# wiedenhoeft/HaMMLET

Hardware: AMD Instinct MI355X
Metric: block-updates/sec (Gibbs sweep) + HBM GB/s, 10^8 pos / 5 states (higher is better)
Workload: dtype f32; 1 GPU; c3_1e8_k5_dynamic; positions=100000000, states=5, block_structure=dynamic, chains=1, parallelism=chain-parallel x1

## Files before the change

### hammlet_amd/capi.py

```python
import ctypes as C
import os

import numpy as np

from . import build as _build

_lib = None


class HmlError(RuntimeError):
    def __init__(self, code, msg):
        super().__init__(msg)
        self.code = code


class HmlStats(C.Structure):
    _fields_ = [("sweeps", C.c_uint64), ("block_updates", C.c_uint64), ("uniform_fallbacks", C.c_uint64),
                ("forward_refits", C.c_uint64), ("forward_serial", C.c_uint64), ("forward_warmup", C.c_uint64),
                ("fused_fallbacks", C.c_uint64), ("buffer_growths", C.c_uint64), ("block_capacity", C.c_uint64)]


RECORD_CB = C.CFUNCTYPE(None, C.c_void_p, C.c_uint64, C.c_void_p)

_P = C.c_void_p
SIGNATURES = {
    "hml_last_error": (C.c_char_p, []),
    "hml_abi_version": (C.c_uint32, []),
    "hml_device_arch": (C.c_char_p, []),
    "hml_device_count": (C.c_int, [C.POINTER(C.c_int)]),
    "hml_create": (C.c_int, [C.POINTER(_P), C.c_int, C.c_uint64, C.c_uint32, _P]),
    "hml_destroy": (None, [_P]),
    "hml_load_observations": (C.c_int, [_P, _P, C.c_uint64]),
    "hml_load_observations_device": (C.c_int, [_P, _P, C.c_uint64]),
    "hml_attach_observations": (C.c_int, [_P, _P]),
    "hml_text_open": (C.c_int, [C.POINTER(_P), C.c_int, C.c_uint64]),
    "hml_text_close": (None, [_P]),
    "hml_text_buffer": (C.c_int, [_P, C.POINTER(_P), C.POINTER(C.c_uint64)]),
    "hml_text_commit": (C.c_int, [_P, C.c_uint64]),
    "hml_text_feed": (C.c_int, [_P, C.c_char_p, C.c_uint64]),
    "hml_text_reserve": (C.c_int, [_P, C.c_uint64]),
    "hml_text_finish": (C.c_int, [_P, C.POINTER(C.c_uint64), C.POINTER(C.c_int)]),
    "hml_text_values": (C.c_int, [_P, _P]),
    "hml_text_counters": (C.c_int, [_P, C.POINTER(C.c_uint64), C.POINTER(C.c_uint64), C.POINTER(C.c_uint64)]),
    "hml_set_dimensions": (C.c_int, [_P, C.c_int, C.c_int]),
    "hml_get_dimensions": (C.c_int, [_P, C.POINTER(C.c_int), C.POINTER(C.c_int)]),
    "hml_set_weights": (C.c_int, [_P, _P, C.c_uint64]),
    "hml_noise_sigma": (C.c_int, [_P, C.POINTER(C.c_double)]),
    "hml_scale_weights": (C.c_int, [_P, C.c_float]),
    "hml_autoprior": (C.c_int, [_P, C.c_float, C.c_float, _P]),
    "hml_set_model": (C.c_int, [_P, C.c_int, _P, C.c_float, C.c_float, C.c_float, C.c_int]),
    "hml_set_self_transitions": (C.c_int, [_P, C.c_int]),
    "hml_sample_prior": (C.c_int, [_P]),
    "hml_set_static_blocks": (C.c_int, [_P]),
    "hml_set_dynamic": (C.c_int, [_P, C.c_int]),
    "hml_create_blocks": (C.c_int, [_P, C.c_float]),
    "hml_iterate": (C.c_int, [_P, C.c_char, C.c_uint64, C.c_uint64]),
    "hml_iterate_many": (C.c_int, [_P, C.c_int, C.c_char, C.c_uint64, C.c_uint64]),
    "hml_set_recording": (C.c_int, [_P, C.c_int, RECORD_CB, _P]),
    "hml_set_option": (C.c_int, [_P, C.c_char_p, C.c_int]),
    "hml_sync": (C.c_int, [_P]),
    "hml_get_num_blocks": (C.c_int, [_P, C.POINTER(C.c_uint64)]),
    "hml_get_blocks": (C.c_int, [_P, _P]),
    "hml_get_block_stats": (C.c_int, [_P, _P, _P]),
    "hml_get_states": (C.c_int, [_P, _P]),
    "hml_get_theta": (C.c_int, [_P, _P]),
    "hml_get_transitions": (C.c_int, [_P, _P, _P]),
    "hml_set_parameters": (C.c_int, [_P, _P, _P, _P]),
    "hml_get_threshold": (C.c_int, [_P, C.POINTER(C.c_float)]),
    "hml_enable_probes": (C.c_int, [_P, C.c_int]),
    "hml_get_block_loglik": (C.c_int, [_P, _P]),
    "hml_get_forward_rows": (C.c_int, [_P, _P]),
    "hml_get_counts": (C.c_int, [_P, _P, _P, _P, _P, _P]),
    "hml_get_weights": (C.c_int, [_P, _P]),
    "hml_get_coefficients": (C.c_int, [_P, _P]),
    "hml_get_integral_array": (C.c_int, [_P, _P, _P]),
    "hml_marginals_rle": (C.c_int, [_P, C.POINTER(C.c_uint64), C.POINTER(C.c_int), _P, _P]),
    "hml_max_segmentation": (C.c_int, [_P, C.POINTER(C.c_uint64), _P, _P]),
    "hml_marginals_dense_device": (C.c_int, [_P, _P, _P]),
    "hml_recorded_sweeps": (C.c_int, [_P, C.POINTER(C.c_uint64)]),
    "hml_set_level_recording": (C.c_int, [_P, C.c_int]),
    "hml_levels_rle": (C.c_int, [_P, C.POINTER(C.c_uint64), C.POINTER(C.c_uint64), _P, _P, _P]),
    "hml_levels_dense_device": (C.c_int, [_P, _P]),
    "hml_levels_merge": (C.c_int, [_P, _P]),
    "hml_levels_on_segments": (C.c_int, [_P, C.c_uint64, _P, _P, _P]),
    "hml_levels_agreement_rle": (C.c_int, [_P, C.c_int, C.POINTER(C.c_uint64), C.POINTER(C.c_uint64), _P, _P, _P, _P]),
    "hml_levels_agreement_dense_device": (C.c_int, [_P, C.c_int, _P]),
    "hml_levels_agreement_summary": (C.c_int, [_P, C.c_int, C.c_double, _P, _P, _P]),
    "hml_set_break_recording": (C.c_int, [_P, C.c_int]),
    "hml_breaks_list": (C.c_int, [_P, C.POINTER(C.c_uint64), C.POINTER(C.c_uint64), _P, _P]),
    "hml_breaks_dense_device": (C.c_int, [_P, _P, C.c_uint32]),
    "hml_breaks_merge": (C.c_int, [_P, _P]),
    "hml_breaks_consensus": (C.c_int, [_P, C.c_uint32, C.c_uint64, C.POINTER(C.c_uint64), _P, _P, _P]),
    "hml_set_level_bands": (C.c_int, [_P, C.c_int, _P]),
    "hml_get_level_bands": (C.c_int, [_P, C.POINTER(C.c_int), _P]),
    "hml_bands_rle": (C.c_int, [_P, C.POINTER(C.c_uint64), C.POINTER(C.c_int), C.POINTER(C.c_uint64), _P, _P]),
    "hml_bands_dense_device": (C.c_int, [_P, _P, C.c_int]),
    "hml_bands_call": (C.c_int, [_P, C.c_uint64, C.POINTER(C.c_uint64), _P, _P]),
    "hml_bands_merge": (C.c_int, [_P, _P]),
    "hml_recording_payload_size": (C.c_int, [_P, C.c_int, C.POINTER(C.c_uint64)]),
    "hml_recording_export": (C.c_int, [_P, C.c_int, _P, C.c_uint64, C.POINTER(C.c_uint64)]),
    "hml_recording_merge_payload": (C.c_int, [_P, C.c_int, _P, C.c_uint64]),
    "hml_recording_merge_across": (C.c_int, [_P, _P, C.c_int]),
    "hml_categorical_draw": (C.c_int, [_P, _P, C.c_int, C.POINTER(C.c_uint32)]),
    "hml_relabel_permutation": (C.c_int, [_P, _P]),
    "hml_pool_payload_size": (C.c_int, [_P, C.POINTER(C.c_uint64)]),
    "hml_pool_export": (C.c_int, [_P, _P, _P]),
    "hml_pool_install": (C.c_int, [_P, _P]),
    "hml_pool_unique_id": (C.c_int, [_P]),
    "hml_pool_create": (C.c_int, [C.POINTER(_P), C.c_int, C.c_int, C.c_int, _P]),
    "hml_pool_destroy": (None, [_P]),
    "hml_pool_marginals": (C.c_int, [_P, _P, _P]),
    "hml_pool_info": (C.c_int, [_P, C.POINTER(C.c_int), C.POINTER(C.c_int), C.POINTER(C.c_double), C.POINTER(C.c_uint64), C.POINTER(C.c_int)]),
    "hml_pool_set_form": (C.c_int, [_P, C.c_int]),
    "hml_pool_last": (C.c_int, [_P, C.POINTER(C.c_int), C.POINTER(C.c_uint64)]),
    "hml_allreduce_marginals": (C.c_int, [_P, C.c_int]),
    "hml_allreduce_marginals_perm": (C.c_int, [_P, C.c_int, _P]),
    "hml_pool_permutation": (C.c_int, [_P, _P]),
    "hml_get_stats": (C.c_int, [_P, C.POINTER(HmlStats)]),
    "hml_profile_enable": (C.c_int, [_P, C.c_int]),
    "hml_profile_get": (C.c_int, [_P, C.c_char_p, C.POINTER(C.c_double), C.POINTER(C.c_uint64)]),
    "hml_debug_eval": (C.c_int, [C.c_int, C.c_int, _P, _P, _P, C.c_uint64, C.c_uint64]),
    "hml_synth_depth": (C.c_int, [_P, _P, C.c_uint64, C.c_double, C.c_double, C.c_uint64, C.c_int]),
    "hml_synth_gauss": (C.c_int, [_P, _P, C.c_uint64, C.c_int, _P, C.c_float, C.c_double, C.c_uint64, C.c_int]),
}


ABI_VERSION = 5

RECORDING_LEVELS, RECORDING_BREAKS, RECORDING_BANDS = 0, 1, 2


def load_library(path=None):
    global _lib
    if _lib is not None and path is None:
        return _lib
    path = path or os.environ.get("HML_LIBRARY") or _build.LIB_PATH
    if not os.path.exists(path):
        raise HmlError(-1, "%s is missing: build it with `python -c 'import __graft_entry__ as g; g.build()'` "
                           "(hipcc --offload-arch=gfx950); there is no CPU fallback" % path)
    lib = C.CDLL(path, mode=C.RTLD_GLOBAL)
    for name, (res, args) in SIGNATURES.items():
        fn = getattr(lib, name)
        fn.restype = res
        fn.argtypes = args
    if lib.hml_abi_version() != ABI_VERSION:
        raise HmlError(-1, "%s has ABI version %d, this package expects %d: rebuild the library" % (path, lib.hml_abi_version(), ABI_VERSION))
    _lib = lib
    return lib


def _check(rc):
    if rc != 0:
        raise HmlError(rc, load_library().hml_last_error().decode())


def parse_text(source, device=0, chunk_bytes=0, feed_bytes=None, with_info=False):
    lib = load_library()
    h = _P()
    _check(lib.hml_text_open(C.byref(h), device, chunk_bytes))
    try:
        if isinstance(source, (bytes, bytearray, memoryview)):
            data = bytes(source)
            step = feed_bytes or max(len(data), 1)
            for i in range(0, len(data), step):
                part = data[i:i + step]
                _check(lib.hml_text_feed(h, part, len(part)))
        else:
            with open(source, "rb", buffering=0) as f:
                while True:
                    buf, cap = _P(), C.c_uint64()
                    _check(lib.hml_text_buffer(h, C.byref(buf), C.byref(cap)))
                    view = (C.c_char * cap.value).from_address(buf.value)
# ... 569 lines not shown
```

### hammlet_amd/csrc/hml_capi.hip

```cpp
#include "hml_capi_shared.hpp"

static thread_local std::string g_err;
int hml_set_err(int code, const std::string& msg) { g_err = msg; return code; }

static const hml_ktab* ktab(int K);
#define HML_KTAB(KV, tab) const hml_ktab* tab = ktab(KV); if (!tab) return set_err(HML_ERR_ARG, "number of states must be in [2,16]")

std::atomic<int> hml_live_ctx[64];
int hml_ctx_bind(hml_ctx* c) { return ctx_bind(c); }
int hml_ctx_fetch_model(hml_ctx* c, hml_model* out) { return fetch_model(c, out); }

HML_KERNEL void hml_k_debug_eval(int fn, const float* __restrict__ a, const float* __restrict__ b, float* __restrict__ out,
                                 uint64_t n, uint64_t seed) {
    if (fn == 24) {
        const uint64_t nw = ((uint64_t)gridDim.x * blockDim.x) >> 6;
        if ((threadIdx.x & 63) != 0) return;
        for (uint64_t i = ((uint64_t)blockIdx.x * blockDim.x + threadIdx.x) >> 6; i < n; i += nw) {
            hml_dev_src src;
            src.s = hml_stream_open(hml_make_key(seed, 0), HML_KIND_THETA, seed, (uint32_t)i);
            out[i] = hml_gamma_f32<hml_devmath>(src, a[i], b[i]);
        }
        return;
    }
    const uint64_t stride = (uint64_t)gridDim.x * blockDim.x;
// ... 23 lines not shown
            case 40: r = hml_glibc_expf(x); break;
            case 41: r = hml_glibc_logf(x); break;
            case 42: r = hml_glibc_powf_unit(x, y); break;
            case 43: { const double Zd = (double)y; r = hml_tr2_quotient(x, Zd, hml_tr2_reciprocal(Zd)); } break;
            case 10: r = (float)(1.0 / (double)x); break;
            case 12: case 13: case 14: case 15: case 16: case 17: case 18: case 19: case 20: case 21: case 22: case 23: {
                hml_dev_src src; src.s = hml_stream_open(hml_make_key(seed, 0), HML_KIND_THETA, seed, (uint32_t)i);
                const float alpha = x, beta = y; (void)beta;
                const float malpha = alpha < 1.0f ? alpha + 1.0f : alpha;
                const float a1 = malpha - 1.0f / 3.0f;
                const float a2 = 1.0f / hml_devmath::sqrtf_(9.0f * a1);
                hml_normal_f32<hml_devmath> nd;
                float n = nd.draw(src, 0.0f, 1.0f);
                float v = 1.0f + a2 * n;
                float v3 = v * v * v;
                float u = hml_canonical_f32(src);
                const bool c1 = (double)u > (double)1.0f - 0.0331 * (double)n * (double)n * (double)n * (double)n;
                const bool c2 = ((double)hml_devmath::logf_(u) > (0.5 * (double)n * (double)n + (double)a1 * ((1.0 - (double)v3) + (double)hml_devmath::logf_(v3))));
                float n2 = nd.draw(src, 0.0f, 1.0f);
                float vb = 1.0f + a2 * n2;
                float vb3 = vb * vb * vb;
                float ub = hml_canonical_f32(src);
                const bool d1 = (double)ub > (double)1.0f - 0.0331 * (double)n2 * (double)n2 * (double)n2 * (double)n2;
                const bool d2 = ((double)hml_devmath::logf_(ub) > (0.5 * (double)n2 * (double)n2 + (double)a1 * ((1.0 - (double)vb3) + (double)hml_devmath::logf_(vb3))));
                r = fn == 12 ? n : fn == 13 ? v3 : fn == 14 ? u : fn == 15 ? (float)(c1 ? 1 : 0) + 2.0f * (c2 ? 1 : 0) : fn == 16 ? n2 : fn == 17 ? a2
                    : fn == 18 ? vb3 : fn == 19 ? ub : fn == 20 ? (float)(d1 ? 1 : 0) + 2.0f * (d2 ? 1 : 0) : fn == 21 ? (float)src.s.n : 0.0f;
                if (fn == 22) r = nd.draw(src, 0.0f, 1.0f);
                if (fn == 23) { hml_normal_f32<hml_devmath> nf; r = nf.draw(src, 0.0f, 1.0f); r = nf.draw(src, 0.0f, 1.0f); }
            } break;
            case 30: case 31: {
                r = 0.0f;
                const int Kc = fn == 30 ? 16 : 5;
                if (i % Kc == 0 && i + Kc <= n) {
                    bool unsure = false;
                    int fastr, lit;
                    if (fn == 30) { float w[16]; for (int j = 0; j < 16; ++j) w[j] = a[i + j]; fastr = hml_categorical_k_fast<16>(w, (double)y, unsure); lit = hml_categorical_k_literal<16>(w, (double)y); if (unsure) fastr = lit; }
                    else { float w[5]; for (int j = 0; j < 5; ++j) w[j] = a[i + j]; fastr = hml_categorical_k_fast<5>(w, (double)y, unsure); lit = hml_categorical_k_literal<5>(w, (double)y); if (unsure) fastr = lit; }
                    out[i] = (float)fastr; out[i + 1] = (float)lit; out[i + 2] = unsure ? 1.0f : 0.0f;
                }
                continue;
            }
            case 11: { const double d = HML_SQRT((double)x * 1.0000001); r = (float)((d - (double)(float)d) * 1e9); } break;
        }
        out[i] = r;
    }
}

static bool parse_band_edges(const char* text, int* n, float* edges) {
    *n = 0;
    const char* p = text;
    while (*p) {
        char* end = nullptr;
        const float v = strtof(p, &end);
        if (end == p || *n >= HML_MAX_BAND_EDGES) return false;
        edges[(*n)++] = v;
        p = end;
        if (*p == ',') ++p; else if (*p) return false;
    }
    return *n > 0;
}

static const char* band_edges_fault(int n, const float* edges) {
    if (n < 1 || n > HML_MAX_BAND_EDGES) return "level bands take 1 to 31 edges";
    for (int j = 0; j < n; ++j) {
        if (!std::isfinite(edges[j])) return "the edges of the level bands must be finite";
        if (j > 0 && !(edges[j - 1] < edges[j])) return "the edges of the level bands must be strictly ascending";
    }
    return nullptr;
}

static int bands_from_env(hml_ctx* c) {
    if (const char* e = getenv("HML_BANDS")) {
        int n = 0; float edges[HML_MAX_BAND_EDGES];
        if (!parse_band_edges(e, &n, edges)) return set_err(HML_ERR_ARG, "HML_BANDS: expected up to 31 comma-separated numbers");
        if (const char* why = band_edges_fault(n, edges)) return set_err(HML_ERR_ARG, std::string("HML_BANDS: ") + why);
        c->n_band_edges = n;
        memcpy(c->band_edges, edges, (size_t)n * sizeof(float));
        c->rec[HML_REC_BANDS].on = c->rec[HML_REC_BANDS].asked = true;
    }
    return 0;
}

extern "C" {

const char* hml_last_error(void) { return g_err.c_str(); }
uint32_t hml_abi_version(void) { return 5; }
const char* hml_device_arch(void) { return "gfx950"; }
int hml_device_count(int* n) {
    if (!n) return set_err(HML_ERR_ARG, "null argument");
    HIPCHK(hipGetDeviceCount(n));
    return 0;
}

static void free_all(hml_ctx* c);

static int create_inner(hml_ctx* c, void* stream) {
    HIPCHK(hipSetDevice(c->device));
    if (stream) { c->stream = (hipStream_t)stream; c->own_stream = false; }
    else { HIPCHK(hipStreamCreateWithFlags(&c->stream, hipStreamNonBlocking)); c->own_stream = true; }
    HIPCHK(hipMalloc(&c->d_mdl, sizeof(hml_model)));
    HIPCHK(hipMemsetAsync(c->d_mdl, 0, sizeof(hml_model), c->stream));
    HIPCHK(hipHostMalloc(&c->h_B, 4 * sizeof(uint32_t), hipHostMallocMapped));
    c->h_B[0] = 0; c->h_B[1] = 0; c->h_B[2] = 0; c->h_B[3] = 0;
    HIPCHK(hipHostGetDevicePointer((void**)&c->d_hB, c->h_B, 0));
    return 0;
}

int hml_create(hml_ctx** out, int device, uint64_t seed, uint32_t chain_id, void* stream) {
    if (!out) return set_err(HML_ERR_ARG, "null output pointer");
    int n = 0;
    HIPCHK(hipGetDeviceCount(&n));
    if (n <= 0) return set_err(HML_ERR_HIP, "no HIP device available: the MI355X kernels cannot run (there is no CPU fallback)");
    if (device < 0 || device >= n) return set_err(HML_ERR_ARG, "device index out of range");
    hml_ctx* c = new hml_ctx();
    c->device = device; c->seed = seed; c->chain = chain_id;
    if (int r = create_inner(c, stream)) {
        free_all(c);
        if (c->own_stream && c->stream) hipStreamDestroy(c->stream);
        delete c;
        return r;
    }
    if (const char* e = getenv("HML_FWD_CHUNK")) { int l = std::max(1, atoi(e)); int sh = 0; while ((1 << (sh + 1)) <= l && sh < 10) ++sh; c->fwdL = 1 << sh; }
    if (const char* e = getenv("HML_FWD_WARMUP")) c->fwdW = c->fwdW_init = std::max(0, atoi(e));
    if (const char* e = getenv("HML_FWD_BURNIN_SWEEPS")) c->fwd_burnin_sweeps = (uint32_t)std::max(0, atoi(e));
    if (const char* e = getenv("HML_FWD_QUIET")) c->fwd_quiet_need = (uint32_t)std::max(1, atoi(e));
    if (const char* e = getenv("HML_FWD_CHUNK_MANY")) { int l = std::max(1, atoi(e)); int sh = 0; while ((1 << (sh + 1)) <= l && sh < 6) ++sh; c->fwdL_many = 1 << sh; }
    if (const char* e = getenv("HML_FWD_CHUNK_MID")) { int l = std::max(1, atoi(e)); int sh = 0; while ((1 << (sh + 1)) <= l && sh < 10) ++sh; c->fwdL_mid = 1 << sh; }
    if (const char* e = getenv("HML_MID_MIN_BLOCKS")) c->mid_min_blocks = (uint32_t)strtoul(e, nullptr, 10);
    if (const char* e = getenv("HML_FWD_CHUNK_DENSE")) { int l = std::max(1, atoi(e)); int sh = 0; while ((1 << (sh + 1)) <= l && sh < 10) ++sh; c->fwdL_dense = 1 << sh; }
    if (const char* e = getenv("HML_DENSE_MIN_BLOCKS")) c->dense_min_blocks = (uint32_t)strtoul(e, nullptr, 10);
    if (const char* e = getenv("HML_USE_GRAPH")) c->use_graph = atoi(e) != 0;
    if (const char* e = getenv("HML_WEIGHT_KEYS")) c->use_keys = atoi(e) != 0;
    if (const char* e = getenv("HML_FUSED_BLOCKS")) { c->fused_blocks = atoi(e) != 0; c->fused_keep = atoi(e) == 2; }
    if (const char* e = getenv("HML_TRELLIS_FUSED")) c->tre_fused = atoi(e) != 0;
    if (const char* e = getenv("HML_TRELLIS_L")) { const int l = atoi(e); c->tre_L = (l <= 0) ? 0u : (l >= HML_TRE_MAX_L) ? (uint32_t)HML_TRE_MAX_L : (l < 32) ? 32u : (uint32_t)l / 32u * 32u; }
    if (const char* e = getenv("HML_TRELLIS_CKPT")) c->tre_ckpt = atoi(e) != 0;
    if (const char* e = getenv("HML_TRELLIS_REFIT_ROUNDS")) { const int r = atoi(e); c->tre_refit_rounds = r < 0 ? 0u : r > 6 ? 6u : (uint32_t)r; }
    if (const char* e = getenv("HML_STAGE_BITS")) c->stage_bits = atoi(e) != 0;
    if (const char* e = getenv("HML_TRELLIS_ROWS")) c->tre_rows = atoi(e) != 0;
    if (const char* e = getenv("HML_LATE_RESCALE")) c->late_rescale = atoi(e) != 0;
    if (const char* e = getenv("HML_PARAMS_SPREAD")) c->params_spread = atoi(e) != 0;
    if (const char* e = getenv("HML_COMPAT_CHUNKS")) c->compat_chunks = atoi(e);
    if (const char* e = getenv("HML_COMPAT_WARMUP")) c->compat_warmup = atoi(e);
    if (const char* e = getenv("HML_WIDE_LANES")) c->wide_lanes = atoi(e);
    if (const char* e = getenv("HML_WIDE_W0")) c->wide_w0 = std::max(8, atoi(e));
    if (const char* e = getenv("HML_WIDE_MAX_CHUNKS")) c->wide_max_chunks = (uint32_t)std::max(64, atoi(e));
    if (const char* e = getenv("HML_WIDE_L")) {
        const int L = atoi(e);
        if (L >= 1) { int sh = 0; while ((1 << sh) < L && sh < 20) ++sh; c->wide_lshift = sh; }
    }
    if (const char* e = getenv("HML_COMPAT")) c->compat = atoi(e) != 0;
    if (const char* e = getenv("HML_TRELLIS_TUNE")) c->tre_autotune = atoi(e) != 0;
    if (const char* e = getenv("HML_FUSED_SPIN_LIMIT")) c->fused_spin_limit = (uint32_t)strtoul(e, nullptr, 10);
    if (const char* e = getenv("HML_LEVELS")) c->rec[HML_REC_LEVELS].on = c->rec[HML_REC_LEVELS].asked = atoi(e) != 0;
    if (const char* e = getenv("HML_BREAKS")) c->rec[HML_REC_BREAKS].on = c->rec[HML_REC_BREAKS].asked = atoi(e) != 0;
    if (const char* e = getenv("HML_MAX_BLOCKS")) c->cap_opt = strtoull(e, nullptr, 10);
    if (device < 64) g_live_ctx[device].fetch_add(1);
    if (int r = bands_from_env(c)) { hml_destroy(c); return r; }
    *out = c;
    return 0;
}

static void trace_release(hml_ctx* c) {
    if (c->trace) {
        if (c->trace->refs.fetch_sub(1) == 1) {
            void* ptrs[] = {c->trace->d_w, c->trace->d_summary, c->trace->d_coeff, c->trace->d_ia};
            for (void* p : ptrs) if (p) hipFree(p);
            delete c->trace;
        }
        c->trace = nullptr;
    } else {
        void* ptrs[] = {c->d_w, c->d_summary, c->d_coeff, c->d_ia};
        for (void* p : ptrs) if (p) hipFree(p);
    }
    c->d_w = nullptr; c->d_summary = nullptr; c->d_coeff = nullptr; c->d_ia = nullptr;
}
static bool trace_shared(const hml_ctx* c) { return c->trace && c->trace->refs.load() > 1; }

static void free_sweep_buffers(hml_ctx* c, bool keep_engine = false) {
    void** ptrs[] = {(void**)&c->d_em, (void**)&c->d_gsc, (void**)&c->d_rows, (void**)&c->d_entry, (void**)&c->d_exitA, (void**)&c->d_redo, (void**)&c->d_touched,
                     (void**)&c->d_fb, (void**)&c->d_smap, (void**)&c->d_cmap, (void**)&c->d_scmap, (void**)&c->d_super, (void**)&c->d_bentry2, (void**)&c->d_bentry,
                     (void**)&c->d_q, (void**)&c->d_partial, (void**)&c->d_redo2, (void**)&c->d_tre_bitmap, (void**)&c->d_tre_ckpt, (void**)&c->d_crows, (void**)&c->d_cchunk, (void**)&c->d_cdraws, (void**)&c->d_clists, (void**)&c->d_wacc, (void**)&c->d_wA};
    for (void** p : ptrs) if (*p) { hipFree(*p); *p = nullptr; }
    if (!keep_engine && c->d_mt) { hipFree(c->d_mt); c->d_mt = nullptr; }
}

static void free_all(hml_ctx* c) {
    trace_release(c);
    free_sweep_buffers(c);
    void* ptrs[] = {c->d_group_word, c->d_wave_total, c->d_stage, c->d_span_count, c->d_starts, c->d_bstat, c->d_eprobe, c->d_aprobe, c->d_coarse1,
                    c->d_diff, c->d_boundary, c->d_mdl, c->d_many};
    for (void* p : ptrs) if (p) hipFree(p);
    for (hml_recorder& r : c->rec) { if (r.d_acc) hipFree(r.d_acc); if (r.d_boundary) hipFree(r.d_boundary); }
    if (c->h_B) hipHostFree(c->h_B);
    c->h_B = nullptr;
}


void hml_destroy(hml_ctx* c) {
    if (!c) return;
    if (c->device < 64) g_live_ctx[c->device].fetch_sub(1);
    hipSetDevice(c->device);
    hipStreamSynchronize(c->stream);
    for (auto& kv : c->prof) for (auto& p : kv.second.pending) { hipEventDestroy(p.first); hipEventDestroy(p.second); }
    for (auto e : c->ev_pool) hipEventDestroy(e);
    if (c->graph_exec) hipGraphExecDestroy(c->graph_exec);
    free_all(c);
    if (c->own_stream) hipStreamDestroy(c->stream);
    delete c;
}

static int build_keys(hml_ctx* c) {
    if (!c->use_keys) return 0;
    const uint64_t T = c->T;
    if (!c->d_summary) {
        const uint64_t n_spans = (T + HML_SPAN - 1) / HML_SPAN;
        HIPCHK(hipMalloc(&c->d_summary, n_spans * (HML_SPAN / 16) + 16));
        HIPCHK(hipMemsetAsync(c->d_summary, 0, n_spans * (HML_SPAN / 16) + 16, c->stream));
    }
    const float thr0 = (float)(std::sqrt(2 * std::log((double)std::max<uint64_t>(T, 2))) * c->sigma * c->key_scale);
    uint32_t u; memcpy(&u, &thr0, 4);
    c->key_base = (std::isfinite(thr0) && thr0 > 0 ? (int32_t)(u >> 20) : (int32_t)(0x3f800000u >> 20)) - 128;
    hipLaunchKernelGGL(hml_k_build_summary, dim3(grid_for((T + 15) / 16, 256, 1, 65536)), dim3(256), 0, c->stream, c->d_w, T,
                       c->key_base, c->d_summary);
    KLAUNCH_CHECK();
    return 0;
}

HML_KERNEL void hml_k_max_inplace(float* __restrict__ a, const float* __restrict__ b, uint64_t n) {
    const uint64_t stride = (uint64_t)gridDim.x * blockDim.x;
    for (uint64_t i = (uint64_t)blockIdx.x * blockDim.x + threadIdx.x; i < n; i += stride) { const float x = a[i], y = b[i]; a[i] = (x < y) ? y : x; }
}

static int alloc_block_buffers(hml_ctx* c) {
    const uint64_t T = c->T;
    c->n_spans = (uint32_t)((T + HML_SPAN - 1) / HML_SPAN);
    HIPCHK(hipMalloc(&c->d_stage, (uint64_t)c->n_spans * HML_SPAN * sizeof(uint16_t)));
    HIPCHK(hipMalloc(&c->d_span_count, c->n_spans * sizeof(uint32_t)));
    HIPCHK(hipMalloc(&c->d_starts, (c->cap + 1) * sizeof(uint32_t)));
    HIPCHK(hipMalloc(&c->d_coarse1, ((c->n_spans + HML_GROUP_SPANS - 1) / HML_GROUP_SPANS + 1u) * sizeof(uint32_t)));
    {
        const uint64_t n_tiles = (T + HML_FUSED_SUB_POSITIONS - 1) / HML_FUSED_SUB_POSITIONS;
        HIPCHK(hipMalloc(&c->d_group_word, (n_tiles + 1) * sizeof(unsigned long long)));
        HIPCHK(hipMemsetAsync(c->d_group_word, 0, (n_tiles + 1) * sizeof(unsigned long long), c->stream));
        HIPCHK(hipMalloc(&c->d_wave_total, (n_tiles + 1) * (HML_FUSED_WAVES + 2) * sizeof(uint32_t)));
        if (getenv("HML_FUSED_DEBUG")) { HIPCHK(hipMalloc(&c->d_dbg, 4096 * 8 * 8)); HIPCHK(hipMemset(c->d_dbg, 0, 4096 * 8 * 8)); }
    }
    HIPCHK(hipMalloc(&c->d_bstat, c->cap * (uint64_t)c->D * sizeof(float2)));
    const uint32_t cap32 = (uint32_t)c->cap;
    HIPCHK(hipMemcpyAsync(&c->d_mdl->cap, &cap32, sizeof cap32, hipMemcpyHostToDevice, c->stream));
    return 0;
}

static void choose_capacity(hml_ctx* c, bool attached) {
    const uint64_t T = c->T;
    uint64_t cap = T;
    if (c->D == 1) {
        if (c->cap_opt) cap = c->cap_opt;
        else if (attached) cap = std::max<uint64_t>(1ull << 20, T / 16);
    }
    c->cap = std::min<uint64_t>(std::max<uint64_t>(cap, 64), T);
}

static int build_from_device_x(hml_ctx* c, const float* const* d_x, const float* const* h_x) {
    const uint64_t T = c->T;
    const int D = c->D;
    {
        trace_release(c);
        void** stale[] = {(void**)&c->d_stage, (void**)&c->d_span_count, (void**)&c->d_starts, (void**)&c->d_coarse1, (void**)&c->d_group_word, (void**)&c->d_wave_total, (void**)&c->d_bstat};
        for (void** q : stale) if (*q) { hipFree(*q); *q = nullptr; }
    }
    {
        const float sqrt2 = (float)std::sqrt(2.0);
        const float sqrt2half = (float)(sqrt2 / 2.0);
        double acc = 0; uint64_t cnt = 0;
        for (uint64_t i = 1; i < T; i += 2) {
            float mx = 0.0f;
            for (int d = 0; d < D; ++d) {
                const float df = std::abs(h_x[d][i - 1] - h_x[d][i]);
                const float cf = sqrt2half * df;
                mx = (mx < cf) ? cf : mx;
            }
            acc += mx;
            cnt++;
        }
        acc /= cnt;
        acc /= 0.797884560802865355879892119868763736951717262329869315331;
        c->sigma = acc;
    }
    HIPCHK(hipMalloc(&c->d_w, T * sizeof(float)));
    HIPCHK(hipMalloc(&c->d_coeff, T * sizeof(float)));
    HIPCHK(hipMalloc(&c->d_ia, (T + 1) * (uint64_t)D * sizeof(float2)));
    {
        float h_norm[64];
        const float sqrt2 = (float)std::sqrt(2.0);
        const float sqrt2half = (float)(sqrt2 / 2.0);
        h_norm[0] = 1.0f;
        float nrm = sqrt2half;
        for (int l = 1; l < 64; ++l) { h_norm[l] = nrm; nrm *= sqrt2half; }
        DevScratch s_norm, s_a, s_b, s_other;
        HIPCHK(hipMalloc(&s_norm.p, sizeof h_norm));
        float* d_norm = s_norm.as<float>();
        HIPCHK(hipMemcpyAsync(d_norm, h_norm, sizeof h_norm, hipMemcpyHostToDevice, c->stream));
        const uint64_t n1 = T >> HML_MAXLET_LOG_TILE;
        HIPCHK(hipMalloc(&s_a.p, std::max<uint64_t>(n1, 1) * sizeof(float)));
        HIPCHK(hipMalloc(&s_b.p, std::max<uint64_t>(n1 >> HML_MAXLET_LOG_TILE, 1) * sizeof(float)));
        if (D > 1) HIPCHK(hipMalloc(&s_other.p, T * sizeof(float)));
        float *bufA = s_a.as<float>(), *bufB = s_b.as<float>(), *d_other = s_other.as<float>();
        for (int d = 0; d < D; ++d) {
            float* coeff_out = d == 0 ? c->d_coeff : d_other;
            uint64_t n = T;
            int base = 0;
            const float* in = d_x[d];
            float* outb = bufA;
            while (true) {
                const uint64_t tiles = (n + HML_MAXLET_TILE - 1) / HML_MAXLET_TILE;
                hipLaunchKernelGGL(hml_k_maxlet, dim3((unsigned)tiles), dim3(256), 0, c->stream, in, n, base, coeff_out, T, outb, d_norm);
                KLAUNCH_CHECK();
                base += HML_MAXLET_LOG_TILE;
                if (base >= 40 || (1ull << base) >= T) break;
                n = T >> base;
                in = outb;
                outb = (outb == bufA) ? bufB : bufA;
            }
            if (d > 0) {
                hipLaunchKernelGGL(hml_k_max_inplace, dim3(grid_for(T, 256, 1, 65536)), dim3(256), 0, c->stream, c->d_coeff, d_other, T);
                KLAUNCH_CHECK();
            }
        }
        HIPCHK(hipStreamSynchronize(c->stream));
    }
    hipLaunchKernelGGL(hml_k_weights, dim3(grid_for(T, 256, 1, 65536)), dim3(256), 0, c->stream, c->d_coeff, c->d_w, T, 1.0f);
    KLAUNCH_CHECK();
    if (int r = build_keys(c)) return r;
    {
        const uint64_t cells = (T + 1 + HML_CELLSIZE - 1) / HML_CELLSIZE;
        for (int d = 0; d < D; ++d) {
            hipLaunchKernelGGL(hml_k_integral, dim3((unsigned)((cells + 3) / 4)), dim3(256), 0, c->stream, d_x[d], c->d_ia + (uint64_t)d * (T + 1), T);
            KLAUNCH_CHECK();
        }
    }
    choose_capacity(c, false);
    if (int r = alloc_block_buffers(c)) return r;
    HIPCHK(hipStreamSynchronize(c->stream));
    c->trace = new hml_trace();
    c->trace->d_w = c->d_w; c->trace->d_summary = c->d_summary; c->trace->d_coeff = c->d_coeff; c->trace->d_ia = c->d_ia;
    c->loaded = true;
    return 0;
}

int hml_set_dimensions(hml_ctx* c, int D, int P) {
    if (!c) return set_err(HML_ERR_ARG, "null context");
    if (c->loaded) return set_err(HML_ERR_ARG, "dimensions must be set before the observations are loaded");
    if (D <= 0) return set_err(HML_ERR_MODEL, "Number of data dimensions must be positive!");
    if (P < 0) return set_err(HML_ERR_MODEL, "Number of parameters must be positive!");
    if (D > HML_MAX_D) return set_err(HML_ERR_ARG, "at most 4 data dimensions are supported");
    if (P > 0) {
        long k = 1;
        for (int d = 0; d < D; ++d) { k *= P; if (k > HML_CAP_K) return set_err(HML_ERR_ARG, "number of states must be in [2,64]"); }
        if (k <= 1) return set_err(HML_ERR_MODEL, "Requested parameters would yield an HMM with less than 2 states!");
    }
    c->D = D; c->P = P;
    return 0;
}

int hml_load_observations(hml_ctx* c, const float* x, uint64_t n_values) {
    if (!c || !x) return set_err(HML_ERR_ARG, "null argument");
    if (n_values == 0) return set_err(HML_ERR_ARG, "Input vector for breakpoint weights is empty!");
    const uint64_t D = (uint64_t)c->D;
    if (n_values % D != 0) return set_err(HML_ERR_MODEL, "Input stream did not contain enough values to fill all dimensions at last position!");
    const uint64_t T = n_values / D;
    if (T >= 0xffffffffull) return set_err(HML_ERR_ARG, "at most 2^32-2 positions are supported");
    if (c->loaded) return set_err(HML_ERR_ARG, "observations already loaded");
    if (int r = ctx_bind(c)) return r;
    c->T = T;
    DevScratch s_x;
    HIPCHK(hipMalloc(&s_x.p, n_values * sizeof(float)));
    float* d_x = s_x.as<float>();
    std::vector<float> planes;
    const float* h_dim[HML_MAX_D];
    const float* d_dim[HML_MAX_D];
    if (D == 1) { h_dim[0] = x; }
    else {
        planes.resize(n_values);
        for (uint64_t t = 0; t < T; ++t) for (uint64_t d = 0; d < D; ++d) planes[d * T + t] = x[t * D + d];
        for (uint64_t d = 0; d < D; ++d) h_dim[d] = planes.data() + d * T;
    }
    HIPCHK(hipMemcpyAsync(d_x, D == 1 ? x : planes.data(), n_values * sizeof(float), hipMemcpyHostToDevice, c->stream));
    for (uint64_t d = 0; d < D; ++d) d_dim[d] = d_x + d * T;
    return build_from_device_x(c, d_dim, h_dim);
}

int hml_load_observations_device(hml_ctx* c, const void* x_dev, uint64_t T) {
    if (!c || !x_dev) return set_err(HML_ERR_ARG, "null argument");
    if (c->D != 1) return set_err(HML_ERR_ARG, "device input is univariate");
    if (T == 0) return set_err(HML_ERR_ARG, "Input vector for breakpoint weights is empty!");
    if (T >= 0xffffffffull) return set_err(HML_ERR_ARG, "at most 2^32-2 positions are supported");
    if (c->loaded) return set_err(HML_ERR_ARG, "observations already loaded");
    if (int r = ctx_bind(c)) return r;
    c->T = T;
    std::vector<float> h(T);
    HIPCHK(hipMemcpy(h.data(), x_dev, T * sizeof(float), hipMemcpyDeviceToHost));
    const float* h_dim[1] = {h.data()};
    const float* d_dim[1] = {(const float*)x_dev};
    return build_from_device_x(c, d_dim, h_dim);
}

int hml_attach_observations(hml_ctx* c, hml_ctx* src) {
    if (!c || !src) return set_err(HML_ERR_ARG, "null argument");
    if (c == src) return set_err(HML_ERR_ARG, "a context cannot be attached to itself");
    if (!src->loaded || !src->trace) return set_err(HML_ERR_ARG, "the source context has no observations loaded");
    if (c->loaded) return set_err(HML_ERR_ARG, "observations already loaded");
    if (c->device != src->device) return set_err(HML_ERR_ARG, "contexts that share observations must live on one device");
    if (c->use_keys != src->use_keys) return set_err(HML_ERR_ARG, "option weight_keys differs from the source context's");
    if (int r = ctx_bind(c)) return r;
    HIPCHK(hipStreamSynchronize(src->stream));
    trace_release(c);
    {
        void** stale[] = {(void**)&c->d_stage, (void**)&c->d_span_count, (void**)&c->d_starts, (void**)&c->d_coarse1, (void**)&c->d_group_word, (void**)&c->d_wave_total, (void**)&c->d_bstat};
        for (void** q : stale) if (*q) { hipFree(*q); *q = nullptr; }
    }
    c->T = src->T; c->D = src->D;
    if (c->P == 0 || c->D > 1) c->P = src->P;
    c->sigma = src->sigma; c->key_base = src->key_base; c->key_scale = src->key_scale;
    c->trace = src->trace;
    c->trace->refs.fetch_add(1);
    c->d_w = src->d_w; c->d_summary = src->d_summary; c->d_coeff = src->d_coeff; c->d_ia = src->d_ia;
    choose_capacity(c, true);
    if (int r = alloc_block_buffers(c)) { trace_release(c); return r; }
    HIPCHK(hipStreamSynchronize(c->stream));
    c->loaded = true;
    return 0;
}

int hml_noise_sigma(hml_ctx* c, double* sigma) {
    if (!c || !c->loaded) return set_err(HML_ERR_ARG, "no observations loaded");
    *sigma = c->sigma;
    return 0;
}

int hml_scale_weights(hml_ctx* c, float mult) {
    if (!c || !c->loaded) return set_err(HML_ERR_ARG, "no observations loaded");
    if (trace_shared(c)) return set_err(HML_ERR_ARG, "the weights are shared with attached contexts: scale them before hml_attach_observations");
    if (int r = ctx_bind(c)) return r;
    hipLaunchKernelGGL(hml_k_scale, dim3(grid_for(c->T, 256, 1, 65536)), dim3(256), 0, c->stream, c->d_w, c->T, mult);
    KLAUNCH_CHECK();
    c->key_scale *= std::fabs((double)mult) > 0 ? std::fabs((double)mult) : 1.0;
    if (int r = build_keys(c)) return r;
    c->blocks_valid = false;
    return 0;
}

int hml_set_weights(hml_ctx* c, const float* w, uint64_t T) {
    if (!c || !c->loaded || !w) return set_err(HML_ERR_ARG, "no observations loaded");
    if (T != c->T) return set_err(HML_ERR_MODEL, "Block structure and statistics have different number of data points!");
    if (trace_shared(c)) return set_err(HML_ERR_ARG, "the weights are shared with attached contexts: set them before hml_attach_observations");
    if (int r = ctx_bind(c)) return r;
    HIPCHK(hipMemcpyAsync(c->d_w, w, T * sizeof(float), hipMemcpyHostToDevice, c->stream));
    HIPCHK(hipStreamSynchronize(c->stream));
    if (int r = build_keys(c)) return r;
    c->blocks_valid = false;
    c->hint_stale = true;
    return 0;
}

}

extern "C" {
}
static int grow_capacity(hml_ctx* c, uint64_t needed);
static int enumerate_blocks_sync(hml_ctx* c, float threshold) {
    if (int r = settle_if_limited(c)) return r;
    for (int round = 0; round < 64; ++round) {
        if (int r = launch_compact(c, true, threshold)) return r;
        HIPCHK(hipStreamSynchronize(c->stream));
        if (!chain_halted(c)) return 0;
        if (int r = grow_capacity(c, c->h_B[2])) return r;
    }
    return set_err(HML_ERR_HIP, "internal error: the block capacity did not settle");
}
extern "C" {

int hml_create_blocks(hml_ctx* c, float threshold) {
    if (!c || !c->loaded) return set_err(HML_ERR_ARG, "no observations loaded");
    if (int r = ctx_bind(c)) return r;
    if (int r = enumerate_blocks_sync(c, threshold)) return r;
    refresh_hint(c);
    c->blocks_valid = false;
    return 0;
}

int hml_autoprior(hml_ctx* c, float s2, float p, float out4[4]) {
    if (!c || !c->loaded) return set_err(HML_ERR_ARG, "no observations loaded");
    if (int r = ctx_bind(c)) return r;
    const float thr0 = (float)(std::sqrt(2 * std::log((double)c->T)) * c->sigma);
    if (int r = enumerate_blocks_sync(c, thr0)) return r;
    refresh_hint(c);
    const uint32_t B = *c->h_B;
    std::vector<uint32_t> st(B + 1);
    const int D = c->D;
    std::vector<float2> bs((size_t)B * D);
    HIPCHK(hipMemcpy(st.data(), c->d_starts, (B + 1) * sizeof(uint32_t), hipMemcpyDeviceToHost));
    for (int d = 0; d < D; ++d)
        HIPCHK(hipMemcpy(bs.data() + (size_t)d * B, c->d_bstat + (uint64_t)d * c->cap, B * sizeof(float2), hipMemcpyDeviceToHost));
    float muSum = 0, muSq = 0;
    for (uint32_t b = 0; b < B; ++b) {
        for (int d = 0; d < D; ++d) {
            const float m = bs[(size_t)d * B + b].x / (float)(st[b + 1] - st[b]);
            muSum += m;
            muSq += m * m;
        }
    }
    const double n = (double)((uint64_t)B * (uint64_t)D);
    const double blocksMean = (double)(float)(muSum / n);
    const double avg = (double)(float)(muSum / n);
    const double blocksVar = (double)(float)(muSq / n - (avg * avg));
    const float dataMean = (float)blocksMean, dataVar = (float)blocksVar;
    if (p < 0 || p > 1) return set_err(HML_ERR_MODEL, "Parameter p for automatic priors is a probability and must be in [0,1]!");
    if (s2 <= 0) return set_err(HML_ERR_MODEL, "Parameter s2  for automatic priors is a variance and must be positive!");
    if (dataVar <= 0) return set_err(HML_ERR_MODEL, "Data variance provided to autoprior must be positive!");
    const float M1 = 0.3361, M2 = -0.0042, M3 = -0.0201;
    const float b = -std::log(p);
    const float alpha = 2.0;
    const float beta = s2 * ((2.0 * std::sqrt(b)) / (M1 * std::sqrt(b) + std::sqrt(2.0) * (M2 * b * std::exp(M3 * std::sqrt(b)) + 1)) + b);
    const float mu0 = dataMean;
    const float nu = beta / dataVar;
    if (beta <= 0) return set_err(HML_ERR_MODEL, "Autoprior yields non-positive beta!");
    if (nu <= 0) return set_err(HML_ERR_MODEL, "Autoprior yields non-positive nu!");
    if (!std::isfinite(beta)) return set_err(HML_ERR_MODEL, "Autoprior yields non-finite beta!");
    if (!std::isfinite(mu0)) return set_err(HML_ERR_MODEL, "Autoprior yields non-finite mu0!");
    if (!std::isfinite(nu)) return set_err(HML_ERR_MODEL, "Autoprior yields non-finite nu!");
    out4[0] = alpha; out4[1] = beta; out4[2] = mu0; out4[3] = nu;
    return 0;
}

}

static uint64_t compat_list_entries(const hml_ctx* c) { return (c->cap + 4u * (uint64_t)HML_CAP_K + 3u) & ~(uint64_t)3u; }

static uint32_t wide_max_chunks_of(const hml_ctx* c) {
    if (c->wide_max_chunks) return std::min<uint32_t>(c->wide_max_chunks, HML_WL_MAX_CHUNKS);
    return c->K <= HML_WL_TWO_WAVES_KC ? (uint32_t)HML_WL_MAX_CHUNKS : (uint32_t)HML_WL_MAX_CHUNKS / 2u;
}

static int alloc_sweep_buffers(hml_ctx* c) {
    const int K = c->K;
    const uint64_t cap = c->cap;
    if (c->compat) {
        HIPCHK(hipMalloc(&c->d_em, cap * K * sizeof(float)));
        HIPCHK(hipMalloc(&c->d_gsc, cap * K * sizeof(float)));
        HIPCHK(hipMalloc(&c->d_crows, (cap + 1) * K * sizeof(float)));
        HIPCHK(hipMalloc(&c->d_cchunk, (uint64_t)HML_COMPAT_MAX_CHUNKS * (2 * K * sizeof(float) + 4 * sizeof(uint32_t)) + 64));
        HIPCHK(hipMalloc(&c->d_cdraws, 2 * cap * sizeof(uint32_t)));
        HIPCHK(hipMalloc(&c->d_clists, 3 * compat_list_entries(c) * sizeof(uint32_t) + (uint64_t)HML_CAP_K * HML_CAP_K * sizeof(unsigned long long) +
                                        ((cap + HML_COMPAT_PART_TILE - 1) / HML_COMPAT_PART_TILE) * K * sizeof(uint32_t) + 2 * (HML_CAP_K + 1) * sizeof(uint32_t) + 64));
        HIPCHK(hipMalloc(&c->d_q, cap * sizeof(int16_t)));
        return 0;
    }
    if (c->wide) {
        uint64_t Lmax = 1ull << HML_WL_MIN_LSHIFT;
        if (c->wide_lshift >= 0) Lmax = std::max<uint64_t>(Lmax, 1ull << c->wide_lshift);
        while ((cap + Lmax - 1) / Lmax > (uint64_t)wide_max_chunks_of(c)) Lmax *= 2;
        const uint64_t plane = (cap + 1 + 64 * Lmax) * K;
        HIPCHK(hipMalloc(&c->d_em, plane * sizeof(float)));
        HIPCHK(hipMalloc(&c->d_gsc, plane * sizeof(float)));
        HIPCHK(hipMalloc(&c->d_crows, plane * sizeof(float)));
        const uint64_t Lmin = c->wide_lshift >= 0 ? (1ull << c->wide_lshift) : (1ull << HML_WL_MIN_LSHIFT);
        c->wide_chunks_cap = std::max<uint64_t>(HML_COMPAT_MAX_CHUNKS, std::min<uint64_t>(HML_WL_MAX_CHUNKS, (cap + Lmin - 1) / Lmin + 64));
        const uint64_t chunk_bytes = c->wide_chunks_cap * (2 * K * sizeof(float) + 4 * sizeof(uint32_t));
        HIPCHK(hipMalloc(&c->d_cchunk, chunk_bytes + HML_WL_TOT_WORDS * sizeof(unsigned long long)));
        HIPCHK(hipMemsetAsync((char*)c->d_cchunk + chunk_bytes, 0, HML_WL_TOT_WORDS * sizeof(unsigned long long), c->stream));
        HIPCHK(hipMalloc(&c->d_wA, ((uint64_t)HML_WL_PITCH * HML_WL_PITCH + (uint64_t)HML_CAP_K * HML_WL_GTAB) * sizeof(float)));
        HIPCHK(hipMalloc(&c->d_cdraws, 2 * (cap + 1) * sizeof(uint32_t)));
        HIPCHK(hipMalloc(&c->d_q, cap * sizeof(int16_t)));
        const uint64_t n_partial = (uint64_t)HML_REDUCE_GROUPS * K * 2;
        HIPCHK(hipMalloc(&c->d_partial, n_partial * sizeof(double)));
        HIPCHK(hipMemsetAsync(c->d_partial, 0, n_partial * sizeof(double), c->stream));
        HIPCHK(hipMalloc(&c->d_wacc, sizeof(hml_wide_acc)));
        HIPCHK(hipMemsetAsync(c->d_wacc, 0, sizeof(hml_wide_acc), c->stream));
        return 0;
    }
    const int minL = std::min(std::min(std::min(c->fwdL, c->fwdL_dense), c->fwdL_many), c->fwdL_mid);
    const uint64_t maxChunks = (cap + minL - 1) / minL + 1;
    uint64_t plane = 0;
    auto layout = [&](int L, hml_layout& lay) {
        int sh = 0; while ((1 << sh) < L) ++sh;
        lay.lshift = (uint32_t)sh;
        lay.cstride = (uint32_t)(((cap + L - 1) / L + 1 + 63) / 64 * 64);
        plane = std::max(plane, (uint64_t)L * K * lay.cstride);
    };
    layout(c->fwdL, c->lay);
    layout(c->fwdL_dense, c->lay_dense);
    layout(c->fwdL_mid, c->lay_mid);
    layout(c->fwdL_many, c->lay_many);
    HIPCHK(hipMalloc(&c->d_em, plane * sizeof(float)));
    HIPCHK(hipMalloc(&c->d_gsc, plane * sizeof(float)));
    HIPCHK(hipMalloc(&c->d_rows, plane * sizeof(float)));
    HIPCHK(hipMalloc(&c->d_entry, maxChunks * K * sizeof(float)));
    HIPCHK(hipMalloc(&c->d_exitA, maxChunks * K * sizeof(float)));
    HIPCHK(hipMalloc(&c->d_fb, maxChunks * sizeof(uint32_t)));
    HIPCHK(hipMalloc(&c->d_smap, (cap + 2) * sizeof(unsigned long long)));
    const uint64_t bchunks = (cap + 15) / 16 + 1;
    HIPCHK(hipMalloc(&c->d_cmap, bchunks * sizeof(unsigned long long)));
    HIPCHK(hipMalloc(&c->d_bentry, bchunks));
    HIPCHK(hipMalloc(&c->d_scmap, bchunks * sizeof(unsigned long long)));
    HIPCHK(hipMalloc(&c->d_super, (bchunks / 64 + 2) * sizeof(unsigned long long)));
    HIPCHK(hipMalloc(&c->d_bentry2, bchunks / 64 + 2));
    HIPCHK(hipMalloc(&c->d_redo, bchunks * sizeof(uint32_t)));
    HIPCHK(hipMemsetAsync(c->d_redo, 0, bchunks * sizeof(uint32_t), c->stream));
    HIPCHK(hipMalloc(&c->d_touched, bchunks * sizeof(uint32_t)));
    HIPCHK(hipMemsetAsync(c->d_touched, 0, bchunks * sizeof(uint32_t), c->stream));
    HIPCHK(hipMalloc(&c->d_redo2, bchunks * sizeof(uint32_t)));
    HIPCHK(hipMalloc(&c->d_tre_bitmap, (bchunks / 32 + 2) * sizeof(uint32_t)));
    HIPCHK(hipMalloc(&c->d_tre_ckpt, (cap / HML_TRE_CKPT_ROWS + 64) * (uint64_t)(K + 1) * sizeof(uint32_t)));
    HIPCHK(hipMalloc(&c->d_q, cap * sizeof(int16_t)));
    const uint64_t n_partial = ((uint64_t)HML_REDUCE_GROUPS + HML_PARAMS_TREE_WGS) * K * 2;
    HIPCHK(hipMalloc(&c->d_partial, n_partial * sizeof(double)));
    HIPCHK(hipMemsetAsync(c->d_partial, 0, n_partial * sizeof(double), c->stream));
    return 0;
}

static int grow_capacity(hml_ctx* c, uint64_t needed) {
    const uint64_t cap = std::min<uint64_t>(c->T, std::max<uint64_t>(needed + needed / 2 + 1024, 2 * c->cap));
    if (c->graph_exec) { hipGraphExecDestroy(c->graph_exec); c->graph_exec = nullptr; }
    void** blocks[] = {(void**)&c->d_starts, (void**)&c->d_bstat};
    for (void** q : blocks) if (*q) { hipFree(*q); *q = nullptr; }
    free_sweep_buffers(c,  true);
    if (c->d_eprobe) { hipFree(c->d_eprobe); c->d_eprobe = nullptr; }
    if (c->d_aprobe) { hipFree(c->d_aprobe); c->d_aprobe = nullptr; }
    c->cap = cap;
    HIPCHK(hipMalloc(&c->d_starts, (cap + 1) * sizeof(uint32_t)));
    HIPCHK(hipMalloc(&c->d_bstat, cap * (uint64_t)c->D * sizeof(float2)));
    if (c->model_set) {
        if (int r = alloc_sweep_buffers(c)) return r;
        if (c->probes) {
            HIPCHK(hipMalloc(&c->d_eprobe, c->cap * c->K * sizeof(float)));
            HIPCHK(hipMalloc(&c->d_aprobe, (c->cap + 1) * c->K * sizeof(float)));
        }
    }
    const uint32_t words[2] = {(uint32_t)cap, 0u};
    static_assert(offsetof(hml_model, halted) == offsetof(hml_model, cap) + sizeof(uint32_t), "cap and halted are written together");
    HIPCHK(hipMemcpyAsync(&c->d_mdl->cap, words, sizeof words, hipMemcpyHostToDevice, c->stream));
    HIPCHK(hipStreamSynchronize(c->stream));
    c->h_B[2] = 0u;
    c->blocks_valid = false;
    c->hint_stale = false;
    c->grown++;
    return 0;
}

static int sweep_dispatch(hml_ctx* c, char method, bool record);

int hml_settle(hml_ctx* c) {
    for (int round = 0; round < 64; ++round) {
        HIPCHK(hipStreamSynchronize(c->stream));
        if (!chain_halted(c)) { c->sweep_log.clear(); c->log_base = c->requested; return 0; }
        const uint64_t needed = c->h_B[2];
        if (c->cap >= c->T) return set_err(HML_ERR_HIP, "internal error: a chain with full block capacity halted");
        std::vector<uint8_t> pending;
        if (c->model_set) {
            hml_model m;
            if (int r = fetch_model(c, &m)) return r;
            const uint64_t ran = m.sweeps >= c->log_base ? m.sweeps - c->log_base : 0;
            if (ran < c->sweep_log.size()) pending.assign(c->sweep_log.begin() + ran, c->sweep_log.end());
            c->log_base = m.sweeps;
        }
        if (int r = grow_capacity(c, needed)) return r;
        c->sweep_log = pending;
        bool halted_again = false;
        for (size_t i = 0; i < pending.size() && !halted_again; ++i) {
            const char method = (pending[i] & 1) ? HML_METHOD_MIXTURE : HML_METHOD_FB;
            const bool record = (pending[i] & 2) != 0;
            if (int r = sweep_dispatch(c, method, record)) return r;
            if (record && c->cb) {
                HIPCHK(hipStreamSynchronize(c->stream));
                halted_again = chain_halted(c);
                if (!halted_again) {
                    if (int r = check_device_error(c)) return r;
                    const unsigned long long ordinal = c->log_base + i;
                    c->cb(c, ordinal >= c->call_base ? (uint64_t)(ordinal - c->call_base) : 0u, c->cb_user);
                }
            }
        }
    }
    return set_err(HML_ERR_HIP, "internal error: the block capacity did not settle");
}

extern "C" {

int hml_set_model(hml_ctx* c, int K, const float nig4[4], float a_off, float a_diag, float pi_alpha, int self_trans) {
    if (!c || !c->loaded) return set_err(HML_ERR_ARG, "no observations loaded");
    if (K < 2) return set_err(HML_ERR_MODEL, "Requested parameters would yield an HMM with less than 2 states!");
    if (K > HML_CAP_K) return set_err(HML_ERR_ARG, "number of states must be in [2,64]");
    if (c->model_set) return set_err(HML_ERR_ARG, "model already set");
    if (c->D > 1 && c->P == 0) {
        for (int pp = 2; pp <= K; ++pp) { long k = 1; for (int d = 0; d < c->D; ++d) k *= pp; if (k == K) { c->P = pp; break; } if (k > K) break; }
        if (c->P == 0) return set_err(HML_ERR_ARG, "number of states must be (number of parameters)^(data dimensions)");
    }
    if (c->P > 0) {
        long k = 1;
        for (int d = 0; d < c->D; ++d) k *= c->P;
        if (k != K) return set_err(HML_ERR_ARG, "number of states must be (number of parameters)^(data dimensions)");
    }
    if (!(nig4[0] > 0)) return set_err(HML_ERR_MODEL, "Alpha (" + std::to_string(nig4[0]) + ") must be positive!");
    if (!(nig4[1] > 0)) return set_err(HML_ERR_MODEL, "Beta (" + std::to_string(nig4[1]) + ") must be positive!");
    if (!(nig4[3] > 0)) return set_err(HML_ERR_MODEL, "Nu (" + std::to_string(nig4[3]) + ")must be positive!");
    const hml_ktab* kt = nullptr;
    c->wide = !c->compat && (K > HML_MAX_K || (getenv("HML_WIDE") && atoi(getenv("HML_WIDE")) != 0));
    if (!c->compat && !c->wide) { kt = ktab(K); if (!kt) return set_err(HML_ERR_ARG, "number of states must be in [2,16]"); }
    if (int r = ctx_bind(c)) return r;
    free_sweep_buffers(c);
    c->K = K;
    if (!getenv("HML_PARAMS_SPREAD")) c->params_spread = K >= 8;
    const uint64_t T = c->T;
    if (int r = alloc_sweep_buffers(c)) return r;

    hml_model m;
    memset(&m, 0, sizeof m);
    m.K = K; m.self_trans = self_trans ? 1 : 0; m.dynamic = 1; m.T = (uint32_t)T;
    m.D = c->D; m.P = c->P > 0 ? c->P : K; m.stat_stride = T;
    m.cap = (uint32_t)c->cap;
    for (int st = 0; st < K; ++st) {
        int nn = st;
        for (int d = 0; d < HML_MAX_D; ++d) { m.map[st][d] = (uint8_t)(d < c->D ? nn % m.P : 0); nn /= m.P; }
    }
    for (int i = 0; i < 4; ++i) m.nig_prior[i] = nig4[i];
    m.a_off = a_off; m.a_diag = a_diag; m.pi_alpha = pi_alpha;
    m.key = hml_make_key(c->seed, c->chain);
    for (int k = 0; k < K; ++k) {
        for (int i = 0; i < 4; ++i) m.nig_post[k][i] = nig4[i];
        m.dirPi[k] = pi_alpha;
        m.pi[k] = 1.0f / K;
        for (int j = 0; j < K; ++j) { m.dirA[k * K + j] = (k == j) ? a_diag : a_off; m.A[k * K + j] = 1.0f / K; }
    }
    m.max_state_recorded = -1;
    m.tre_fused = (c->tre_fused && c->D == 1) ? 1u : 0u;
    m.tre_hi_shift = 17u; m.tre_lo_shift = 20u;
    if (const char* e = getenv("HML_TRE_REFIT_SHIFTS")) { unsigned a = 17, b = 20; if (sscanf(e, "%u,%u", &a, &b) == 2 && a < 32 && b < 32) { m.tre_hi_shift = a; m.tre_lo_shift = b; } }
    m.fwd_W0 = (uint32_t)c->fwdW;
    m.fwd_W = m.fwd_W_burnin = (uint32_t)std::max(c->fwdW, c->fwdW_init);
    if (c->compat || c->wide) { m.fwd_W = 64u; m.fwd_W0 = c->wide ? (uint32_t)c->wide_w0 : 32u; }
    m.wl_bwd_W = 64u; m.wl_bwd_quiet = 0u; m.wl_retry = 0u; m.wl_W_need = 0u; m.wl_need_age = 0u;
    m.fwd_burnin_sweeps = c->fwd_burnin_sweeps;
    m.fwd_quiet_need = c->fwd_quiet_need;
    m.n_spans = c->n_spans;
    HIPCHK(hipMemcpyAsync(c->d_mdl, &m, sizeof m, hipMemcpyHostToDevice, c->stream));
    HIPCHK(hipStreamSynchronize(c->stream));
    c->dynamic = true;
    c->hint_stale = true;
    if (c->compat) {
        hml_mt_state h;
        hml_mt_seed(&h, c->seed + (uint64_t)c->chain);
        HIPCHK(hipMalloc(&c->d_mt, sizeof(hml_mt_state)));
        HIPCHK(hipMemcpyAsync(c->d_mt, &h, sizeof h, hipMemcpyHostToDevice, c->stream));
        HIPCHK(hipStreamSynchronize(c->stream));
        hipLaunchKernelGGL(hml_k_compat_draw, dim3(1), dim3(64), 0, c->stream, c->d_mdl, (hml_mt_state*)c->d_mt, 2);
        KLAUNCH_CHECK();
        c->model_set = true;
        return 0;
    }
    if (c->wide) hipLaunchKernelGGL(hml_k_wide_params, dim3(1), dim3(1024), 0, c->stream, c->d_mdl, c->d_partial, (hml_wide_acc*)c->d_wacc, 2);
    else kt->params(c, 2);
    KLAUNCH_CHECK();
    c->model_set = true;
    return 0;
}

int hml_sample_prior(hml_ctx* c) {
    if (!c || !c->model_set) return set_err(HML_ERR_ARG, "model not set");
    if (int r = ctx_bind(c)) return r;
    if (int r = settle_if_limited(c)) return r;
    if (c->compat) {
        hipLaunchKernelGGL(hml_k_compat_draw, dim3(1), dim3(64), 0, c->stream, c->d_mdl, (hml_mt_state*)c->d_mt, 1);
    } else if (c->wide) {
        hipLaunchKernelGGL(hml_k_wide_params, dim3(1), dim3(1024), 0, c->stream, c->d_mdl, c->d_partial, (hml_wide_acc*)c->d_wacc, 1);
    } else { HML_KTAB(c->K, kt); kt->params(c, 1); }
    KLAUNCH_CHECK();
    if (c->dynamic) c->blocks_valid = false;
    c->hint_stale = true;
    return 0;
}

HML_KERNEL __launch_bounds__(64) void hml_k_set_self_trans(hml_model* mdl, int on) {
    if (threadIdx.x == 0) mdl->self_trans = on;
}

int hml_set_self_transitions(hml_ctx* c, int on) {
    if (!c || !c->model_set) return set_err(HML_ERR_ARG, "model not set");
    if (int r = ctx_bind(c)) return r;
    if (int r = settle_if_limited(c)) return r;
    hipLaunchKernelGGL(hml_k_set_self_trans, dim3(1), dim3(64), 0, c->stream, c->d_mdl, on ? 1 : 0);
    KLAUNCH_CHECK();
    if (c->graph_exec) { hipGraphExecDestroy(c->graph_exec); c->graph_exec = nullptr; }
    return 0;
}

int hml_set_static_blocks(hml_ctx* c) {
    if (!c || !c->model_set) return set_err(HML_ERR_ARG, "model not set");
    if (int r = ctx_bind(c)) return r;
    if (int r = settle_if_limited(c)) return r;
    hipLaunchKernelGGL(hml_k_set_dynamic, dim3(1), dim3(64), 0, c->stream, c->d_mdl, 0, 1);
    KLAUNCH_CHECK();
    c->dynamic = false;
    if (!cap_limited(c)) {
        if (int r = launch_compact(c, false, 0.0f)) return r;
    } else {
        bool fitted = false;
        for (int round = 0; round < 64 && !fitted; ++round) {
            if (int r = launch_compact(c, false, 0.0f)) return r;
            HIPCHK(hipStreamSynchronize(c->stream));
            fitted = !chain_halted(c);
            if (!fitted) { if (int r = grow_capacity(c, c->h_B[2])) return r; }
        }
        if (!fitted) return set_err(HML_ERR_HIP, "internal error: the block capacity did not settle");
        refresh_hint(c);
    }
    c->blocks_valid = true;
    return 0;
}

int hml_set_dynamic(hml_ctx* c, int on) {
    if (!c || !c->model_set) return set_err(HML_ERR_ARG, "model not set");
    if (int r = ctx_bind(c)) return r;
    if (int r = settle_if_limited(c)) return r;
    hipLaunchKernelGGL(hml_k_set_dynamic, dim3(1), dim3(64), 0, c->stream, c->d_mdl, on ? 1 : 0, on ? 1 : 0);
    KLAUNCH_CHECK();
    c->dynamic = on != 0;
    if (on) { c->blocks_valid = false; c->hint_stale = true; }
    return 0;
}

int hml_set_recording(hml_ctx* c, int marginals, hml_record_cb cb, void* user) {
// ... 161 lines not shown
    const int mix = method == HML_METHOD_MIXTURE ? 1 : 0;
    const bool lanes = c->wide_lanes != 0 && !c->probes && !mix && c->compat_chunks == 0;
    if (lanes) {
        hml_compat_chunks ch = chunk_views(c);
        ch.W = c->compat_warmup > 0 ? (uint32_t)c->compat_warmup : c->compat_warmup < 0 ? 0u : HML_CHUNK_W_ADAPTIVE;
        const uint64_t room = (uint64_t)hint + hint / 4 + 1024;
        hipLaunchKernelGGL(hml_k_wl_prepare, dim3(1), dim3(256), 0, s, c->d_mdl, c->d_wA, c->wide_lshift, wide_max_chunks_of(c));
        hipLaunchKernelGGL(hml_k_wl_gtable, dim3(grid_for((uint64_t)c->K * HML_WL_GTAB, 256, 1, 512)), dim3(256), 0, s, c->d_mdl, c->d_wA + HML_WL_PITCH * HML_WL_PITCH);
        {
            ProfScope ps(c, "stats_emission");
            hipLaunchKernelGGL(hml_k_wl_emission, dim3(grid_for(room, 64 * HML_WL_EMIT_ROWS * 4, 1, 32768)), dim3(256), 0, s, c->d_mdl, c->d_starts, c->d_bstat, c->d_em, c->d_gsc, c->d_wA + HML_WL_PITCH * HML_WL_PITCH);
        }
        const uint64_t minL = c->wide_lshift >= 0 ? (1ull << c->wide_lshift) : (1ull << HML_WL_MIN_LSHIFT);
        const int tiles = grid_for(room, (int)std::min<uint64_t>(64 * minL, 1u << 30), 1, HML_WL_MAX_CHUNKS / 64);
#define HML_WL_FB(KC)                                                                                                                                   \
        case KC: {                                                                                                                                      \
            constexpr int KS = (KC <= 32) ? 32 : 64;                                                                                                    \
            {                                                                                                                                           \
                ProfScope ps(c, "forward");                                                                                                             \
                hipLaunchKernelGGL(HIP_KERNEL_NAME(hml_k_wl_forward<KC>), dim3(tiles), dim3(64), 0, s, c->d_mdl, c->d_wA, c->d_em, c->d_gsc, c->d_crows, ch, 0); \
                hipLaunchKernelGGL(hml_k_wl_forward_verify, dim3(grid_for(room / 16 * c->K, 256, 1, 4096)), dim3(256), 0, s, c->d_mdl, ch, 0);          \
                                      \
                hipLaunchKernelGGL(hml_k_wl_retry_decide, dim3(1), dim3(256), 0, s, c->d_mdl, ch);                                                      \
                hipLaunchKernelGGL(HIP_KERNEL_NAME(hml_k_wl_forward<KC>), dim3(tiles), dim3(64), 0, s, c->d_mdl, c->d_wA, c->d_em, c->d_gsc, c->d_crows, ch, 1); \
                hipLaunchKernelGGL(hml_k_wl_forward_verify, dim3(grid_for(room / 16 * c->K, 256, 1, 4096)), dim3(256), 0, s, c->d_mdl, ch, 1);          \
                hipLaunchKernelGGL(HIP_KERNEL_NAME(hml_k_wl_forward_check<KS>), dim3(1), dim3(256), 0, s, c->d_mdl, c->d_em, c->d_gsc, c->d_crows, ch);  \
            }                                                                                                                                           \
            {                                                                                                                                           \
                ProfScope ps(c, "backward_maps");                                                                                                       \
                hipLaunchKernelGGL(HIP_KERNEL_NAME(hml_k_wl_backward<KC>), dim3(tiles), dim3(64), 0, s, c->d_mdl, c->d_crows, c->d_q, ch);               \
                hipLaunchKernelGGL(hml_k_wl_backward_verify, dim3(grid_for(room / 16, 256, 1, 256)), dim3(256), 0, s, c->d_mdl, ch);                     \
                hipLaunchKernelGGL(HIP_KERNEL_NAME(hml_k_wl_backward_check<KS>), dim3(1), dim3(256), 0, s, c->d_mdl, c->d_crows, c->d_q, ch);          \
            }                                                                                                                                           \
        } break;
        switch ((c->K + 3) / 4 * 4) {
            HML_WL_FB(4) HML_WL_FB(8) HML_WL_FB(12) HML_WL_FB(16)
            HML_WL_FB(20) HML_WL_FB(24) HML_WL_FB(28) HML_WL_FB(32) HML_WL_FB(36) HML_WL_FB(40) HML_WL_FB(44) HML_WL_FB(48) HML_WL_FB(52) HML_WL_FB(56)
            HML_WL_FB(60) HML_WL_FB(64)
            default: return set_err(HML_ERR_HIP, "internal error: a model of this many states on the path for more than 16");
        }
#undef HML_WL_FB
    } else {
    {
        ProfScope ps(c, "stats_emission");
        hipLaunchKernelGGL(hml_k_wide_emission, dim3(grid_for(hint, 256, 1, 4096)), dim3(256), 0, s, c->d_mdl, c->d_starts, c->d_bstat,
                           c->d_em, c->d_gsc, mix, c->probes ? c->d_eprobe : nullptr);
    }
    if (mix) hipLaunchKernelGGL(hml_k_wide_mixture, dim3(grid_for(hint, 256, 1, 16384)), dim3(256), 0, s, c->d_mdl, c->d_em, c->d_q);
    else {
        float* const aprobe = c->probes ? c->d_aprobe : nullptr;
        uint32_t C = 1u;
        if (!c->probes && c->compat_chunks > 1) C = std::min<uint32_t>((uint32_t)c->compat_chunks, HML_COMPAT_MAX_CHUNKS);
        else if (!c->probes && c->compat_chunks == 0 && hint >= 2048u) C = std::min<uint32_t>((uint32_t)HML_COMPAT_MAX_CHUNKS, hint / 64u);
        hml_compat_chunks ch = chunk_views(c);
        ch.W = c->compat_warmup > 0 ? (uint32_t)c->compat_warmup : c->compat_warmup < 0 ? 0u : HML_CHUNK_W_ADAPTIVE;
        hipLaunchKernelGGL(hml_k_wide_uniforms, dim3(grid_for((hint + 1u) / 2u, 256, 1, 4096)), dim3(256), 0, s, c->d_mdl, c->d_cdraws);
        if (c->K <= 32) launch_chunked_fb<32, hml_dev_exp, true>(c, s, C, ch, aprobe);
        else launch_chunked_fb<64, hml_dev_exp, true>(c, s, C, ch, aprobe);
    }
    }
    {
        ProfScope ps(c, "counts");
        hipLaunchKernelGGL(hml_k_wide_counts, dim3(HML_REDUCE_GROUPS), dim3(256), 0, s, c->d_q, c->d_starts, c->d_bstat, c->d_mdl, c->d_partial, (hml_wide_acc*)c->d_wacc);
    }
    if (record && c->rec_marginals) {
        if (c->pooled) return set_err(HML_ERR_ARG, "the marginals of this context are pooled (common labels, several chains): further sweeps cannot be recorded into them");
        if (int r = ensure_marginal_buffers(c)) return r;
        hipLaunchKernelGGL(hml_k_record, dim3(grid_for(hint, 256, 64, 16384)), dim3(256), 0, s, c->d_q, c->d_starts, c->d_mdl, c->d_diff, c->d_boundary);
    }
    {
        ProfScope ps(c, "params");
        hipLaunchKernelGGL(hml_k_wide_params, dim3(1), dim3(1024), 0, s, c->d_mdl, c->d_partial, (hml_wide_acc*)c->d_wacc, 0);
    }
    if (record) { if (int r = launch_recorders(c, s, hint)) return r; }
    KLAUNCH_CHECK();
    return 0;
}

static int sweep_dispatch(hml_ctx* c, char method, bool record) {
    if (c->compat) return sweep_compat(c, method, record);
    if (c->wide) return sweep_wide(c, method, record);
    HML_KTAB(c->K, kt);
    return kt->sweep(c, method, record);
}

extern "C" {

int hml_iterate(hml_ctx* c, char method, uint64_t iterations, uint64_t thinning) {
    if (!c || !c->model_set) return set_err(HML_ERR_ARG, "model not set");
    if (method != HML_METHOD_FB && method != HML_METHOD_MIXTURE)
        return set_err(HML_ERR_ARG, std::string("Unknown sampling type ") + method + "!");
    if (int r = ctx_bind(c)) return r;
    c->call_base = c->requested;
    if (thinning > 0 && thinning <= iterations && c->rec_marginals && c->pooled)
        return set_err(HML_ERR_ARG, "the marginals of this context are pooled (common labels, several chains): further sweeps cannot be recorded into them");
    for (uint64_t i = 0; i < iterations; ++i) {
        const bool record = thinning > 0 && ((i + 1) % thinning == 0);
        if (chain_halted(c)) { if (int r = hml_settle(c)) return r; }
        refresh_hint(c);
        const bool tre_path = c->tre_fused && c->D == 1 && method == HML_METHOD_FB && c->B_hint >= c->dense_min_blocks;
        if (c->use_graph && !c->compat && !record && !c->profiling && !c->probes && (c->dynamic || c->blocks_valid) &&
            !(tre_path && tre_wants_measurement(c, c->B_hint))) {
            const uint32_t hint = c->B_hint;
            bool unused = false;
            const bool wants_fused = c->fused_blocks && !(c->h_B[1] && !c->fused_keep) && !shares_device(c);
            const bool stale = !c->graph_exec || c->graph_method != method || c->graph_dynamic != c->dynamic ||
                               hint > c->graph_hint || hint * 2u < c->graph_hint || c->graph_fused != wants_fused ||
                               c->graph_dense != (hint >= c->dense_min_blocks) || c->graph_mid != (hint >= c->mid_min_blocks) ||
                               (tre_path && c->graph_tre_L != tre_pick_L(c, hint, true, &unused));
            if (stale && hint) {
                if (c->graph_exec) { hipGraphExecDestroy(c->graph_exec); c->graph_exec = nullptr; }
                hipGraph_t g = nullptr;
                HIPCHK(hipStreamBeginCapture(c->stream, hipStreamCaptureModeThreadLocal));
                int rr = sweep_dispatch(c, method, false);
                const hipError_t ec = hipStreamEndCapture(c->stream, &g);
                if (rr || ec != hipSuccess) {
                    if (g) hipGraphDestroy(g);
                    (void)hipGetLastError();
                    return rr ? rr : set_err(HML_ERR_HIP, std::string("hipStreamEndCapture: ") + hipGetErrorString(ec));
                }
                const hipError_t ei = hipGraphInstantiate(&c->graph_exec, g, nullptr, nullptr, 0);
                hipGraphDestroy(g);
                if (ei != hipSuccess) { c->graph_exec = nullptr; return set_err(HML_ERR_HIP, std::string("hipGraphInstantiate: ") + hipGetErrorString(ei)); }
                c->graph_method = method; c->graph_dynamic = c->dynamic; c->graph_hint = c->B_hint; c->graph_fused = wants_fused;
                c->graph_dense = c->B_hint >= c->dense_min_blocks;
                c->graph_mid = c->B_hint >= c->mid_min_blocks;
            }
            if (c->graph_exec) {
                log_sweep(c, method, false);
                HIPCHK(hipGraphLaunch(c->graph_exec, c->stream));
                if (tre_path) c->tre_dense_sweeps++;
                continue;
            }
        }
        log_sweep(c, method, record);
        if (int r = sweep_dispatch(c, method, record)) return r;
        if (record && c->cb) {
            HIPCHK(hipStreamSynchronize(c->stream));
            if (chain_halted(c)) { if (int r = hml_settle(c)) return r; continue; }
            if (int r = check_device_error(c)) return r;
            c->cb(c, i, c->cb_user);
        }
    }
    return 0;
}

}

extern "C" int hml_iterate_many(hml_ctx* const* cs, int n, char method, uint64_t iterations, uint64_t thinning) {
    if (!cs || n < 1) return set_err(HML_ERR_ARG, "no contexts");
    for (int i = 0; i < n; ++i) if (!cs[i] || !cs[i]->model_set) return set_err(HML_ERR_ARG, "model not set");
    if (method != HML_METHOD_FB && method != HML_METHOD_MIXTURE) return set_err(HML_ERR_ARG, std::string("Unknown sampling type ") + method + "!");
    for (int i = 0; i < n; ++i) cs[i]->call_base = cs[i]->requested;
    uint64_t done = 0;
    while (done < iterations && many_eligible(cs, n, method)) {
        if (int r = ctx_bind(cs[0])) return r;
        for (int i = 0; i < n; ++i) {
            hml_ctx* c = cs[i];
            if (int r = settle_if_limited(c)) return r;
            if (c->hint_stale) { launch_compact_pair(c, 0, 0.0f); KLAUNCH_CHECK(); }
            HIPCHK(hipStreamSynchronize(c->stream));
            c->hint_stale = false;
            if (c->graph_exec) { hipGraphExecDestroy(c->graph_exec); c->graph_exec = nullptr; }
        }
        int r = 0;
        uint64_t reached = done;
        { HML_KTAB(cs[0]->K, kt); r = kt->iterate_many(cs, n, done, iterations, thinning, &reached); }
        if (r) return r;
        hipEvent_t ev = ev_get(cs[0]);
        HIPCHK(hipEventRecord(ev, cs[0]->stream));
        for (int i = 1; i < n; ++i) HIPCHK(hipStreamWaitEvent(cs[i]->stream, ev, 0));
        cs[0]->ev_pool.push_back(ev);
        if (reached == iterations) return 0;
        HIPCHK(hipStreamSynchronize(cs[0]->stream));
        bool halted = false;
        for (int i = 0; i < n; ++i) halted = halted || chain_halted(cs[i]);
        const bool progress = reached > done;
        done = reached;
        if (!halted && !progress) break;
        if (!halted) { bool sparse = true; for (int i = 0; i < n; ++i) sparse = sparse && many_sparse(cs[i]); if (!sparse) break; }
    }
    for (int i = 0; i < n; ++i) if (int r = settle_if_limited(cs[i])) return r;
    for (uint64_t i = done; i < iterations; ++i) {
        const bool record = thinning > 0 && ((i + 1) % thinning == 0);
        for (int k = 0; k < n; ++k) {
            hml_ctx* c = cs[k];
            if (int r = ctx_bind(c)) return r;
            if (record && c->rec_marginals && c->pooled) return set_err(HML_ERR_ARG, "the marginals of a context are pooled (common labels, several chains): further sweeps cannot be recorded into them");
            if (chain_halted(c)) { if (int r = hml_settle(c)) return r; }
            log_sweep(c, method, record);
            if (int r = sweep_dispatch(c, method, record)) return r;
            if (record && c->cb) {
                HIPCHK(hipStreamSynchronize(c->stream));
                if (chain_halted(c)) { if (int r = hml_settle(c)) return r; continue; }
                if (int r = check_device_error(c)) return r;
                c->cb(c, i, c->cb_user);
            }
        }
    }
    return 0;
}

extern "C" {

int hml_set_option(hml_ctx* c, const char* name, int value) {
    if (!c || !name) return set_err(HML_ERR_ARG, "null argument");
    if (std::string(name) == "weight_keys") {
        if (c->loaded) return set_err(HML_ERR_ARG, "weight_keys must be set before the observations are loaded");
        c->use_keys = value != 0;
        c->summary_always = value == 2;
        return 0;
    }
    if (std::string(name) == "max_blocks") {
        if (c->loaded) return set_err(HML_ERR_ARG, "max_blocks must be set before the observations are loaded");
        if (value < 0) return set_err(HML_ERR_ARG, "max_blocks: a number of blocks, or 0 for the default");
        c->cap_opt = (uint64_t)value;
        return 0;
    }
    if (std::string(name) == "fused_blocks") {
        c->fused_blocks = value != 0;
        c->fused_keep = value == 2;
        if (c->graph_exec) { hipGraphExecDestroy(c->graph_exec); c->graph_exec = nullptr; }
        return 0;
    }
    if (std::string(name) == "compat") {
        if (c->model_set) return set_err(HML_ERR_ARG, "compat must be set before the model");
        c->compat = value != 0;
        return 0;
    }
    if (std::string(name) == "trellis_L") {
        if (value < 0 || value > HML_TRE_MAX_L || value % 32) return set_err(HML_ERR_ARG, "trellis_L: 0 or a multiple of 32 up to 1024");
        c->tre_L = (uint32_t)value;
        return 0;
    }
    return set_err(HML_ERR_ARG, std::string("unknown option ") + name);
}

int hml_sync(hml_ctx* c) {
    if (!c) return set_err(HML_ERR_ARG, "null context");
    if (int r = ctx_bind(c)) return r;
    if (int r = hml_settle(c)) return r;
    if (c->d_dbg && getenv("HML_FUSED_DEBUG") && atoi(getenv("HML_FUSED_DEBUG")) == 2) {
        std::vector<unsigned long long> h(4096 * 8);
        hipMemcpy(h.data(), c->d_dbg, h.size() * 8, hipMemcpyDeviceToHost);
        uint32_t n = 0; while (n < 4096 && h[n * 8]) ++n;
        unsigned long long t0 = ~0ull; for (uint32_t i = 0; i < n; ++i) t0 = std::min(t0, h[i * 8]);
        double mx[5] = {0, 0, 0, 0, 0}, av[5] = {0, 0, 0, 0, 0};
        if (n) for (uint32_t i = 0; i < n; ++i) for (int k = 0; k < 5; ++k) { const double d = (double)(h[i * 8 + k] - t0) * 0.01; mx[k] = std::max(mx[k], d); av[k] += d / n; }
        if (n) fprintf(stderr, "[fused-many dbg] n=%u start avg %.2f max %.2f | phaseA avg %.2f max %.2f | requested avg %.2f max %.2f | offsets avg %.2f max %.2f | end avg %.2f max %.2f (us)\n",
                n, av[0], mx[0], av[1], mx[1], av[2], mx[2], av[3], mx[3], av[4], mx[4]);
        if (n) for (uint32_t i : {0u, n / 4, n / 2, n - 1}) if (i < n) fprintf(stderr, "   wg %u: %.2f %.2f %.2f %.2f %.2f | wavefront 0: parameters in LDS %.2f, weights arrived %.2f, its lists done %.2f\n", i, (h[i*8]-t0)*0.01, (h[i*8+1]-t0)*0.01, (h[i*8+2]-t0)*0.01, (h[i*8+3]-t0)*0.01, (h[i*8+4]-t0)*0.01,
                                                                                  (h[i*8+5]-t0)*0.01, (h[i*8+6]-t0)*0.01, (h[i*8+7]-t0)*0.01);
    } else if (c->d_dbg) {
        std::vector<unsigned long long> h(4096 * 4);
        hipMemcpy(h.data(), c->d_dbg, h.size() * 8, hipMemcpyDeviceToHost);
        const uint32_t n = (uint32_t)std::min<uint64_t>(4096, (c->T + HML_FUSED_SUB_POSITIONS - 1) / HML_FUSED_SUB_POSITIONS);
        unsigned long long t0 = ~0ull; for (uint32_t i = 0; i < n; ++i) if (h[i * 4]) t0 = std::min(t0, h[i * 4]);
        double mx[4] = {0, 0, 0, 0}, av[4] = {0, 0, 0, 0};
        for (uint32_t i = 0; i < n; ++i) for (int k = 0; k < 4; ++k) { const double d = (double)(h[i * 4 + k] - t0) * 0.01; mx[k] = std::max(mx[k], d); av[k] += d / n; }
        fprintf(stderr, "[fused dbg] n=%u start avg %.2f max %.2f | phaseA avg %.2f max %.2f | offsets avg %.2f max %.2f | end avg %.2f max %.2f (us)\n", n, av[0], mx[0], av[1], mx[1], av[2], mx[2], av[3], mx[3]);
        { uint32_t late = 0, first_late = n; for (uint32_t i = 0; i < n; ++i) if ((h[i * 4] - t0) * 0.01 > 2.0) { ++late; first_late = std::min(first_late, i); }
          fprintf(stderr, "   late starters: %u, first index %u\n", late, first_late); }
        for (uint32_t i : {0u, n / 4, n / 2, n - 1}) fprintf(stderr, "   wg %u: %.2f %.2f %.2f %.2f\n", i, (h[i*4]-t0)*0.01, (h[i*4+1]-t0)*0.01, (h[i*4+2]-t0)*0.01, (h[i*4+3]-t0)*0.01);
    }
    if (c->model_set && getenv("HML_PARAMS_DEBUG")) {
        hml_model m;
        if (fetch_model(c, &m) == 0) {
            fprintf(stderr, "[params dbg] us since the kernel's start: accumulators read %.2f | tree %.2f | theta drawn %.2f | A gammas %.2f | barrier %.2f | end %.2f\n",
                    (m.dbg_t[1] - m.dbg_t[0]) * 0.01, (m.dbg_t[2] - m.dbg_t[0]) * 0.01, (m.dbg_t[3] - m.dbg_t[0]) * 0.01, (m.dbg_t[4] - m.dbg_t[0]) * 0.01,
                    (m.dbg_t[5] - m.dbg_t[0]) * 0.01, (m.dbg_t[6] - m.dbg_t[0]) * 0.01);
            fprintf(stderr, "[params dbg]   theta's gamma core + normal drawn %.2f | last wavefront's tree %.2f\n", (m.dbg_t[7] - m.dbg_t[0]) * 0.01, (m.dbg_t[8] - m.dbg_t[0]) * 0.01);
        }
    }
    if (c->model_set) return check_device_error(c);
    return 0;
}


static int current_B(hml_ctx* c, uint32_t* B) {
    HIPCHK(hipMemcpyAsync(c->h_B, &c->d_mdl->B, sizeof(uint32_t), hipMemcpyDeviceToHost, c->stream));
    HIPCHK(hipStreamSynchronize(c->stream));
    *B = *c->h_B;
    return 0;
}

int hml_get_num_blocks(hml_ctx* c, uint64_t* B) {
    NEED_LOADED();
    uint32_t b; if (int r = current_B(c, &b)) return r;
    *B = b; return 0;
}
int hml_get_blocks(hml_ctx* c, uint32_t* starts) {
    NEED_LOADED();
    uint32_t b; if (int r = current_B(c, &b)) return r;
    HIPCHK(hipMemcpy(starts, c->d_starts, ((uint64_t)b + 1) * sizeof(uint32_t), hipMemcpyDeviceToHost));
    return 0;
}
int hml_get_block_stats(hml_ctx* c, float* sum, float* sum_sq) {
    NEED_LOADED();
    uint32_t b; if (int r = current_B(c, &b)) return r;
    std::vector<float2> v(b);
    for (int d = 0; d < c->D; ++d) {
        HIPCHK(hipMemcpy(v.data(), c->d_bstat + (uint64_t)d * c->T, (uint64_t)b * sizeof(float2), hipMemcpyDeviceToHost));
        for (uint32_t i = 0; i < b; ++i) { sum[(uint64_t)d * b + i] = v[i].x; sum_sq[(uint64_t)d * b + i] = v[i].y; }
    }
    return 0;
}
int hml_get_states(hml_ctx* c, int16_t* q) {
    NEED_MODEL();
    uint32_t b; if (int r = current_B(c, &b)) return r;
    HIPCHK(hipMemcpy(q, c->d_q, (uint64_t)b * sizeof(int16_t), hipMemcpyDeviceToHost));
    return 0;
}
int hml_get_theta(hml_ctx* c, float* mean_var) {
    NEED_MODEL();
    hml_model m; if (int r = fetch_model(c, &m)) return r;
    for (int k = 0; k < m.P; ++k) { mean_var[2 * k] = m.mu[k]; mean_var[2 * k + 1] = m.var[k]; }
    return 0;
}
int hml_get_dimensions(hml_ctx* c, int* D, int* P) {
    if (!c) return set_err(HML_ERR_ARG, "null context");
    if (D) *D = c->D;
    if (P) *P = c->P > 0 ? c->P : c->K;
    return 0;
}
int hml_get_transitions(hml_ctx* c, float* A, float* pi) {
    NEED_MODEL();
    hml_model m; if (int r = fetch_model(c, &m)) return r;
    if (A) memcpy(A, m.A, (size_t)c->K * c->K * sizeof(float));
    if (pi) memcpy(pi, m.pi, (size_t)c->K * sizeof(float));
    return 0;
}
int hml_set_parameters(hml_ctx* c, const float* mean_var, const float* A, const float* pi) {
    NEED_MODEL();
    hml_model m; if (int r = fetch_model(c, &m)) return r;
    const int K = c->K;
    for (int k = 0; k < m.P; ++k) {
        const float mean = mean_var[2 * k], var = mean_var[2 * k + 1];
        if (!std::isfinite(mean)) return set_err(HML_ERR_MODEL, "Mean (" + std::to_string(mean) + ") must be set to a finite value!");
        if (!std::isfinite(var)) return set_err(HML_ERR_MODEL, "Variance(" + std::to_string(var) + ") must be set to a finite value!");
        if (var <= 0) return set_err(HML_ERR_MODEL, "Variance (" + std::to_string(var) + ") must be positive!");
        m.mu[k] = mean; m.var[k] = var; m.sd[k] = sqrtf(var);
    }
    memcpy(m.A, A, (size_t)K * K * sizeof(float));
    memcpy(m.pi, pi, (size_t)K * sizeof(float));
    HIPCHK(hipMemcpyAsync(c->d_mdl, &m, sizeof m, hipMemcpyHostToDevice, c->stream));
    if (c->compat) hipLaunchKernelGGL(hml_k_compat_derive, dim3(1), dim3(64), 0, c->stream, c->d_mdl);
    else if (c->wide) hipLaunchKernelGGL(hml_k_wide_derive, dim3(1), dim3(64), 0, c->stream, c->d_mdl);
    else { HML_KTAB(K, kt); kt->derive(c); }
    KLAUNCH_CHECK();
    HIPCHK(hipStreamSynchronize(c->stream));
    if (c->dynamic) c->blocks_valid = false;
    return 0;
}
int hml_get_threshold(hml_ctx* c, float* thr) {
    NEED_MODEL();
    hml_model m; if (int r = fetch_model(c, &m)) return r;
    *thr = m.thr; return 0;
}
int hml_get_block_loglik(hml_ctx* c, float* E) {
    NEED_MODEL();
    if (!c->probes) return set_err(HML_ERR_ARG, "probes are not enabled");
    uint32_t b; if (int r = current_B(c, &b)) return r;
    HIPCHK(hipMemcpy(E, c->d_eprobe, (uint64_t)b * c->K * sizeof(float), hipMemcpyDeviceToHost));
    return 0;
}
int hml_get_forward_rows(hml_ctx* c, float* rows) {
    NEED_MODEL();
    if (!c->probes) return set_err(HML_ERR_ARG, "probes are not enabled");
    uint32_t b; if (int r = current_B(c, &b)) return r;
    HIPCHK(hipMemcpy(rows, c->d_aprobe, ((uint64_t)b + 1) * c->K * sizeof(float), hipMemcpyDeviceToHost));
    return 0;
}
int hml_get_counts(hml_ctx* c, uint64_t* trans, uint64_t* occ, float* sum, float* sum_sq, uint64_t* nterms) {
    NEED_MODEL();
    hml_model m; if (int r = fetch_model(c, &m)) return r;
    const int K = c->K;
    for (int i = 0; i < K * K; ++i) trans[i] = m.last_trans[i];
    for (int k = 0; k < K; ++k) { occ[k] = m.last_occ[k]; nterms[k] = m.last_occ[k]; sum[k] = m.last_sum[k]; sum_sq[k] = m.last_sumsq[k]; }
    return 0;
}
int hml_get_weights(hml_ctx* c, float* w) {
    NEED_LOADED();
    HIPCHK(hipStreamSynchronize(c->stream));
    HIPCHK(hipMemcpy(w, c->d_w, c->T * sizeof(float), hipMemcpyDeviceToHost));
    return 0;
}
int hml_get_coefficients(hml_ctx* c, float* cf) {
    NEED_LOADED();
    HIPCHK(hipStreamSynchronize(c->stream));
    HIPCHK(hipMemcpy(cf, c->d_coeff, c->T * sizeof(float), hipMemcpyDeviceToHost));
    return 0;
}
int hml_get_integral_array(hml_ctx* c, float* sum, float* sum_sq) {
    NEED_LOADED();
    HIPCHK(hipStreamSynchronize(c->stream));
    std::vector<float2> v(c->T + 1);
    HIPCHK(hipMemcpy(v.data(), c->d_ia, (c->T + 1) * sizeof(float2), hipMemcpyDeviceToHost));
    for (uint64_t i = 0; i <= c->T; ++i) { sum[i] = v[i].x; sum_sq[i] = v[i].y; }
    return 0;
}

int hml_recorded_sweeps(hml_ctx* c, uint64_t* n) {
    NEED_MODEL();
    hml_model m; if (int r = fetch_model(c, &m)) return r;
    *n = m.n_recorded; return 0;
}

int hml_relabel_permutation(hml_ctx* c, int32_t* perm) {
    NEED_MODEL();
    if (!perm) return set_err(HML_ERR_ARG, "null argument");
    hml_model m; if (int r = fetch_model(c, &m)) return r;
    const int K = c->K, D = m.D;
    std::vector<int32_t> p(K);
    for (int k = 0; k < K; ++k) p[k] = k;
    std::stable_sort(p.begin(), p.end(), [&](int32_t a, int32_t b) {
        for (int d = 0; d < D; ++d) {
            const float ma = m.mu[m.map[a][d]], mb = m.mu[m.map[b][d]];
            if (ma < mb) return true;
            if (mb < ma) return false;
        }
        return false;
    });
    for (int k = 0; k < K; ++k) perm[k] = p[k];
    return 0;
}

int hml_categorical_draw(hml_ctx* c, const float* weights, int K, uint32_t* index) {
    if (!c || !weights || !index || K < 1) return set_err(HML_ERR_ARG, "invalid argument");
    if (K == 1) { *index = 0; return 0; }
    const uint64_t n = c->host_draws++;
    const hml_u32x4 o = hml_stream4(hml_make_key(c->seed, c->chain), HML_KIND_HOST, n >> 32, (uint32_t)n, 0);
    *index = (uint32_t)hml_categorical(weights, K, hml_canonical_f64(o.v[0], o.v[1]));
    return 0;
}

int hml_get_stats(hml_ctx* c, hml_stats* out) {
    NEED_MODEL();
    hml_model m; if (int r = fetch_model(c, &m)) return r;
    out->sweeps = m.sweeps; out->block_updates = m.block_updates; out->uniform_fallbacks = m.uniform_fallbacks;
    out->forward_refits = m.forward_refits; out->forward_serial = m.forward_serial;
    out->forward_warmup = m.fwd_W;
    out->fused_fallbacks = m.fused_fallbacks;
    out->buffer_growths = c->grown; out->block_capacity = c->cap;
    return 0;
}

int hml_profile_enable(hml_ctx* c, int on) {
    if (!c) return set_err(HML_ERR_ARG, "null context");
    if (on && c->ev_pool.size() < 64) {
        if (int r = ctx_bind(c)) return r;
        while (c->ev_pool.size() < 64) { hipEvent_t e; HIPCHK(hipEventCreate(&e)); c->ev_pool.push_back(e); }
    }
    c->profiling = on;
    return 0;
}

int hml_profile_get(hml_ctx* c, const char* name, double* total_ms, uint64_t* launches) {
    if (!c) return set_err(HML_ERR_ARG, "null context");
    if (int r = ctx_bind(c)) return r;
    HIPCHK(hipStreamSynchronize(c->stream));
    auto& acc = c->prof[name];
    for (auto& p : acc.pending) {
        float ms = 0;
        hipEventElapsedTime(&ms, p.first, p.second);
        acc.ms += ms; acc.n++;
        c->ev_pool.push_back(p.first); c->ev_pool.push_back(p.second);
    }
    acc.pending.clear();
    if (total_ms) *total_ms = acc.ms;
    if (launches) *launches = acc.n;
    return 0;
}

int hml_debug_eval(int device, int fn, const float* a, const float* b, float* out, uint64_t n, uint64_t seed) {
    HIPCHK(hipSetDevice(device));
    float *d_a = nullptr, *d_b = nullptr, *d_o = nullptr;
    HIPCHK(hipMalloc(&d_a, n * 4)); HIPCHK(hipMalloc(&d_o, n * 4));
    HIPCHK(hipMemcpy(d_a, a, n * 4, hipMemcpyHostToDevice));
    if (b) { HIPCHK(hipMalloc(&d_b, n * 4)); HIPCHK(hipMemcpy(d_b, b, n * 4, hipMemcpyHostToDevice)); }
    hipLaunchKernelGGL(hml_k_debug_eval, dim3(1024), dim3(256), 0, 0, fn, d_a, d_b, d_o, n, seed);
    KLAUNCH_CHECK();
    HIPCHK(hipMemcpy(out, d_o, n * 4, hipMemcpyDeviceToHost));
    hipFree(d_a); hipFree(d_o); if (d_b) hipFree(d_b);
    return 0;
}

int hml_synth_gauss(float* x, int16_t* states, uint64_t T, int K, const float* mu, float sigma, double mean_dwell,
                    uint64_t seed, int nthreads) {
    if (!x || !mu || K < 1) return set_err(HML_ERR_ARG, "invalid argument");
    hml_synth_gauss_trace(x, states, T, K, mu, sigma, mean_dwell, seed, nthreads);
    return 0;
}


int hml_synth_depth(float* x, int16_t* states, uint64_t T, double depth, double ln_sigma, uint64_t seed, int nthreads) {
    if (!x) return set_err(HML_ERR_ARG, "invalid argument");
    hml_synth_depth_trace(x, states, T, depth, ln_sigma, seed, nthreads);
    return 0;
}

}


#if defined(HML_ONLY_K)
#define HML_DECLARE_KTAB_(K) extern hml_ktab hml_ktab_##K; static const hml_ktab* ktab(int k) { return k == K ? &hml_ktab_##K : nullptr; }
#define HML_DECLARE_KTAB(K) HML_DECLARE_KTAB_(K)
HML_DECLARE_KTAB(HML_ONLY_K)
#else
#define HML_EXT_KTAB(K) extern hml_ktab hml_ktab_##K;
HML_EXT_KTAB(2) HML_EXT_KTAB(3) HML_EXT_KTAB(4) HML_EXT_KTAB(5) HML_EXT_KTAB(6) HML_EXT_KTAB(7) HML_EXT_KTAB(8) HML_EXT_KTAB(9)
HML_EXT_KTAB(10) HML_EXT_KTAB(11) HML_EXT_KTAB(12) HML_EXT_KTAB(13) HML_EXT_KTAB(14) HML_EXT_KTAB(15) HML_EXT_KTAB(16)
static const hml_ktab* ktab(int k) {
    static const hml_ktab* const tabs[17] = {nullptr, nullptr, &hml_ktab_2, &hml_ktab_3, &hml_ktab_4, &hml_ktab_5, &hml_ktab_6, &hml_ktab_7, &hml_ktab_8,
                                             &hml_ktab_9, &hml_ktab_10, &hml_ktab_11, &hml_ktab_12, &hml_ktab_13, &hml_ktab_14, &hml_ktab_15, &hml_ktab_16};
    return (k >= 2 && k <= 16) ? tabs[k] : nullptr;
}
#endif
```

### hammlet_amd/csrc/hml_capi_shared.hpp

```cpp
#ifndef HML_CAPI_SHARED_HPP
#define HML_CAPI_SHARED_HPP

#include <hip/hip_runtime.h>

#include <algorithm>
#include <atomic>
#include <cmath>
#include <cstdio>
#include <cstring>
#include <map>
#include <string>
#include <vector>

#include "../../include/hml.h"
#include "hml_k_backward.h"
#include "hml_k_blocks.h"
#include "hml_k_blocks_fused.h"
#include "hml_k_blocks_fused_many.h"
#include "hml_k_build.h"
#include "hml_k_forward.h"
#include "hml_k_marginals.h"
#include "hml_k_scan.h"
#include "hml_k_levels.h"
#include "hml_k_breaks.h"
#include "hml_k_bands.h"
#include "hml_k_segment.h"
#include "hml_k_trellis.h"
#include "hml_k_trellis_rows.h"
#include "hml_k_compat.h"
#include "hml_k_wide.h"
#include "hml_k_wide_lanes.h"
#include "hml_k_blocks_split_many.h"
#include "hml_k_many.h"
#include "hml_k_params.h"
#include "hml_state.h"
#include "hml_synth_host.hpp"

#include "hml_host_common.hpp"
#include "hml_ctx.hpp"

int hml_set_err(int code, const std::string& msg);
static int set_err(int code, const std::string& msg) { return hml_set_err(code, msg); }


struct hml_ktab {
    int (*sweep)(hml_ctx* c, char method, bool record);
    int (*iterate_many)(hml_ctx* const* cs, int n, uint64_t first, uint64_t iterations, uint64_t thinning, uint64_t* done);
    void (*params)(hml_ctx* c, int mode);
    void (*derive)(hml_ctx* c);
};

extern std::atomic<int> hml_live_ctx[64];
#define g_live_ctx hml_live_ctx
static bool shares_device(const hml_ctx* c) { return c->device < 64 && g_live_ctx[c->device].load() > 1; }


static int ctx_bind(hml_ctx* c) {
    HIPCHK(hipSetDevice(c->device));
    return 0;
}

static hipEvent_t ev_get(hml_ctx* c) {
    if (!c->ev_pool.empty()) { hipEvent_t e = c->ev_pool.back(); c->ev_pool.pop_back(); return e; }
    hipEvent_t e;
    hipEventCreate(&e);
    return e;
}

struct ProfScope {
    hml_ctx* c; const char* name; hipEvent_t a = nullptr, b = nullptr;
    bool on;
    ProfScope(hml_ctx* c_, const char* n, int level = 2) : c(c_), name(n), on(c_->profiling >= level) {
        if (on && c->profiling == 1 && (c->prof[name].tick++ & 31u) != 0u) on = false;
        if (on) { a = ev_get(c); b = ev_get(c); hipEventRecord(a, c->stream); }
    }
    ~ProfScope() {
        if (!on) return;
        hipEventRecord(b, c->stream);
        c->prof[name].pending.push_back({a, b});
        if (c->profiling == 1) {
            hipEvent_t n0 = ev_get(c), n1 = ev_get(c);
            hipEventRecord(n0, c->stream);
            hipEventRecord(n1, c->stream);
            c->prof["event_null"].pending.push_back({n0, n1});
        }
    }
};

struct DevScratch {
    void* p = nullptr;
    ~DevScratch() { if (p) hipFree(p); }
    template <typename T> T* as() const { return static_cast<T*>(p); }
};

static int grid_for(uint64_t items, int per_block, int lo, int hi) {
    uint64_t g = (items + per_block - 1) / per_block;
    if (g < (uint64_t)lo) g = lo;
    if (g > (uint64_t)hi) g = hi;
    return (int)g;
}

static const char* deverr_text(uint32_t code, float v, char* buf, size_t n) {
    switch (code) {
        case HML_DEVERR_IP_NOT_FINITE: snprintf(buf, n, "Result of Normal inner product is not finite!"); break;
        case HML_DEVERR_NEG_BACKWARD: snprintf(buf, n, "Negative backward variable!"); break;
        case HML_DEVERR_NEG_SUMSQ: snprintf(buf, n, "Sum of squares is negative (%s)!", std::to_string(v).c_str()); break;
        case HML_DEVERR_NIG_ALPHA: snprintf(buf, n, "Alpha (%s) must be positive!", std::to_string(v).c_str()); break;
        case HML_DEVERR_NIG_BETA: snprintf(buf, n, "Beta (%s) must be positive!", std::to_string(v).c_str()); break;
        case HML_DEVERR_NIG_NU: snprintf(buf, n, "Nu (%s)must be positive!", std::to_string(v).c_str()); break;
        case HML_DEVERR_NIG_MU0: snprintf(buf, n, "Mu0 (%s)  must be finite!", std::to_string(v).c_str()); break;
        case HML_DEVERR_MEAN_NOT_FINITE: snprintf(buf, n, "Mean (%s) must be set to a finite value!", std::to_string(v).c_str()); break;
        case HML_DEVERR_VAR_NOT_FINITE: snprintf(buf, n, "Variance(%s) must be set to a finite value!", std::to_string(v).c_str()); break;
        case HML_DEVERR_VAR_NOT_POSITIVE: snprintf(buf, n, "Variance (%s) must be positive!", std::to_string(v).c_str()); break;
        case HML_DEVERR_TOO_MANY_RECORDS: snprintf(buf, n, "Too many recorded iterations for the marginal counters!"); break;
        case HML_DEVERR_LAUNCH_GEOMETRY: snprintf(buf, n, "internal error: a one-wavefront kernel was launched with %d threads per workgroup", (int)v); break;
        default: snprintf(buf, n, "device error %u", code);
    }
    return buf;
}

static int fetch_model(hml_ctx* c, hml_model* out) {
    HIPCHK(hipMemcpyAsync(out, c->d_mdl, sizeof(hml_model), hipMemcpyDeviceToHost, c->stream));
    HIPCHK(hipStreamSynchronize(c->stream));
    return 0;
}

static int check_device_error(hml_ctx* c) {
    struct { uint32_t code; float value; } e;
    static_assert(offsetof(hml_model, err_value) == offsetof(hml_model, err_code) + sizeof(uint32_t), "err_code and err_value are read together");
    HIPCHK(hipMemcpyAsync(&e, &c->d_mdl->err_code, sizeof e, hipMemcpyDeviceToHost, c->stream));
    HIPCHK(hipStreamSynchronize(c->stream));
    if (e.code != 0) {
        char buf[256];
        return set_err(HML_ERR_MODEL, deverr_text(e.code, e.value, buf, sizeof buf));
    }
    return 0;
}



static void launch_compact_pair(hml_ctx* c, int mode, float thr) {
    const uint32_t n_groups = (c->n_spans + HML_GROUP_SPANS - 1) / HML_GROUP_SPANS;
    const bool dense = !c->summary_always && c->B_hint && (uint64_t)c->B_hint * 24u > c->T;
    const bool bits = dense && c->stage_bits;
    {
        ProfScope ps(c, "blocks_compact", 1);
        if (c->use_keys && !dense) {
            hipLaunchKernelGGL(hml_k_compact_scan_summary, dim3(n_groups), dim3(256), 0, c->stream, c->d_summary, c->d_w,
                               (uint32_t)c->T, c->d_mdl, thr, mode, c->key_base, c->d_stage, c->d_span_count, c->d_coarse1);
        } else if (bits) {
            hipLaunchKernelGGL(hml_k_compact_scan_bits, dim3((c->n_spans + 3) / 4), dim3(256), 0, c->stream, c->d_w, (uint32_t)c->T,
                               c->d_mdl, thr, mode, (unsigned long long*)c->d_stage, c->d_span_count);
        } else {
            hipLaunchKernelGGL(hml_k_compact_scan, dim3((c->n_spans + 3) / 4), dim3(256), 0, c->stream, c->d_w, (uint32_t)c->T,
                               c->d_mdl, thr, mode, c->d_stage, c->d_span_count);
        }
    }
    {
        ProfScope ps(c, "blocks_scatter");
        if (!(c->use_keys && !dense))
            hipLaunchKernelGGL(hml_k_group_totals, dim3((n_groups + 255) / 256), dim3(256), 0, c->stream, c->d_span_count,
                               c->n_spans, c->d_coarse1);
        if (bits)
            hipLaunchKernelGGL(hml_k_compact_scatter_bits, dim3(n_groups), dim3(256), 0, c->stream, (const unsigned long long*)c->d_stage,
                               c->d_span_count, c->d_coarse1, c->n_spans, (uint32_t)c->T, c->d_mdl, c->d_starts, c->d_hB);
        else
        hipLaunchKernelGGL(hml_k_compact_scatter, dim3(n_groups), dim3(256), 0, c->stream, c->d_stage, c->d_span_count,
                           c->d_coarse1, c->n_spans, (uint32_t)c->T, c->d_mdl, c->d_starts, c->d_hB);
    }
}

static int launch_compact(hml_ctx* c, bool use_override, float thr) {
    launch_compact_pair(c, use_override ? 1 : 0, thr);
    KLAUNCH_CHECK();
    {
        ProfScope ps(c, "block_stats");
        const uint32_t hint = c->B_hint ? c->B_hint : (uint32_t)std::min<uint64_t>(c->T, 1u << 20);
        for (int d = 0; d < c->D; ++d)
            hipLaunchKernelGGL(hml_k_block_stats, dim3(grid_for(hint, 256, 64, 16384)), dim3(256), 0, c->stream,
                               c->d_ia + (uint64_t)d * (c->T + 1), c->d_starts, c->d_mdl, c->d_bstat + (uint64_t)d * c->T);
    }
    KLAUNCH_CHECK();
    return 0;
}

static inline bool cap_limited(const hml_ctx* c) { return c->cap != 0 && c->cap < c->T; }
static inline bool chain_halted(const hml_ctx* c) { return cap_limited(c) && ((volatile uint32_t*)c->h_B)[2] != 0u; }
static inline void log_sweep(hml_ctx* c, char method, bool record) {
    c->requested++;
    if (cap_limited(c)) c->sweep_log.push_back((uint8_t)((method == HML_METHOD_MIXTURE ? 1 : 0) | (record ? 2 : 0)));
}
static inline int settle_if_limited(hml_ctx* c) { return cap_limited(c) ? hml_settle(c) : 0; }

#define NEED_MODEL() if (!c || !c->model_set) return set_err(HML_ERR_ARG, "model not set"); if (int r_ = ctx_bind(c)) return r_; if (int r_ = settle_if_limited(c)) return r_
#define NEED_LOADED() if (!c || !c->loaded) return set_err(HML_ERR_ARG, "no observations loaded"); if (int r_ = ctx_bind(c)) return r_; if (int r_ = settle_if_limited(c)) return r_

static void refresh_hint(hml_ctx* c) {
    const uint32_t b = *(volatile uint32_t*)c->h_B;
    if (b) c->B_hint = b + b / 4 + 1024;
}


static int ensure_marginal_buffers(hml_ctx* c) {
    if (c->d_diff) return 0;
    const uint64_t n = (uint64_t)c->K * (c->T + 1);
    HIPCHK(hipMalloc(&c->d_diff, n * sizeof(int32_t)));
    HIPCHK(hipMemsetAsync(c->d_diff, 0, n * sizeof(int32_t), c->stream));
    const uint64_t words = (c->T + 1 + 31) / 32 + 1;
    HIPCHK(hipMalloc(&c->d_boundary, words * sizeof(uint32_t)));
    HIPCHK(hipMemsetAsync(c->d_boundary, 0, words * sizeof(uint32_t), c->stream));
    return 0;
}

struct hml_recorder_kind {
    const char* family;
    size_t elem;
    size_t counter;
    const char* none;
    const char* noun;
    const char* file;
};
static const hml_recorder_kind hml_recorder_kinds[HML_REC_KINDS] = {
    {"levels", sizeof(double), offsetof(hml_model, n_levels_recorded),
     "no emission levels were recorded by %s context: enable them with hml_set_level_recording (or HML_LEVELS=1) before the recorded sweeps", "emission levels", "levels"},
    {"breaks", sizeof(uint32_t), offsetof(hml_model, n_breaks_recorded),
     "no breakpoints were recorded by %s context: enable them with hml_set_break_recording (or HML_BREAKS=1) before the recorded sweeps", "breakpoints", "breakpoints"},
    {"bands", sizeof(int32_t), offsetof(hml_model, n_bands_recorded),
     "no level bands were recorded by %s context: give the edges with hml_set_level_bands (or HML_BANDS=e0,e1,...) before the recorded sweeps", "level bands", "bands"},
};
static int recorder_rows(const hml_ctx* c, int kind) {
    return kind == HML_REC_LEVELS ? 2 * c->D : kind == HML_REC_BREAKS ? 1 : c->D * (c->n_band_edges + 1);
}
static unsigned long long* recorder_counter(const hml_ctx* c, int kind) {
    return (unsigned long long*)((char*)c->d_mdl + hml_recorder_kinds[kind].counter);
}
static int recorder_none(int kind, const char* whose) {
    char buf[256];
    snprintf(buf, sizeof buf, hml_recorder_kinds[kind].none, whose);
    return set_err(HML_ERR_ARG, buf);
}

static int ensure_recorder_buffers(hml_ctx* c, int kind) {
    hml_recorder& r = c->rec[kind];
    if (r.d_acc) return 0;
    if (kind == HML_REC_BANDS && (c->n_band_edges < 1 || recorder_rows(c, kind) > HML_CAP_K))
        return set_err(HML_ERR_ARG, "level bands: the data dimensions times (edges + 1) must be between 2 and 64 columns");
    const uint64_t bytes = (uint64_t)recorder_rows(c, kind) * (c->T + 1) * hml_recorder_kinds[kind].elem;
    const uint64_t words = (c->T + 32) / 32;
    HIPCHK(hipMalloc(&r.d_acc, bytes));
    HIPCHK(hipMalloc(&r.d_boundary, words * sizeof(uint32_t)));
    HIPCHK(hipMemsetAsync(r.d_acc, 0, bytes, c->stream));
    HIPCHK(hipMemsetAsync(r.d_boundary, 0, words * sizeof(uint32_t), c->stream));
    hipStreamCaptureStatus cap = hipStreamCaptureStatusNone;
    if (hipStreamIsCapturing(c->stream, &cap) == hipSuccess && cap == hipStreamCaptureStatusNone) HIPCHK(hipStreamSynchronize(c->stream));
    return 0;
}
static int ensure_recorders(hml_ctx* c) {
    for (int kind = 0; kind < HML_REC_KINDS; ++kind)
        if (c->rec[kind].on) { if (int r = ensure_recorder_buffers(c, kind)) return r; }
    return 0;
}

static hml_band_edges band_edges_of(const hml_ctx* c) {
    hml_band_edges ed;
    memset(&ed, 0, sizeof ed);
    ed.n = c->n_band_edges;
    for (int j = 0; j < c->n_band_edges; ++j) ed.e[j] = c->band_edges[j];
    return ed;
}
static bool same_band_edges(const hml_ctx* a, int n, const float* edges) {
    return a->n_band_edges == n && memcmp(a->band_edges, edges, (size_t)n * sizeof(float)) == 0;
}

static void launch_record_kernel(hml_ctx* c, int kind, hipStream_t s, dim3 grid) {
    const hml_recorder& r = c->rec[kind];
    if (kind == HML_REC_LEVELS)
        hipLaunchKernelGGL(hml_k_levels_record, grid, dim3(256), 0, s, c->d_q, c->d_starts, c->d_mdl, r.acc<double>(), r.d_boundary);
    else if (kind == HML_REC_BREAKS)
        hipLaunchKernelGGL(hml_k_breaks_record, grid, dim3(256), 0, s, c->d_q, c->d_starts, c->d_mdl, r.acc<uint32_t>(), r.d_boundary);
    else
        hipLaunchKernelGGL(hml_k_bands_record, grid, dim3(256), 0, s, c->d_q, c->d_starts, c->d_mdl, band_edges_of(c), r.acc<int32_t>(), r.d_boundary);
}

static int launch_recorders(hml_ctx* c, hipStream_t s, uint32_t hint) {
    for (int kind = 0; kind < HML_REC_KINDS; ++kind) {
        if (!c->rec[kind].on) continue;
        if (int r = ensure_recorder_buffers(c, kind)) return r;
        ProfScope ps(c, hml_recorder_kinds[kind].family);
        launch_record_kernel(c, kind, s, dim3(grid_for(hint, 256, 64, 16384)));
    }
    return 0;
}


#define HML_TRE_TUNE_AFTER 48u
static uint32_t tre_default_L_old(uint32_t hint) { return hint >= (1u << 26) ? 128u : hint >= (1u << 24) ? 64u : (uint32_t)HML_TRE_MIN_L; }
static int tre_candidates(const hml_ctx* c, uint32_t hint, uint32_t* out) {
    int n = 0;
    if (!c->tre_rows || c->tre_slots <= 0) {
        const uint32_t L0 = tre_default_L_old(hint);
        for (uint32_t q = 4; q <= 8; ++q) {
            const uint32_t l = L0 * q / 4u;
            if (l % 32u == 0u && l <= 256u) out[n++] = l;
        }
        return n;
    }
    const uint32_t blocks = hint > 1024u ? (uint32_t)(((uint64_t)hint - 1024u) * 4u / 5u) : hint;
    for (uint32_t rounds = 1; rounds <= 8u && n < 6; ++rounds) {
        const double waves = 0.985 * (double)c->tre_slots * rounds;
        uint32_t l = (uint32_t)((double)blocks / (64.0 * waves)) + 1u;
        l = (l + 31u) / 32u * 32u;
        if (l < (uint32_t)HML_TRE_MIN_L) l = HML_TRE_MIN_L;
        if (l > (c->tre_ckpt ? (uint32_t)HML_TRE_MAX_L : 512u)) continue;
        bool seen = false;
        for (int i = 0; i < n; ++i) seen = seen || out[i] == l;
        if (!seen) out[n++] = l;
        if (l == (uint32_t)HML_TRE_MIN_L) break;
    }
    if (n == 0) out[n++] = 512u;
    return n;
}
static uint32_t tre_default_L(const hml_ctx* c, uint32_t hint) {
    if (!c->tre_rows || c->tre_slots <= 0) return tre_default_L_old(hint);
    uint32_t cand[8];
    const int n = tre_candidates(c, hint, cand);
    return cand[n > 1 ? 1 : 0];
}
static bool tre_tuned_for(const hml_ctx* c, uint32_t hint) {
    return c->tre_tuned_L && hint <= c->tre_tuned_hint + c->tre_tuned_hint / 8u && hint + hint / 8u >= c->tre_tuned_hint;
}
static bool tre_wants_measurement(const hml_ctx* c, uint32_t hint) {
    return !c->tre_L && c->tre_autotune && !tre_tuned_for(c, hint) && c->tre_dense_sweeps >= HML_TRE_TUNE_AFTER;
}
static uint32_t tre_pick_L(hml_ctx* c, uint32_t hint, bool capturing, bool* measure) {
    *measure = false;
    if (c->tre_L) return c->tre_L;
    if (tre_tuned_for(c, hint)) return c->tre_tuned_L;
    if (capturing || !tre_wants_measurement(c, hint)) return c->tre_tuned_L ? c->tre_tuned_L : tre_default_L(c, hint);
    if (c->tre_tune_step < 0) {
        c->tre_cand_n = tre_candidates(c, hint, c->tre_cand);
        if (c->tre_cand_n < 2) { c->tre_tuned_L = c->tre_cand[0]; c->tre_tuned_hint = hint; return c->tre_cand[0]; }
        c->tre_tune_step = 0;
        for (float& v : c->tre_tune_ms) v = 3.4e38f;
    }
    *measure = true;
// ... 41 lines not shown
```

### hammlet_amd/csrc/hml_ctx.hpp

```cpp
#ifndef HML_CTX_HPP
#define HML_CTX_HPP

#include <hip/hip_runtime.h>

#include <atomic>
#include <map>
#include <string>
#include <utility>
#include <vector>

#include "../../include/hml.h"
#include "hml_host_common.hpp"
#include "hml_state.h"

struct hml_trace {
    std::atomic<int> refs{1};
    float* d_w = nullptr;
    uint8_t* d_summary = nullptr;
    float* d_coeff = nullptr;
    float2* d_ia = nullptr;
};

struct ProfAcc { double ms = 0; uint64_t n = 0; uint32_t tick = 0; std::vector<std::pair<hipEvent_t, hipEvent_t>> pending; };

enum { HML_REC_LEVELS = 0, HML_REC_BREAKS = 1, HML_REC_BANDS = 2, HML_REC_KINDS = 3 };
struct hml_recorder {
    bool on = false;
    bool asked = false;
    void* d_acc = nullptr;
    uint32_t* d_boundary = nullptr;
    template <class E> E* acc() const { return static_cast<E*>(d_acc); }
};

struct hml_ctx {
    int device = 0;
    hipStream_t stream = nullptr;
    bool own_stream = false;
    uint64_t seed = 0;
    uint32_t chain = 0;
    uint64_t T = 0;
    int K = 0;
    int D = 1, P = 0;
    bool loaded = false, model_set = false;
    bool dynamic = true;
    bool blocks_valid = false;
    double sigma = 0;
    hml_trace* trace = nullptr;
    float* d_w = nullptr;
    uint8_t* d_summary = nullptr;
    int32_t key_base = 0;
    double key_scale = 1.0;
    bool use_keys = true;
    bool fused_blocks = true;
    uint64_t host_draws = 0;
    bool summary_always = false;
    float* d_coeff = nullptr;
    float2* d_ia = nullptr;
    uint16_t* d_stage = nullptr;
    uint32_t *d_span_count = nullptr, *d_starts = nullptr;
    float2* d_bstat = nullptr;
    uint32_t n_spans = 0;
    uint32_t* d_coarse1 = nullptr;
    unsigned long long* d_group_word = nullptr;
    uint32_t* d_wave_total = nullptr;
    int fused_slots = 0;
    uint32_t fused_spin_limit = 4096;
    bool fused_keep = false;
    unsigned long long* d_dbg = nullptr;
    bool use_graph = false;
    hipGraphExec_t graph_exec = nullptr;
    char graph_method = 0;
    uint32_t graph_hint = 0;
    bool graph_dynamic = false, graph_valid_blocks = false;
    bool graph_fused = false;
    float *d_em = nullptr, *d_gsc = nullptr, *d_rows = nullptr, *d_eprobe = nullptr, *d_aprobe = nullptr;
    float *d_entry = nullptr, *d_exitA = nullptr;
    uint32_t* d_redo = nullptr;
    uint32_t* d_redo2 = nullptr;
    uint32_t* d_tre_bitmap = nullptr;
    uint32_t* d_tre_ckpt = nullptr;
    bool late_rescale = true;
    uint32_t tre_L = 0;
    bool tre_autotune = true;
    uint32_t tre_tuned_L = 0, tre_tuned_hint = 0;
    int tre_tune_step = -1;
    float tre_tune_ms[8] = {0, 0, 0, 0, 0, 0, 0, 0};
    uint32_t tre_cand[8] = {0, 0, 0, 0, 0, 0, 0, 0};
    int tre_cand_n = 0;
    uint64_t tre_dense_sweeps = 0;
    uint32_t graph_tre_L = 0;
    int tre_slots = 0;
    bool stage_bits = true;
    uint32_t tre_refit_rounds = 2;
    bool tre_ckpt = true;
    bool tre_rows = true;
    bool tre_fused = true;
    uint32_t* d_touched = nullptr;
    uint32_t* d_fb = nullptr;
    unsigned long long *d_smap = nullptr, *d_cmap = nullptr;
    unsigned long long *d_scmap = nullptr, *d_super = nullptr;
    uint8_t *d_bentry = nullptr, *d_bentry2 = nullptr;
    int16_t* d_q = nullptr;
    double* d_partial = nullptr;
    bool params_spread = false;
    int32_t* d_diff = nullptr;
    uint32_t* d_boundary = nullptr;
    hml_recorder rec[HML_REC_KINDS];
    int n_band_edges = 0;
    float band_edges[31] = {};
    hml_model* d_mdl = nullptr;
    uint32_t* h_B = nullptr;
    uint64_t cap = 0;
    uint64_t cap_opt = 0;
    std::vector<uint8_t> sweep_log;
    unsigned long long log_base = 0;
    unsigned long long requested = 0;
    unsigned long long call_base = 0;
    uint64_t grown = 0;
    uint32_t* d_hB = nullptr;
    uint32_t B_hint = 0;
    bool hint_stale = true;
    int fwdL = 4, fwdW = 12;
    uint32_t fwd_burnin_sweeps = 64, fwd_quiet_need = 16;
    int fwdW_init = 24;
    hml_layout lay = {2, 0};
    int fwdL_dense = 16;
    hml_layout lay_dense = {4, 0};
    int fwdL_mid = 8;
    hml_layout lay_mid = {3, 0};
    uint32_t mid_min_blocks = 1u << 18;
    int fwdL_many = 8;
    hml_layout lay_many = {3, 0};
    uint32_t dense_min_blocks = 1u << 22;
    bool graph_dense = false, graph_mid = false;
    bool probes = false;
    bool rec_marginals = true;
    hml_record_cb cb = nullptr;
    void* cb_user = nullptr;
    int fm_slots = 0;
    void* d_many = nullptr;
    int many_cap = 0;
    bool compat = false;
    void* d_mt = nullptr;
    float* d_crows = nullptr;
    void* d_cchunk = nullptr;
    uint32_t* d_cdraws = nullptr;
    void* d_clists = nullptr;
    int compat_chunks = 0;
    int compat_warmup = 0;
    bool wide = false;
    void* d_wacc = nullptr;
    float* d_wA = nullptr;
    int wide_lanes = 1;
    int wide_w0 = 32;
    uint32_t wide_max_chunks = 0;
    uint64_t wide_chunks_cap = 0;
    int wide_lshift = -1;
    bool pooled = false;
    std::vector<int32_t> pool_perm;
    int profiling = 0;
    uint32_t prof_tick = 0;
    std::map<std::string, ProfAcc> prof;
    std::vector<hipEvent_t> ev_pool;
};

int hml_ctx_bind(hml_ctx* c);
int hml_ctx_fetch_model(hml_ctx* c, hml_model* out);
int hml_ctx_ensure_marginal_buffers(hml_ctx* c);
int hml_settle(hml_ctx* c);
int hml_ctx_gather_marginal_segments(hml_ctx* c, uint64_t* M, DevBuf& d_seg, DevBuf& d_g);

#endif
```

### hammlet_amd/csrc/hml_k_blocks.h

```cpp
#ifndef HML_K_BLOCKS_H
#define HML_K_BLOCKS_H

#include "hml_state.h"


typedef float hml_f4 __attribute__((ext_vector_type(4)));

HML_KERNEL __launch_bounds__(256) void hml_k_compact_scan(const float* __restrict__ w, uint32_t T,
                                                          const hml_model* __restrict__ mdl, float thr_override,
                                                          int use_override, uint16_t* __restrict__ stage,
                                                          uint32_t* __restrict__ span_count) {
    const int wave = threadIdx.x >> 6, lane = threadIdx.x & 63;
    const uint32_t span = blockIdx.x * 4u + (uint32_t)wave;
    const uint64_t base = (uint64_t)span * HML_SPAN;
    if (base >= T) return;
    const float thr = use_override ? thr_override : mdl->thr;
    uint32_t running = 0;
    uint16_t* __restrict__ out = stage + base;
    if (base + HML_SPAN <= T) {
        hml_f4 v[16];
        const hml_f4* __restrict__ p = reinterpret_cast<const hml_f4*>(w + base) + lane;
#pragma unroll
        for (int it = 0; it < 16; ++it) v[it] = __builtin_nontemporal_load(p + it * 64);
#pragma unroll
// ... 257 lines not shown
        const uint32_t in_group = (uint32_t)wave * HML_SUM_SPANS + (uint32_t)k;
        const uint32_t span = first + in_group;
        if (span >= n_spans) break;
        const uint32_t cnt = __shfl(cnt_l, (int)in_group);
        const uint32_t off = __shfl(excl_l, (int)in_group);
        const bool is_last = (span == n_spans - 1u);
        const uint32_t base = span * (uint32_t)HML_SPAN;
        const uint16_t* __restrict__ in = stage + (uint64_t)base;
        for (uint32_t i = lane; i < cnt; i += 64) if (off + i < cap) starts[off + i] = base + (uint32_t)in[i];
        if (is_last && lane == 0) {
            const uint32_t B = off + cnt;
            if (B > cap) hml_halt(mdl, B, host_B);
            else {
                mdl->B = B;
                hml_warmup_for_many_blocks(mdl, B);
                starts[B] = T;
                if (host_B) __hip_atomic_store(host_B, B, __ATOMIC_RELAXED, __HIP_MEMORY_SCOPE_SYSTEM);
            }
        }
    }
}
HML_KERNEL __launch_bounds__(256) void hml_k_compact_scatter(const uint16_t* __restrict__ stage,
                                                             const uint32_t* __restrict__ span_count,
                                                             const uint32_t* __restrict__ group_total, uint32_t n_spans,
                                                             uint32_t T, hml_model* __restrict__ mdl,
                                                             uint32_t* __restrict__ starts, uint32_t* __restrict__ host_B) {
    hml_b_compact_scatter(stage, span_count, group_total, n_spans, T, mdl, starts, host_B);
}


__device__ __forceinline__ void hml_wave_lds_order() {
    __builtin_amdgcn_fence(__ATOMIC_RELEASE, "wavefront");
    __builtin_amdgcn_wave_barrier();
    __builtin_amdgcn_fence(__ATOMIC_ACQUIRE, "wavefront");
}
HML_KERNEL __launch_bounds__(256) void hml_k_compact_scan_bits(const float* __restrict__ w, uint32_t T,
                                                               const hml_model* __restrict__ mdl, float thr_override,
                                                               int use_override, unsigned long long* __restrict__ stage_bits,
                                                               uint32_t* __restrict__ span_count) {
    const int wave = threadIdx.x >> 6, lane = threadIdx.x & 63;
    const uint32_t span = blockIdx.x * 4u + (uint32_t)wave;
    const uint64_t base = (uint64_t)span * HML_SPAN;
    if (base >= T) return;
    const float thr = use_override ? thr_override : mdl->thr;
    uint32_t running = 0;
    unsigned long long mine = 0ull;
    if (base + HML_SPAN <= T) {
        hml_f4 v[16];
        const hml_f4* __restrict__ p = reinterpret_cast<const hml_f4*>(w + base) + lane;
#pragma unroll
        for (int it = 0; it < 16; ++it) v[it] = __builtin_nontemporal_load(p + it * 64);
#pragma unroll
        for (int it = 0; it < 16; ++it) {
            bool f0 = !(v[it].x < thr);
            const bool f1 = !(v[it].y < thr), f2 = !(v[it].z < thr), f3 = !(v[it].w < thr);
            if (span == 0 && it == 0 && lane == 0) f0 = true;
            const unsigned long long m0 = __ballot(f0), m1 = __ballot(f1), m2 = __ballot(f2), m3 = __ballot(f3);
            mine = (lane == 4 * it) ? m0 : (lane == 4 * it + 1) ? m1 : (lane == 4 * it + 2) ? m2 : (lane == 4 * it + 3) ? m3 : mine;
            running += __popcll(m0) + __popcll(m1) + __popcll(m2) + __popcll(m3);
        }
    } else {
        for (int it = 0; it < 16; ++it) {
            bool f[4];
#pragma unroll
            for (int j = 0; j < 4; ++j) {
                const uint64_t t = base + (uint64_t)it * 256u + (uint64_t)lane * 4u + j;
                f[j] = (t < T) ? (t == 0 || !(w[t] < thr)) : false;
            }
            const unsigned long long m0 = __ballot(f[0]), m1 = __ballot(f[1]), m2 = __ballot(f[2]), m3 = __ballot(f[3]);
            mine = (lane == 4 * it) ? m0 : (lane == 4 * it + 1) ? m1 : (lane == 4 * it + 2) ? m2 : (lane == 4 * it + 3) ? m3 : mine;
            running += __popcll(m0) + __popcll(m1) + __popcll(m2) + __popcll(m3);
        }
    }
    stage_bits[(uint64_t)span * 64u + (uint32_t)lane] = mine;
    if (lane == 0) span_count[span] = running;
}

HML_KERNEL __launch_bounds__(256) void hml_k_compact_scatter_bits(const unsigned long long* __restrict__ stage_bits,
                                                                  const uint32_t* __restrict__ span_count,
                                                                  const uint32_t* __restrict__ group_total, uint32_t n_spans,
                                                                  uint32_t T, hml_model* __restrict__ mdl,
                                                                  uint32_t* __restrict__ starts, uint32_t* __restrict__ host_B) {
    static_assert(4 * HML_SUM_SPANS == HML_GROUP_SPANS && HML_GROUP_SPANS <= 64, "one workgroup per span group");
    __shared__ uint32_t part[4];
    __shared__ uint32_t buf[4][256];
    const int wave = threadIdx.x >> 6, lane = threadIdx.x & 63;
    const uint32_t g = blockIdx.x;
    const uint32_t first = g * HML_GROUP_SPANS;
    const uint32_t cap = mdl->cap;
    uint32_t acc = 0u;
    for (uint32_t i = threadIdx.x; i < g; i += 256u) acc += group_total[i];
    const uint32_t cnt_l = ((uint32_t)lane < HML_GROUP_SPANS && first + (uint32_t)lane < n_spans) ? span_count[first + (uint32_t)lane] : 0u;
    acc = hml_wave_sum_u32(acc);
    if (lane == 0) part[wave] = acc;
    __syncthreads();
    const uint32_t before_group = part[0] + part[1] + part[2] + part[3];
    uint32_t incl = cnt_l;
#pragma unroll
    for (int d = 1; d < HML_GROUP_SPANS; d <<= 1) {
        const uint32_t o = __shfl_up(incl, d);
        if (lane >= d) incl += o;
    }
    const uint32_t excl_l = before_group + incl - cnt_l;
    uint32_t* const mybuf = buf[wave];
    const unsigned long long lt = (1ull << lane) - 1ull;
    unsigned long long word[HML_SUM_SPANS];
#pragma unroll
    for (int k = 0; k < HML_SUM_SPANS; ++k) {
        const uint32_t span = first + (uint32_t)wave * HML_SUM_SPANS + (uint32_t)k;
        word[k] = (span < n_spans) ? stage_bits[(uint64_t)span * 64u + (uint32_t)lane] : 0ull;
    }
#pragma unroll
    for (int k = 0; k < HML_SUM_SPANS; ++k) {
        const uint32_t in_group = (uint32_t)wave * HML_SUM_SPANS + (uint32_t)k;
        const uint32_t span = first + in_group;
        if (span >= n_spans) break;
        const uint32_t cnt = __shfl(cnt_l, (int)in_group);
        const uint32_t off = __shfl(excl_l, (int)in_group);
        const uint32_t base = span * (uint32_t)HML_SPAN;
        const uint32_t wlo = (uint32_t)word[k], whi = (uint32_t)(word[k] >> 32);
        uint32_t running = 0u;
        for (int it = 0; it < 16; ++it) {
            unsigned long long m[4];
#pragma unroll
            for (int j = 0; j < 4; ++j)
                m[j] = ((unsigned long long)(uint32_t)__builtin_amdgcn_readlane((int)whi, 4 * it + j) << 32) |
                       (unsigned long long)(uint32_t)__builtin_amdgcn_readlane((int)wlo, 4 * it + j);
            const uint32_t n_it = (uint32_t)(__popcll(m[0]) + __popcll(m[1]) + __popcll(m[2]) + __popcll(m[3]));
            if (n_it == 0u) continue;
            uint32_t pos = (uint32_t)(__popcll(m[0] & lt) + __popcll(m[1] & lt) + __popcll(m[2] & lt) + __popcll(m[3] & lt));
            const uint32_t t0 = base + (uint32_t)it * 256u + (uint32_t)lane * 4u;
#pragma unroll
            for (int j = 0; j < 4; ++j)
                if ((m[j] >> lane) & 1ull) mybuf[pos++] = t0 + (uint32_t)j;
            hml_wave_lds_order();
            for (uint32_t i = (uint32_t)lane; i < n_it; i += 64u) if (off + running + i < cap) starts[off + running + i] = mybuf[i];
            hml_wave_lds_order();
            running += n_it;
        }
        if (span == n_spans - 1u && lane == 0) {
            const uint32_t B = off + cnt;
            if (B > cap) hml_halt(mdl, B, host_B);
            else {
                mdl->B = B;
                hml_warmup_for_many_blocks(mdl, B);
                starts[B] = T;
                if (host_B) __hip_atomic_store(host_B, B, __ATOMIC_RELAXED, __HIP_MEMORY_SCOPE_SYSTEM);
            }
        }
    }
}


__device__ __forceinline__ void hml_block_stats_one(const float2* __restrict__ ia, uint32_t start, uint32_t end,
                                                    float& s, float& q) {
    float ps = 0.0f, pq = 0.0f, es = 0.0f, eq = 0.0f;
    {
        const float2 v = ia[start];
        const float y = v.x - es, t = ps + y; es = (t - ps) - y; ps = t;
        const float y2 = v.y - eq, t2 = pq + y2; eq = (t2 - pq) - y2; pq = t2;
    }
    for (uint64_t c = ((uint64_t)start + HML_CELLSIZE) / HML_CELLSIZE * HML_CELLSIZE; c < end; c += HML_CELLSIZE) {
        const float2 v = ia[c];
        const float y = v.x - es, t = ps + y; es = (t - ps) - y; ps = t;
        const float y2 = v.y - eq, t2 = pq + y2; eq = (t2 - pq) - y2; pq = t2;
    }
    float ns = 0.0f, nq = 0.0f;
    if (end % HML_CELLSIZE != 0) {
        const float2 v = ia[end];
        const float y = v.x - 0.0f; ns = 0.0f + y;
        const float y2 = v.y - 0.0f; nq = 0.0f + y2;
    }
    s = ps - ns;
    q = pq - nq;
}

HML_KERNEL __launch_bounds__(256) void hml_k_block_stats(const float2* __restrict__ ia,
                                                         const uint32_t* __restrict__ starts,
                                                         const hml_model* __restrict__ mdl,
                                                         float2* __restrict__ bstat) {
    const uint32_t B = mdl->B;
    const uint32_t stride = gridDim.x * blockDim.x;
    for (uint32_t b = blockIdx.x * blockDim.x + threadIdx.x; b < B; b += stride) {
        const uint32_t s = starts[b], e = starts[b + 1];
        float sx, sq;
        hml_block_stats_one(ia, s, e, sx, sq);
        bstat[b] = make_float2(sx, sq);
    }
}

#endif
```

### hammlet_amd/csrc/hml_state.h

```cpp
#ifndef HML_STATE_H
#define HML_STATE_H

#include "hml_common.h"
#include "hml_philox.h"

#define HML_TRE_HALO_MAX 128
#define HML_SPAN 4096
#define HML_GROUP_SPANS 16
#define HML_REDUCE_CHUNK 256
#define HML_REDUCE_GROUPS 1024
#define HML_BWD_CHUNK 64
#define HML_FWD_GROUP 16
struct hml_layout {
    uint32_t lshift;
    uint32_t cstride;
};
HML_HD uint64_t hml_bk(const hml_layout lay, uint32_t b, int K, int s) {
    const uint32_t r = b & ((1u << lay.lshift) - 1u), c = b >> lay.lshift;
    return ((uint64_t)r * (uint32_t)K + (uint32_t)s) * lay.cstride + c;
}

#define HML_CNT_SPLIT 16

enum {
    HML_DEVERR_NONE = 0,
    HML_DEVERR_IP_NOT_FINITE = 1,
    HML_DEVERR_NEG_BACKWARD = 2,
    HML_DEVERR_NEG_SUMSQ = 3,
    HML_DEVERR_NIG_ALPHA = 4,
    HML_DEVERR_NIG_BETA = 5,
    HML_DEVERR_NIG_NU = 6,
    HML_DEVERR_NIG_MU0 = 7,
    HML_DEVERR_MEAN_NOT_FINITE = 8,
    HML_DEVERR_VAR_NOT_FINITE = 9,
    HML_DEVERR_VAR_NOT_POSITIVE = 10,
    HML_DEVERR_TOO_MANY_RECORDS = 11,
    HML_DEVERR_LAUNCH_GEOMETRY = 12
};

#define HML_MAX_D 4

struct hml_model {
    int32_t K;
    int32_t D, P;
    uint8_t map[HML_CAP_K][HML_MAX_D];
    float logNs[HML_CAP_K];
    uint64_t stat_stride;
    int32_t self_trans;
    int32_t dynamic;
    uint32_t T;
    float nig_prior[4];
    float a_off, a_diag, pi_alpha;
    hml_key key;
    float mu[HML_CAP_K], var[HML_CAP_K], sd[HML_CAP_K];
    double rvar2[HML_CAP_K];
    float logN[HML_CAP_K];
    float logA[HML_CAP_K];
    float A[HML_CAP_K * HML_CAP_K];
    float pi[HML_CAP_K];
    float thr;
    float thr_theta;
    float nig_post[HML_CAP_K][4];
    float dirA[HML_CAP_K * HML_CAP_K];
    float dirPi[HML_CAP_K];
    uint32_t B;
    uint32_t n_spans;
    uint32_t cap;
    uint32_t halted;
    unsigned long long trans[HML_CNT_SPLIT][HML_MAX_K * HML_MAX_K];
    unsigned long long occ[HML_CNT_SPLIT][HML_MAX_K];
    unsigned long long last_trans[HML_CAP_K * HML_CAP_K];
    unsigned long long last_occ[HML_CAP_K];
    float last_sum[HML_CAP_K], last_sumsq[HML_CAP_K];
    unsigned long long epoch;
    unsigned long long sweeps, block_updates, uniform_fallbacks, forward_refits, forward_serial;
    unsigned long long fused_fallbacks;
    unsigned long long n_recorded;
    int32_t max_state_recorded;
    uint32_t err_code;
    float err_value;
    unsigned long long err_count;
    uint32_t fwd_mismatch;
    uint32_t fwd_mismatch2;
    uint32_t fwd_W, fwd_W0, fwd_serial_ran, fwd_quiet;
    uint32_t fwd_W_burnin;
    uint32_t fwd_burnin_sweeps;
    uint32_t fwd_quiet_need;
    uint32_t tre_fused;
    uint32_t tre_hi_shift, tre_lo_shift;
    uint32_t tre_W_floor, tre_floor_age;
    unsigned long long fwd_refits_seen, fwd_serial_seen;
    uint32_t params_ticket;
    unsigned long long dbg_t[12];
    uint32_t wl_lshift, wl_cstride;
    uint32_t wl_bwd_W, wl_bwd_quiet;
    uint32_t wl_W_need, wl_need_age;
    uint32_t wl_retry;
    unsigned long long n_levels_recorded;
    unsigned long long n_breaks_recorded;
    unsigned long long n_bands_recorded;
};

#if defined(__HIPCC__)
__device__ __forceinline__ void hml_halt(hml_model* mdl, uint32_t found, uint32_t* host_words) {
    mdl->B = 0u;
    mdl->halted = found;
    if (host_words) {
        __hip_atomic_store(host_words, found, __ATOMIC_RELAXED, __HIP_MEMORY_SCOPE_SYSTEM);
        __hip_atomic_store(host_words + 2, found, __ATOMIC_RELAXED, __HIP_MEMORY_SCOPE_SYSTEM);
    }
}
__device__ __forceinline__ void hml_warmup_for_many_blocks(hml_model* mdl, uint32_t B) {
    if (B >= (1u << 22) && !mdl->tre_fused && mdl->sweeps < 4ull && mdl->fwd_W < 4u * mdl->fwd_W_burnin) mdl->fwd_W = 4u * mdl->fwd_W_burnin;
    if (B >= (1u << 22) && mdl->tre_fused && mdl->sweeps < 4ull && mdl->fwd_W < 64u) mdl->fwd_W = 64u;
}
#endif

#endif
```

### hammlet_amd/csrc/hml_sweep.hip

```cpp
#include "hml_capi_shared.hpp"

template <int KK>
static bool fused_geometry(hml_ctx* c, uint32_t* n_sub, uint32_t* n_wg) {
    if (c->fused_slots == 0) {
        int per_cu = 0, cus = 0;
        if (hipOccupancyMaxActiveBlocksPerMultiprocessor(&per_cu, hml_k_blocks_fused<KK>, HML_FUSED_WAVES * 64, 0) != hipSuccess ||
            hipDeviceGetAttribute(&cus, hipDeviceAttributeMultiprocessorCount, c->device) != hipSuccess || per_cu <= 0 || cus <= 0) {
            (void)hipGetLastError();
            c->fused_slots = -1;
        } else {
            c->fused_slots = per_cu * cus;
        }
        if (const char* e = getenv("HML_FUSED_SLOTS")) c->fused_slots = atoi(e);
    }
    if (c->fused_slots <= 0) return false;
    const uint64_t batches = (c->T + HML_FUSED_SUB_POSITIONS - 1) / HML_FUSED_SUB_POSITIONS;
    const uint64_t m = (batches + (uint64_t)c->fused_slots - 1) / (uint64_t)c->fused_slots;
    if (m > HML_FUSED_MAX_SUB) return false;
    *n_sub = (uint32_t)m;
    *n_wg = (uint32_t)((c->T + m * HML_FUSED_SUB_POSITIONS - 1) / (m * HML_FUSED_SUB_POSITIONS));
    return true;
}


template <int KK>
static int sweep_k(hml_ctx* c, char method, bool record) {
    hipStream_t s = c->stream;
    const bool mix = (method == HML_METHOD_MIXTURE);
    const uint32_t T = (uint32_t)c->T;
    bool emitted = false, fused = false;
    if (c->hint_stale && (c->dynamic || !c->blocks_valid)) {
        hipStreamCaptureStatus cap = hipStreamCaptureStatusNone;
        if (hipStreamIsCapturing(s, &cap) == hipSuccess && cap == hipStreamCaptureStatusNone) {
            launch_compact_pair(c, 0, 0.0f);
            KLAUNCH_CHECK();
            HIPCHK(hipStreamSynchronize(s));
        }
    }
    c->hint_stale = false;
    refresh_hint(c);
    const bool dense_geo = c->B_hint >= c->dense_min_blocks;
    const bool trellis = dense_geo && !mix && c->D == 1 && c->tre_fused;
    const bool mid_geo = !dense_geo && c->fwdL_mid > c->fwdL && c->B_hint >= c->mid_min_blocks;
    const int L = dense_geo ? c->fwdL_dense : mid_geo ? c->fwdL_mid : c->fwdL;
    const hml_layout lay = dense_geo ? c->lay_dense : mid_geo ? c->lay_mid : c->lay;
    float* const gsc_plane = (!dense_geo && c->late_rescale) ? nullptr : c->d_gsc;
    const uint32_t* const starts_for_maps = gsc_plane ? nullptr : c->d_starts;
    if (c->dynamic || !c->blocks_valid) {
        uint32_t n_sub = 0u, n_wg = 0u;
        if (c->h_B[1] && !c->fused_keep) c->fused_blocks = false;
        if (c->D == 1 && c->use_keys && c->fused_blocks && !shares_device(c) &&
            !(!c->summary_always && c->B_hint && (uint64_t)c->B_hint * 24u > c->T) && fused_geometry<KK>(c, &n_sub, &n_wg)) {
            ProfScope ps(c, "blocks_compact", 1);
            hipLaunchKernelGGL(HIP_KERNEL_NAME(hml_k_blocks_fused<KK>), dim3(n_wg), dim3(HML_FUSED_WAVES * 64), 0, s, c->d_summary, c->d_w, c->d_ia,
                               T, c->d_mdl, c->key_base, c->d_group_word, c->d_stage, c->d_starts, c->d_bstat, c->d_em,
                               gsc_plane, c->probes ? c->d_eprobe : nullptr, mix ? 1 : 0, lay, c->d_hB, n_sub, c->fused_spin_limit, c->d_dbg, c->d_mdl);
            fused = true;
        } else {
            launch_compact_pair(c, 0, 0.0f);
        }
        if (!fused && !trellis) {
            refresh_hint(c);
            const uint32_t h0 = c->B_hint ? c->B_hint : (uint32_t)std::min<uint64_t>(c->T, 1u << 20);
            ProfScope ps(c, "stats_emission");
            if (c->D > 1)
                hipLaunchKernelGGL(HIP_KERNEL_NAME(hml_k_emission_mv<KK, true>), dim3(grid_for(h0, 256, 64, 16384)), dim3(256), 0, s,
                                   c->d_ia, c->d_starts, c->d_mdl, c->d_bstat, c->d_em, gsc_plane, c->probes ? c->d_eprobe : nullptr,
                                   mix ? 1 : 0, lay);
            else if (dense_geo && L <= hml_emit_tile<KK>::MAXL)
                hipLaunchKernelGGL(HIP_KERNEL_NAME(hml_k_emission_tiled<KK, true>), dim3(grid_for(h0, hml_emit_tile<KK>::BLOCKS, 64, 65536)),
                                   dim3(256), 0, s, c->d_ia, c->d_starts, c->d_mdl, c->d_bstat, c->d_em, gsc_plane,
                                   c->probes ? c->d_eprobe : nullptr, mix ? 1 : 0, lay);
            else
            hipLaunchKernelGGL(HIP_KERNEL_NAME(hml_k_stats_emission<KK>), dim3(grid_for(h0, 256, 64, 16384)), dim3(256), 0, s,
                               c->d_ia, c->d_starts, c->d_mdl, c->d_bstat, c->d_em, gsc_plane, c->probes ? c->d_eprobe : nullptr,
                               mix ? 1 : 0, lay);
        }
        KLAUNCH_CHECK();
        emitted = true;
        if (!c->dynamic) c->blocks_valid = true;
    }
    refresh_hint(c);
    const uint32_t hint = c->B_hint ? c->B_hint : (uint32_t)std::min<uint64_t>(c->T, 1u << 20);
    const int gB = grid_for(hint, 256, 64, 16384);
    if (!emitted && !trellis) {
        ProfScope ps(c, "emission");
        if (c->D > 1)
            hipLaunchKernelGGL(HIP_KERNEL_NAME(hml_k_emission_mv<KK, false>), dim3(gB), dim3(256), 0, s, c->d_ia, c->d_starts, c->d_mdl,
                               c->d_bstat, c->d_em, gsc_plane, c->probes ? c->d_eprobe : nullptr, mix ? 1 : 0, lay);
        else if (dense_geo && L <= hml_emit_tile<KK>::MAXL)
            hipLaunchKernelGGL(HIP_KERNEL_NAME(hml_k_emission_tiled<KK, false>), dim3(grid_for(hint, hml_emit_tile<KK>::BLOCKS, 64, 65536)),
                               dim3(256), 0, s, c->d_ia, c->d_starts, c->d_mdl, c->d_bstat, c->d_em, gsc_plane,
                               c->probes ? c->d_eprobe : nullptr, mix ? 1 : 0, lay);
        else
        hipLaunchKernelGGL(HIP_KERNEL_NAME(hml_k_emission<KK>), dim3(gB), dim3(256), 0, s, c->d_bstat, c->d_starts, c->d_mdl,
                           c->d_em, gsc_plane, c->probes ? c->d_eprobe : nullptr, mix ? 1 : 0, lay);
    }
    if (trellis) {
        hipStreamCaptureStatus capst = hipStreamCaptureStatusNone;
        (void)hipStreamIsCapturing(s, &capst);
        bool measure = false;
        if (c->tre_rows && c->tre_slots == 0) {
            int per_cu = 0, cus = 0;
            if (hipOccupancyMaxActiveBlocksPerMultiprocessor(&per_cu, hml_k_trellis_rows<KK, false>, 64 * HML_TR2_WAVES, 0) == hipSuccess &&
                hipDeviceGetAttribute(&cus, hipDeviceAttributeMultiprocessorCount, c->device) == hipSuccess && per_cu > 0 && cus > 0)
                c->tre_slots = per_cu * cus * HML_TR2_WAVES;
            else { (void)hipGetLastError(); c->tre_slots = -1; }
            if (const char* e = getenv("HML_TRELLIS_SLOTS")) c->tre_slots = atoi(e);
        }
        const uint32_t TL = tre_pick_L(c, hint, capst != hipStreamCaptureStatusNone, &measure);
        hipEvent_t tev0 = nullptr, tev1 = nullptr;
        if (measure) { tev0 = ev_get(c); tev1 = ev_get(c); hipEventRecord(tev0, s); }
        if (c->graph_tre_L != TL && getenv("HML_TRELLIS_TUNE_DEBUG")) fprintf(stderr, "[trellis] chunk length %u for %u blocks (%d wavefront slots)\n", TL, hint, c->tre_slots);
        c->graph_tre_L = TL;
        const uint64_t tchunks = ((uint64_t)hint + TL - 1) / TL;
        const uint64_t tgroups = (tchunks + HML_TRE_NCH - 1) / HML_TRE_NCH;
        float* ep = c->probes ? c->d_eprobe : nullptr;
        float* ap = c->probes ? c->d_aprobe : nullptr;
        {
            ProfScope ps(c, "trellis", 1);
            if (c->tre_rows && hint > 1024u && ((uint64_t)hint - 1024u) * 8u >= c->T * 9u)
                hipLaunchKernelGGL(HIP_KERNEL_NAME(hml_k_trellis_rows<KK, true>), dim3(grid_for(tgroups, HML_TR2_WAVES, 4, 1 << 20)), dim3(64 * HML_TR2_WAVES), 0, s,
                                   c->d_ia, c->d_starts, c->d_mdl, c->d_mdl, c->d_bstat, c->d_smap, c->d_cmap, c->d_entry, c->d_exitA, c->d_fb, ep, ap, c->d_tre_ckpt, TL);
            else if (c->tre_rows)
                hipLaunchKernelGGL(HIP_KERNEL_NAME(hml_k_trellis_rows<KK, false>), dim3(grid_for(tgroups, HML_TR2_WAVES, 4, 1 << 20)), dim3(64 * HML_TR2_WAVES), 0, s,
                                   c->d_ia, c->d_starts, c->d_mdl, c->d_mdl, c->d_bstat, c->d_smap, c->d_cmap, c->d_entry, c->d_exitA, c->d_fb, ep, ap, c->d_tre_ckpt, TL);
            else
            hipLaunchKernelGGL(HIP_KERNEL_NAME(hml_k_trellis_tile<KK>), dim3(grid_for(tgroups, 1, 16, 1 << 20)), dim3(64), 0, s,
                               c->d_ia, c->d_starts, c->d_mdl, c->d_mdl, c->d_bstat, c->d_smap, c->d_cmap, c->d_entry, c->d_exitA, c->d_fb, ep, ap, TL);
        }
        {
            ProfScope ps(c, "trellis_repair");
            hipLaunchKernelGGL(HIP_KERNEL_NAME(hml_k_trellis_verify<KK>), dim3(grid_for(tchunks, 256, 16, 1 << 14)), dim3(256), 0, s, c->d_mdl,
                               c->d_entry, c->d_exitA, c->d_redo, TL);
            int in_a = 1;
            for (uint32_t round = 0; round < c->tre_refit_rounds; ++round, in_a ^= 1) {
                uint32_t* lin = in_a ? c->d_redo : c->d_redo2;
                uint32_t* lout = in_a ? c->d_redo2 : c->d_redo;
                hipLaunchKernelGGL(HIP_KERNEL_NAME(hml_k_trellis_refit<KK>), dim3(4096), dim3(64), 0, s, c->d_ia, c->d_starts, c->d_mdl, c->d_smap,
                                   c->d_cmap, c->d_entry, c->d_exitA, c->d_fb, ep, ap, lin, in_a, (c->tre_rows && c->tre_ckpt) ? c->d_tre_ckpt : nullptr, TL);
                hipLaunchKernelGGL(HIP_KERNEL_NAME(hml_k_trellis_verify_list<KK>), dim3(64), dim3(256), 0, s, c->d_mdl, c->d_entry, c->d_exitA,
                                   lin, lout, c->d_touched, in_a, round, TL);
            }
            hipLaunchKernelGGL(HIP_KERNEL_NAME(hml_k_trellis_serial<KK>), dim3(1), dim3(256), 0, s, c->d_ia, c->d_starts, c->d_mdl, c->d_smap,
                               c->d_cmap, c->d_entry, c->d_exitA, c->d_fb, ep, ap, in_a ? c->d_redo : c->d_redo2, in_a, c->d_tre_bitmap, TL);
        }
        {
            ProfScope ps(c, "backward_chain");
            const uint64_t supers = (tchunks + 63) / 64;
            hipLaunchKernelGGL(HIP_KERNEL_NAME(hml_k_trellis_super<KK>), dim3(grid_for(supers * 64, 256, 16, 1 << 16)), dim3(256), 0, s, c->d_cmap,
                               c->d_mdl, c->d_scmap, c->d_super, TL);
            hipLaunchKernelGGL(HIP_KERNEL_NAME(hml_k_trellis_chain<KK>), dim3(1), dim3(1024), 0, s, c->d_super, c->d_mdl, c->d_bentry2, TL);
            hipLaunchKernelGGL(HIP_KERNEL_NAME(hml_k_trellis_states<KK>), dim3(grid_for(tgroups, 1, 16, 1 << 20)), dim3(64), 0, s, c->d_smap,
                               c->d_scmap, c->d_bentry2, c->d_mdl, c->d_q, TL);
        }
        if (measure) {
            hipEventRecord(tev1, s);
            float ms = 0.0f;
            const bool ok = hipEventSynchronize(tev1) == hipSuccess && hipEventElapsedTime(&ms, tev0, tev1) == hipSuccess;
            c->ev_pool.push_back(tev0);
            c->ev_pool.push_back(tev1);
            if (ok) tre_tune_report(c, hint, ms); else { (void)hipGetLastError(); c->tre_autotune = false; }
        }
        c->tre_dense_sweeps++;
        {
            ProfScope ps(c, "counts");
            hipLaunchKernelGGL(HIP_KERNEL_NAME(hml_k_counts_dense<KK, false>), dim3(HML_REDUCE_GROUPS), dim3(256), 0, s, c->d_q,
                               c->d_starts, c->d_bstat, c->d_mdl, c->d_partial, (const unsigned long long*)nullptr, (const uint8_t*)nullptr);
        }
    } else if (!mix) {
        const uint64_t chunks = ((uint64_t)hint + L - 1) / L;
        const int gF = grid_for(chunks, 256, 16, 1 << 20);
        {
            ProfScope ps(c, "forward");
            hipLaunchKernelGGL(HIP_KERNEL_NAME(hml_k_forward<KK>), dim3(gF), dim3(256), 0, s, c->d_em, gsc_plane, c->d_mdl, c->d_rows,
                               c->probes ? c->d_aprobe : nullptr, c->d_entry, c->d_exitA, c->d_fb, L, lay);
        }
        {
            const uint64_t bch = ((uint64_t)hint + HML_BWD_CHUNK - 1) / HML_BWD_CHUNK;
            {
                ProfScope ps(c, "backward_maps");
                hipLaunchKernelGGL(HIP_KERNEL_NAME(hml_k_backward_maps<KK>), dim3(grid_for(bch * 64, 256, 16, 1 << 18)), dim3(256), 0,
                                   s, c->d_rows, c->d_mdl, c->d_smap, c->d_cmap, lay, c->d_entry, c->d_exitA, c->d_redo, L, starts_for_maps, c->d_mdl);
            }
            ProfScope ps(c, "backward_chain");
            if (!dense_geo) {
                hipLaunchKernelGGL(HIP_KERNEL_NAME(hml_k_backward_chain<KK>), dim3(1), dim3(1024), 0, s, c->d_cmap, c->d_mdl,
                                   c->d_bentry, c->d_em, gsc_plane, c->d_rows, c->probes ? c->d_aprobe : nullptr, c->d_entry,
                                   c->d_exitA, c->d_fb, c->d_redo, c->d_touched, c->d_smap, L, lay, 3, 0, starts_for_maps);
            } else {
                hipLaunchKernelGGL(HIP_KERNEL_NAME(hml_k_backward_chain<KK>), dim3(1), dim3(1024), 0, s, c->d_cmap, c->d_mdl,
                                   c->d_bentry, c->d_em, gsc_plane, c->d_rows, c->probes ? c->d_aprobe : nullptr, c->d_entry,
                                   c->d_exitA, c->d_fb, c->d_redo, c->d_touched, c->d_smap, L, lay, 1, 0, starts_for_maps);
                hipLaunchKernelGGL(HIP_KERNEL_NAME(hml_k_backward_super<KK>), dim3(grid_for(bch, 256, 16, 1 << 16)), dim3(256), 0, s,
                                   c->d_cmap, c->d_mdl, c->d_scmap, c->d_super);
                hipLaunchKernelGGL(HIP_KERNEL_NAME(hml_k_backward_chain<KK>), dim3(1), dim3(1024), 0, s, c->d_super, c->d_mdl,
                                   c->d_bentry2, c->d_em, gsc_plane, c->d_rows, c->probes ? c->d_aprobe : nullptr, c->d_entry,
                                   c->d_exitA, c->d_fb, c->d_redo, c->d_touched, c->d_smap, L, lay, 2, 1, starts_for_maps);
                hipLaunchKernelGGL(hml_k_backward_entries, dim3(grid_for(bch, 256, 16, 1 << 16)), dim3(256), 0, s, c->d_scmap,
                                   c->d_bentry2, c->d_mdl, c->d_bentry);
            }
        }
        {
            ProfScope ps(c, "counts");
            if (c->D > 1)
                hipLaunchKernelGGL(HIP_KERNEL_NAME(hml_k_counts<KK, true, true>), dim3(HML_REDUCE_GROUPS), dim3(256), 0, s, c->d_q,
// ... 236 lines not shown
```

### include/hml.h

```cpp
#ifndef HML_H
#define HML_H

#include <stddef.h>
#include <stdint.h>

#ifdef __cplusplus
extern "C" {
#endif

typedef struct hml_ctx hml_ctx;

#define HML_METHOD_FB 'F'
#define HML_METHOD_MIXTURE 'M'

#define HML_OK 0
#define HML_ERR_ARG 1
#define HML_ERR_HIP 2
#define HML_ERR_MODEL 3

const char* hml_last_error(void);

uint32_t hml_abi_version(void);
const char* hml_device_arch(void);
int hml_device_count(int* n);

int hml_create(hml_ctx** out, int device, uint64_t seed, uint32_t chain_id, void* stream);
void hml_destroy(hml_ctx* ctx);

int hml_load_observations(hml_ctx* ctx, const float* x, uint64_t n_values);
int hml_load_observations_device(hml_ctx* ctx, const void* x_dev, uint64_t T);

int hml_attach_observations(hml_ctx* ctx, hml_ctx* source);

typedef struct hml_text hml_text;
int hml_text_open(hml_text** out, int device, uint64_t chunk_bytes);
void hml_text_close(hml_text* reader);
int hml_text_buffer(hml_text* reader, char** buf, uint64_t* capacity);
int hml_text_commit(hml_text* reader, uint64_t nbytes);
int hml_text_feed(hml_text* reader, const char* bytes, uint64_t nbytes);
int hml_text_reserve(hml_text* reader, uint64_t n_values);
int hml_text_finish(hml_text* reader, uint64_t* n_values, int* stopped);
int hml_text_values(hml_text* reader, float* out );
int hml_text_counters(hml_text* reader, uint64_t* bytes_in, uint64_t* irregular_tokens, uint64_t* host_chunks);

int hml_set_dimensions(hml_ctx* ctx, int D, int P);
int hml_get_dimensions(hml_ctx* ctx, int* D, int* P);

int hml_set_weights(hml_ctx* ctx, const float* w, uint64_t T);

int hml_noise_sigma(hml_ctx* ctx, double* sigma);

int hml_scale_weights(hml_ctx* ctx, float multiplier);

int hml_autoprior(hml_ctx* ctx, float s2, float p, float out4[4]);

int hml_set_model(hml_ctx* ctx, int K, const float nig4[4], float a_off, float a_diag, float pi_alpha,
                  int self_trans);

int hml_set_self_transitions(hml_ctx* ctx, int on);

int hml_sample_prior(hml_ctx* ctx);

int hml_set_static_blocks(hml_ctx* ctx);
int hml_set_dynamic(hml_ctx* ctx, int on);

int hml_create_blocks(hml_ctx* ctx, float threshold);

int hml_iterate(hml_ctx* ctx, char method, uint64_t iterations, uint64_t thinning);

typedef void (*hml_record_cb)(hml_ctx* ctx, uint64_t sweep_in_call, void* user);
int hml_set_recording(hml_ctx* ctx, int marginals, hml_record_cb cb, void* user);

int hml_set_option(hml_ctx* ctx, const char* name, int value);

int hml_iterate_many(hml_ctx* const* ctxs, int n, char method, uint64_t iterations, uint64_t thinning);

int hml_sync(hml_ctx* ctx);

int hml_get_num_blocks(hml_ctx* ctx, uint64_t* B);
int hml_get_blocks(hml_ctx* ctx, uint32_t* starts );
int hml_get_block_stats(hml_ctx* ctx, float* sum , float* sum_sq );
int hml_get_states(hml_ctx* ctx, int16_t* q );
int hml_get_theta(hml_ctx* ctx, float* mean_var );
int hml_get_transitions(hml_ctx* ctx, float* A , float* pi );
int hml_set_parameters(hml_ctx* ctx, const float* mean_var, const float* A, const float* pi);
int hml_get_threshold(hml_ctx* ctx, float* thr);
int hml_enable_probes(hml_ctx* ctx, int on);
int hml_get_block_loglik(hml_ctx* ctx, float* E );
int hml_get_forward_rows(hml_ctx* ctx, float* rows );
int hml_get_counts(hml_ctx* ctx, uint64_t* trans , uint64_t* occ , float* sum ,
                   float* sum_sq , uint64_t* nterms );
int hml_get_weights(hml_ctx* ctx, float* w );
int hml_get_coefficients(hml_ctx* ctx, float* c );
int hml_get_integral_array(hml_ctx* ctx, float* sum , float* sum_sq );

int hml_marginals_rle(hml_ctx* ctx, uint64_t* n_segments, int* n_columns, uint64_t* seg_len ,
                      int32_t* counts );
int hml_max_segmentation(hml_ctx* ctx, uint64_t* n_runs, uint64_t* run_len , int32_t* run_state );
int hml_marginals_dense_device(hml_ctx* ctx, void* out_dev, const int32_t* perm);
int hml_recorded_sweeps(hml_ctx* ctx, uint64_t* n);

int hml_set_level_recording(hml_ctx* ctx, int on);
int hml_levels_rle(hml_ctx* ctx, uint64_t* n_segments, uint64_t* n_recorded, uint64_t* seg_len ,
                   double* sum , double* sum_sq );
int hml_levels_dense_device(hml_ctx* ctx, void* out_dev );
int hml_levels_merge(hml_ctx* dst, hml_ctx* src);
int hml_levels_on_segments(hml_ctx* ctx, uint64_t n_cuts, const uint32_t* cuts ,
                           double* sum , double* sum_sq );

int hml_levels_agreement_rle(hml_ctx* const* ctxs, int n, uint64_t* n_segments, uint64_t* n_recorded, uint64_t* seg_len ,
                             double* within , double* between , double* rhat );
int hml_levels_agreement_dense_device(hml_ctx* const* ctxs, int n, void* out_dev );
int hml_levels_agreement_summary(hml_ctx* const* ctxs, int n, double threshold, uint64_t* n_above , double* max_finite ,
                                 uint64_t* n_infinite );

int hml_set_break_recording(hml_ctx* ctx, int on);
int hml_breaks_list(hml_ctx* ctx, uint64_t* n_breaks, uint64_t* n_recorded, uint32_t* pos , uint32_t* count );
int hml_breaks_dense_device(hml_ctx* ctx, void* out_dev , uint32_t window);
int hml_breaks_merge(hml_ctx* dst, hml_ctx* src);
int hml_breaks_consensus(hml_ctx* ctx, uint32_t window, uint64_t min_count, uint64_t* n_selected, uint32_t* pos ,
                         uint64_t* mass , uint32_t* peak );

int hml_set_level_bands(hml_ctx* ctx, int n_edges, const float* edges );
int hml_get_level_bands(hml_ctx* ctx, int* n_edges, float* edges );
int hml_bands_rle(hml_ctx* ctx, uint64_t* n_segments, int* n_columns, uint64_t* n_recorded, uint64_t* seg_len ,
                  int32_t* counts );
int hml_bands_dense_device(hml_ctx* ctx, void* out_dev , int cumulative);
int hml_bands_call(hml_ctx* ctx, uint64_t rank, uint64_t* n_runs, uint64_t* run_len , int32_t* run_band );
int hml_bands_merge(hml_ctx* dst, hml_ctx* src);

#define HML_RECORDING_LEVELS 0
#define HML_RECORDING_BREAKS 1
#define HML_RECORDING_BANDS 2
int hml_recording_payload_size(hml_ctx* ctx, int kind, uint64_t* n_bytes);
int hml_recording_export(hml_ctx* ctx, int kind, void* payload_dev, uint64_t capacity_bytes, uint64_t* n_bytes);
int hml_recording_merge_payload(hml_ctx* dst, int kind, const void* payload_dev, uint64_t n_bytes);
int hml_recording_merge_across(hml_ctx* dst, hml_ctx* src, int kind);

int hml_categorical_draw(hml_ctx* ctx, const float* weights, int K, uint32_t* index);

int hml_relabel_permutation(hml_ctx* ctx, int32_t* perm );
int hml_pool_payload_size(hml_ctx* ctx, uint64_t* n_int32);
int hml_pool_export(hml_ctx* ctx, void* payload_dev, int32_t* perm_out_or_null);
int hml_pool_install(hml_ctx* ctx, const void* payload_dev);
typedef struct hml_pool hml_pool;
#define HML_POOL_ID_BYTES 128
int hml_pool_unique_id(void* id );
int hml_pool_create(hml_pool** out, int device, int rank, int n_ranks, const void* id);
void hml_pool_destroy(hml_pool* pool);
int hml_pool_marginals(hml_pool* pool, hml_ctx* ctx, int32_t* perm_out_or_null);
int hml_pool_info(hml_pool* pool, int* rank, int* n_ranks, double* last_allreduce_ms, uint64_t* last_bytes, int* rccl_version);
int hml_pool_set_form(hml_pool* pool, int form);
int hml_pool_last(hml_pool* pool, int* form, uint64_t* entries);
int hml_allreduce_marginals(hml_ctx* const* ctxs, int n);
int hml_allreduce_marginals_perm(hml_ctx* const* ctxs, int n, int32_t* perms );
int hml_pool_permutation(hml_ctx* ctx, int32_t* perm );

typedef struct {
    uint64_t sweeps;
    uint64_t block_updates;
    uint64_t uniform_fallbacks;
    uint64_t forward_refits;
    uint64_t forward_serial;
    uint64_t forward_warmup;
    uint64_t fused_fallbacks;
    uint64_t buffer_growths;
    uint64_t block_capacity;
} hml_stats;
int hml_get_stats(hml_ctx* ctx, hml_stats* out);

int hml_profile_enable(hml_ctx* ctx, int level);
int hml_profile_get(hml_ctx* ctx, const char* name, double* total_ms, uint64_t* launches);

int hml_debug_eval(int device, int fn, const float* a, const float* b_or_null, float* out, uint64_t n, uint64_t seed);

int hml_synth_gauss(float* x, int16_t* states_or_null, uint64_t T, int K, const float* mu, float sigma,
                    double mean_dwell, uint64_t seed, int nthreads);

int hml_synth_depth(float* x, int16_t* states_or_null, uint64_t T, double depth, double ln_sigma, uint64_t seed, int nthreads);

#ifdef __cplusplus
}
#endif
#endif
```

Before: 3.094 billion block-updates/s.

## Add candidate block-boundary table to skip full-position scans in dynamic block builds

```diff
diff --git a/hammlet_amd/capi.py b/hammlet_amd/capi.py
--- a/hammlet_amd/capi.py
+++ b/hammlet_amd/capi.py
@@ -17,7 +17,8 @@
 class HmlStats(C.Structure):
     _fields_ = [("sweeps", C.c_uint64), ("block_updates", C.c_uint64), ("uniform_fallbacks", C.c_uint64),
                 ("forward_refits", C.c_uint64), ("forward_serial", C.c_uint64), ("forward_warmup", C.c_uint64),
-                ("fused_fallbacks", C.c_uint64), ("buffer_growths", C.c_uint64), ("block_capacity", C.c_uint64)]
+                ("fused_fallbacks", C.c_uint64), ("buffer_growths", C.c_uint64), ("block_capacity", C.c_uint64),
+                ("table_builds", C.c_uint64), ("table_misses", C.c_uint64)]
 
 
 RECORD_CB = C.CFUNCTYPE(None, C.c_void_p, C.c_uint64, C.c_void_p)
diff --git a/hammlet_amd/csrc/hml_capi.hip b/hammlet_amd/csrc/hml_capi.hip
--- a/hammlet_amd/csrc/hml_capi.hip
+++ b/hammlet_amd/csrc/hml_capi.hip
@@ -199,6 +199,11 @@
     if (const char* e = getenv("HML_COMPAT")) c->compat = atoi(e) != 0;
     if (const char* e = getenv("HML_TRELLIS_TUNE")) c->tre_autotune = atoi(e) != 0;
     if (const char* e = getenv("HML_FUSED_SPIN_LIMIT")) c->fused_spin_limit = (uint32_t)strtoul(e, nullptr, 10);
+    if (const char* e = getenv("HML_BLOCK_TABLE")) c->tb.enable = atoi(e) != 0;
+    if (const char* e = getenv("HML_TABLE_AFTER")) c->tb.after = (uint32_t)std::max(0, atoi(e));
+    if (const char* e = getenv("HML_TABLE_MARGIN")) { const float m = strtof(e, nullptr); if (m >= 0.0f && m < 1.0f) c->tb.margin = m; }
+    if (const char* e = getenv("HML_TABLE_MAX_SHIFT")) c->tb.max_shift = (uint32_t)std::min(31, std::max(0, atoi(e)));
+    c->tb.next = c->tb.after;
     if (const char* e = getenv("HML_LEVELS")) c->rec[HML_REC_LEVELS].on = c->rec[HML_REC_LEVELS].asked = atoi(e) != 0;
     if (const char* e = getenv("HML_BREAKS")) c->rec[HML_REC_BREAKS].on = c->rec[HML_REC_BREAKS].asked = atoi(e) != 0;
     if (const char* e = getenv("HML_MAX_BLOCKS")) c->cap_opt = strtoull(e, nullptr, 10);
@@ -236,7 +241,7 @@
     trace_release(c);
     free_sweep_buffers(c);
     void* ptrs[] = {c->d_group_word, c->d_wave_total, c->d_stage, c->d_span_count, c->d_starts, c->d_bstat, c->d_eprobe, c->d_aprobe, c->d_coarse1,
-                    c->d_diff, c->d_boundary, c->d_mdl, c->d_many};
+                    c->d_diff, c->d_boundary, c->d_mdl, c->d_many, c->d_table, c->d_table_word};
     for (void* p : ptrs) if (p) hipFree(p);
     for (hml_recorder& r : c->rec) { if (r.d_acc) hipFree(r.d_acc); if (r.d_boundary) hipFree(r.d_boundary); }
     if (c->h_B) hipHostFree(c->h_B);
@@ -490,6 +495,8 @@
     if (!c || !c->loaded) return set_err(HML_ERR_ARG, "no observations loaded");
     if (trace_shared(c)) return set_err(HML_ERR_ARG, "the weights are shared with attached contexts: scale them before hml_attach_observations");
     if (int r = ctx_bind(c)) return r;
+    if (int r = settle_if_limited(c)) return r;
+    hml_table_drop(c->tb);
     hipLaunchKernelGGL(hml_k_scale, dim3(grid_for(c->T, 256, 1, 65536)), dim3(256), 0, c->stream, c->d_w, c->T, mult);
     KLAUNCH_CHECK();
     c->key_scale *= std::fabs((double)mult) > 0 ? std::fabs((double)mult) : 1.0;
@@ -503,6 +510,8 @@
     if (T != c->T) return set_err(HML_ERR_MODEL, "Block structure and statistics have different number of data points!");
     if (trace_shared(c)) return set_err(HML_ERR_ARG, "the weights are shared with attached contexts: set them before hml_attach_observations");
     if (int r = ctx_bind(c)) return r;
+    if (int r = settle_if_limited(c)) return r;
+    hml_table_drop(c->tb);
     HIPCHK(hipMemcpyAsync(c->d_w, w, T * sizeof(float), hipMemcpyHostToDevice, c->stream));
     HIPCHK(hipStreamSynchronize(c->stream));
     if (int r = build_keys(c)) return r;
@@ -699,21 +708,32 @@
 static int sweep_dispatch(hml_ctx* c, char method, bool record);
 
 int hml_settle(hml_ctx* c) {
+    if (c->settling) { HIPCHK(hipStreamSynchronize(c->stream)); return 0; }
+    struct Settling { hml_ctx* c; ~Settling() { c->settling = false; } } settling_guard{c};
+    c->settling = true;
     for (int round = 0; round < 64; ++round) {
         HIPCHK(hipStreamSynchronize(c->stream));
-        if (!chain_halted(c)) { c->sweep_log.clear(); c->log_base = c->requested; return 0; }
+        if (!chain_halted(c)) { c->sweep_log.clear(); c->log_base = c->requested; c->tb.live = false; return 0; }
         const uint64_t needed = c->h_B[2];
-        if (c->cap >= c->T) return set_err(HML_ERR_HIP, "internal error: a chain with full block capacity halted");
+        const bool miss = table_missed(c);
+        if (!miss && c->cap >= c->T) return set_err(HML_ERR_HIP, "internal error: a chain with full block capacity halted");
         std::vector<uint8_t> pending;
         if (c->model_set) {
             hml_model m;
             if (int r = fetch_model(c, &m)) return r;
-            const uint64_t ran = m.sweeps >= c->log_base ? m.sweeps - c->log_base : 0;
-            if (ran < c->sweep_log.size()) pending.assign(c->sweep_log.begin() + ran, c->sweep_log.end());
+            pending = hml_log_pending(c->sweep_log, c->log_base, m.sweeps);
             c->log_base = m.sweeps;
         }
-        if (int r = grow_capacity(c, needed)) return r;
+        if (miss) {
+            hml_table_missed(c->tb);
+            const uint32_t words[2] = {0u, 0u};
+            HIPCHK(hipMemcpyAsync(&c->d_mdl->halted, words, sizeof(uint32_t), hipMemcpyHostToDevice, c->stream));
+            HIPCHK(hipMemcpyAsync(&c->d_mdl->table_miss, words + 1, sizeof(uint32_t), hipMemcpyHostToDevice, c->stream));
+            HIPCHK(hipStreamSynchronize(c->stream));
+            c->h_B[2] = 0u; c->h_B[3] = 0u;
+        } else if (int r = grow_capacity(c, needed)) return r;
         c->sweep_log = pending;
+        const unsigned long long base = c->log_base;
         bool halted_again = false;
         for (size_t i = 0; i < pending.size() && !halted_again; ++i) {
             const char method = (pending[i] & 1) ? HML_METHOD_MIXTURE : HML_METHOD_FB;
@@ -724,7 +744,7 @@
                 halted_again = chain_halted(c);
                 if (!halted_again) {
                     if (int r = check_device_error(c)) return r;
-                    const unsigned long long ordinal = c->log_base + i;
+                    const unsigned long long ordinal = base + i;
                     c->cb(c, ordinal >= c->call_base ? (uint64_t)(ordinal - c->call_base) : 0u, c->cb_user);
                 }
             }
@@ -1192,6 +1212,13 @@
     for (int i = 0; i < n; ++i) if (!cs[i] || !cs[i]->model_set) return set_err(HML_ERR_ARG, "model not set");
     if (method != HML_METHOD_FB && method != HML_METHOD_MIXTURE) return set_err(HML_ERR_ARG, std::string("Unknown sampling type ") + method + "!");
     for (int i = 0; i < n; ++i) cs[i]->call_base = cs[i]->requested;
+    struct InMany { hml_ctx* const* cs; int n; ~InMany() { for (int i = 0; i < n; ++i) cs[i]->in_many = false; } } in_many_guard{cs, n};
+    for (int i = 0; i < n; ++i) {
+        if (int r = ctx_bind(cs[i])) return r;
+        if (int r = settle_if_limited(cs[i])) return r;
+        cs[i]->in_many = true;
+        hml_table_drop(cs[i]->tb);
+    }
     uint64_t done = 0;
     while (done < iterations && many_eligible(cs, n, method)) {
         if (int r = ctx_bind(cs[0])) return r;
@@ -1261,6 +1288,23 @@
         c->fused_blocks = value != 0;
         c->fused_keep = value == 2;
         if (c->graph_exec) { hipGraphExecDestroy(c->graph_exec); c->graph_exec = nullptr; }
+        return 0;
+    }
+    if (std::string(name) == "block_table") {
+        if (c->model_set) { if (int r = ctx_bind(c)) return r; if (int r = settle_if_limited(c)) return r; }
+        c->tb.enable = value != 0;
+        hml_table_drop(c->tb);
+        return 0;
+    }
+    if (std::string(name) == "table_after" || std::string(name) == "table_margin_ppm" || std::string(name) == "table_max_shift") {
+        const bool is_after = std::string(name) == "table_after", is_margin = std::string(name) == "table_margin_ppm";
+        if (value < 0 || (is_margin && value >= 1000000) || (!is_after && !is_margin && value > 31))
+            return set_err(HML_ERR_ARG, "table_after: sweeps >= 0; table_margin_ppm: 0 ... 999999; table_max_shift: 0 ... 31");
+        if (c->model_set) { if (int r = ctx_bind(c)) return r; if (int r = settle_if_limited(c)) return r; }
+        if (is_after) c->tb.after = (uint32_t)value;
+        else if (is_margin) c->tb.margin = (float)value * 1e-6f;
+        else c->tb.max_shift = (uint32_t)value;
+        hml_table_drop(c->tb);
         return 0;
     }
     if (std::string(name) == "compat") {
@@ -1294,7 +1338,8 @@
     } else if (c->d_dbg) {
         std::vector<unsigned long long> h(4096 * 4);
         hipMemcpy(h.data(), c->d_dbg, h.size() * 8, hipMemcpyDeviceToHost);
-        const uint32_t n = (uint32_t)std::min<uint64_t>(4096, (c->T + HML_FUSED_SUB_POSITIONS - 1) / HML_FUSED_SUB_POSITIONS);
+        const uint32_t n = c->tb.valid ? std::min(4096u, c->table_wg)
+                                       : (uint32_t)std::min<uint64_t>(4096, (c->T + HML_FUSED_SUB_POSITIONS - 1) / HML_FUSED_SUB_POSITIONS);
         unsigned long long t0 = ~0ull; for (uint32_t i = 0; i < n; ++i) if (h[i * 4]) t0 = std::min(t0, h[i * 4]);
         double mx[4] = {0, 0, 0, 0}, av[4] = {0, 0, 0, 0};
         for (uint32_t i = 0; i < n; ++i) for (int k = 0; k < 4; ++k) { const double d = (double)(h[i * 4 + k] - t0) * 0.01; mx[k] = std::max(mx[k], d); av[k] += d / n; }
@@ -1482,6 +1527,7 @@
     out->forward_warmup = m.fwd_W;
     out->fused_fallbacks = m.fused_fallbacks;
     out->buffer_growths = c->grown; out->block_capacity = c->cap;
+    out->table_builds = c->tb.builds; out->table_misses = c->tb.misses;
     return 0;
 }
 
diff --git a/hammlet_amd/csrc/hml_capi_shared.hpp b/hammlet_amd/csrc/hml_capi_shared.hpp
--- a/hammlet_amd/csrc/hml_capi_shared.hpp
+++ b/hammlet_amd/csrc/hml_capi_shared.hpp
@@ -17,6 +17,7 @@
 #include "hml_k_blocks.h"
 #include "hml_k_blocks_fused.h"
 #include "hml_k_blocks_fused_many.h"
+#include "hml_k_blocks_table.h"
 #include "hml_k_build.h"
 #include "hml_k_forward.h"
 #include "hml_k_marginals.h"
@@ -185,12 +186,59 @@
 }
 
 static inline bool cap_limited(const hml_ctx* c) { return c->cap != 0 && c->cap < c->T; }
-static inline bool chain_halted(const hml_ctx* c) { return cap_limited(c) && ((volatile uint32_t*)c->h_B)[2] != 0u; }
+static inline bool may_halt(const hml_ctx* c) { return cap_limited(c) || c->tb.live; }
+static inline bool chain_halted(const hml_ctx* c) { return may_halt(c) && ((volatile uint32_t*)c->h_B)[2] != 0u; }
+static inline bool table_missed(const hml_ctx* c) { return ((volatile uint32_t*)c->h_B)[3] != 0u; }
 static inline void log_sweep(hml_ctx* c, char method, bool record) {
-    c->requested++;
-    if (cap_limited(c)) c->sweep_log.push_back((uint8_t)((method == HML_METHOD_MIXTURE ? 1 : 0) | (record ? 2 : 0)));
-}
-static inline int settle_if_limited(hml_ctx* c) { return cap_limited(c) ? hml_settle(c) : 0; }
+    hml_log_note(c->sweep_log, c->log_base, c->requested, may_halt(c), method == HML_METHOD_MIXTURE, record);
+}
+static inline int settle_if_limited(hml_ctx* c) { return may_halt(c) ? hml_settle(c) : 0; }
+
+static int table_build(hml_ctx* c, int slots) {
+    HIPCHK(hipStreamSynchronize(c->stream));
+    float thr = 0.0f;
+    HIPCHK(hipMemcpyAsync(&thr, &c->d_mdl->thr, sizeof thr, hipMemcpyDeviceToHost, c->stream));
+    HIPCHK(hipStreamSynchronize(c->stream));
+    if (!std::isfinite(thr) || !(thr > 0.0f)) { hml_table_built(c->tb, false); return 0; }
+    const float floor = thr * (1.0f - c->tb.margin);
+    const uint32_t hint_word = c->h_B[0];
+    const int profiling = c->profiling;
+    c->profiling = 0;
+    const int r = launch_compact(c, true, floor);
+    c->profiling = profiling;
+    if (r) return r;
+    HIPCHK(hipStreamSynchronize(c->stream));
+    const uint64_t n = (uint64_t)c->h_B[0] + 1u;
+    c->h_B[0] = hint_word;
+    const uint64_t n_wg = (n + HML_TABLE_WG_RECORDS - 1) / HML_TABLE_WG_RECORDS;
+    if (c->h_B[2] != 0u || n < 2 || n > std::max<uint64_t>(c->T >> c->tb.max_shift, 2) || n >= (1ull << HML_TABLE_IDX_BITS) || slots <= 0 ||
+        n_wg > (uint64_t)slots) {
+        hml_table_built(c->tb, false);
+        return 0;
+    }
+    if (c->table_cap < n) {
+        if (c->d_table) { HIPCHK(hipFree(c->d_table)); c->d_table = nullptr; }
+        if (c->d_table_word) { HIPCHK(hipFree(c->d_table_word)); c->d_table_word = nullptr; }
+        c->table_cap = 0;
+        const uint64_t cap = n + n / 4 + HML_TABLE_WG_RECORDS;
+        HIPCHK(hipMalloc(&c->d_table, cap * sizeof(hml_table_rec)));
+        HIPCHK(hipMalloc(&c->d_table_word, (cap / HML_TABLE_WG_RECORDS + 2) * sizeof(unsigned long long)));
+        c->table_cap = cap;
+    }
+    HIPCHK(hipMemsetAsync(c->d_table_word, 0, (c->table_cap / HML_TABLE_WG_RECORDS + 2) * sizeof(unsigned long long), c->stream));
+    hipLaunchKernelGGL(hml_k_table_gather, dim3(grid_for(n, 256, 1, 4096)), dim3(256), 0, c->stream, c->d_starts, c->d_w, c->d_ia, (uint32_t)c->T,
+                       (uint32_t)n, (hml_table_rec*)c->d_table);
+    KLAUNCH_CHECK();
+    struct { float floor; uint32_t n; uint32_t miss; } words = {floor, (uint32_t)n, 0u};
+    static_assert(offsetof(hml_model, table_n) == offsetof(hml_model, table_floor) + 4 && offsetof(hml_model, table_miss) == offsetof(hml_model, table_floor) + 8,
+                  "floor, record count and miss flag are written together");
+    HIPCHK(hipMemcpyAsync(&c->d_mdl->table_floor, &words, sizeof words, hipMemcpyHostToDevice, c->stream));
+    HIPCHK(hipStreamSynchronize(c->stream));
+    c->table_n = (uint32_t)n;
+    c->table_wg = (uint32_t)n_wg;
+    hml_table_built(c->tb, true);
+    return 0;
+}
 
 #define NEED_MODEL() if (!c || !c->model_set) return set_err(HML_ERR_ARG, "model not set"); if (int r_ = ctx_bind(c)) return r_; if (int r_ = settle_if_limited(c)) return r_
 #define NEED_LOADED() if (!c || !c->loaded) return set_err(HML_ERR_ARG, "no observations loaded"); if (int r_ = ctx_bind(c)) return r_; if (int r_ = settle_if_limited(c)) return r_
diff --git a/hammlet_amd/csrc/hml_ctx.hpp b/hammlet_amd/csrc/hml_ctx.hpp
--- a/hammlet_amd/csrc/hml_ctx.hpp
+++ b/hammlet_amd/csrc/hml_ctx.hpp
@@ -12,6 +12,7 @@
 #include "../../include/hml.h"
 #include "hml_host_common.hpp"
 #include "hml_state.h"
+#include "hml_table_host.hpp"
 
 struct hml_trace {
     std::atomic<int> refs{1};
@@ -67,6 +68,14 @@
     uint32_t fused_spin_limit = 4096;
     bool fused_keep = false;
     unsigned long long* d_dbg = nullptr;
+    void* d_table = nullptr;
+    unsigned long long* d_table_word = nullptr;
+    uint64_t table_cap = 0;
+    uint32_t table_n = 0, table_wg = 0;
+    int table_slots = 0;
+    hml_table_book tb;
+    bool settling = false;
+    bool in_many = false;
     bool use_graph = false;
     hipGraphExec_t graph_exec = nullptr;
     char graph_method = 0;
diff --git a/hammlet_amd/csrc/hml_k_blocks.h b/hammlet_amd/csrc/hml_k_blocks.h
--- a/hammlet_amd/csrc/hml_k_blocks.h
+++ b/hammlet_amd/csrc/hml_k_blocks.h
@@ -433,11 +433,11 @@
 }
 
 
-__device__ __forceinline__ void hml_block_stats_one(const float2* __restrict__ ia, uint32_t start, uint32_t end,
-                                                    float& s, float& q) {
+__device__ __forceinline__ void hml_block_stats_ends(const float2* __restrict__ ia, uint32_t start, uint32_t end,
+                                                     const float2 v_start, const float2 v_end, float& s, float& q) {
     float ps = 0.0f, pq = 0.0f, es = 0.0f, eq = 0.0f;
     {
-        const float2 v = ia[start];
+        const float2 v = v_start;
         const float y = v.x - es, t = ps + y; es = (t - ps) - y; ps = t;
         const float y2 = v.y - eq, t2 = pq + y2; eq = (t2 - pq) - y2; pq = t2;
     }
@@ -448,12 +448,18 @@
     }
     float ns = 0.0f, nq = 0.0f;
     if (end % HML_CELLSIZE != 0) {
-        const float2 v = ia[end];
+        const float2 v = v_end;
         const float y = v.x - 0.0f; ns = 0.0f + y;
         const float y2 = v.y - 0.0f; nq = 0.0f + y2;
     }
     s = ps - ns;
     q = pq - nq;
+}
+__device__ __forceinline__ void hml_block_stats_one(const float2* __restrict__ ia, uint32_t start, uint32_t end,
+                                                    float& s, float& q) {
+    const float2 v_start = ia[start];
+    const float2 v_end = (end % HML_CELLSIZE != 0) ? ia[end] : make_float2(0.0f, 0.0f);
+    hml_block_stats_ends(ia, start, end, v_start, v_end, s, q);
 }
 
 HML_KERNEL __launch_bounds__(256) void hml_k_block_stats(const float2* __restrict__ ia,
diff --git a/hammlet_amd/csrc/hml_k_blocks_table.h b/hammlet_amd/csrc/hml_k_blocks_table.h
--- /dev/null
+++ b/hammlet_amd/csrc/hml_k_blocks_table.h
@@ -0,0 +1,210 @@
+#ifndef HML_K_BLOCKS_TABLE_H
+#define HML_K_BLOCKS_TABLE_H
+
+#include "hml_k_blocks_fused.h"
+
+struct __attribute__((aligned(16))) hml_table_rec {
+    uint32_t pos;
+    float w;
+    float2 ia;
+};
+
+#define HML_TABLE_THREADS 512
+#define HML_TABLE_PER_THREAD 4
+#define HML_TABLE_WG_RECORDS (HML_TABLE_THREADS * HML_TABLE_PER_THREAD)
+#define HML_TABLE_IDX_BITS 27
+#define HML_TABLE_CNT_BITS 12
+__device__ __forceinline__ unsigned long long hml_table_word(uint32_t gen, uint32_t count, uint32_t last_idx) {
+    static_assert(25 + HML_TABLE_CNT_BITS + HML_TABLE_IDX_BITS == 64 && (1u << (HML_TABLE_CNT_BITS - 1)) >= HML_TABLE_WG_RECORDS, "bit fields of the word");
+    return ((unsigned long long)(gen & HML_FUSED_GEN_MASK) << (HML_TABLE_CNT_BITS + HML_TABLE_IDX_BITS)) |
+           ((unsigned long long)count << HML_TABLE_IDX_BITS) | (unsigned long long)last_idx;
+}
+__device__ __forceinline__ bool hml_table_selected(const hml_table_rec& r, uint32_t idx, uint32_t n_rec, float thr) {
+    return idx < n_rec && (idx == 0u || idx == n_rec - 1u || !(r.w < thr));
+}
+__device__ __forceinline__ unsigned long long hml_table_wg_word(const hml_table_rec* __restrict__ table, uint32_t n_rec, float thr,
+                                                                uint32_t wg, uint32_t gen) {
+    uint32_t count = 0u, last = 0u;
+    const uint32_t first = wg * (uint32_t)HML_TABLE_WG_RECORDS;
+    for (uint32_t i = first; i < first + (uint32_t)HML_TABLE_WG_RECORDS && i < n_rec; ++i) {
+        const hml_table_rec r = table[i];
+        if (hml_table_selected(r, i, n_rec, thr)) { ++count; last = i; }
+    }
+    return hml_table_word(gen, count, last);
+}
+
+HML_KERNEL __launch_bounds__(256) void hml_k_table_gather(const uint32_t* __restrict__ starts, const float* __restrict__ w,
+                                                          const float2* __restrict__ ia, uint32_t T, uint32_t n_rec,
+                                                          hml_table_rec* __restrict__ table) {
+    const uint32_t stride = gridDim.x * blockDim.x;
+    for (uint32_t i = blockIdx.x * blockDim.x + threadIdx.x; i < n_rec; i += stride) {
+        const uint32_t t = (i == n_rec - 1u) ? T : starts[i];
+        hml_table_rec r;
+        r.pos = t;
+        r.w = (t < T) ? w[t] : 0.0f;
+        r.ia = ia[t <= T ? t : T];
+        table[i] = r;
+    }
+}
+
+template <int K>
+HML_KERNEL __launch_bounds__(HML_TABLE_THREADS) void hml_k_blocks_table(const hml_table_rec* __restrict__ table, const float2* __restrict__ ia,
+                                                                      uint32_t T, hml_model* __restrict__ mdl,
+                                                                      unsigned long long* __restrict__ group_word,
+                                                                      uint32_t* __restrict__ starts, float2* __restrict__ bstat,
+                                                                      float* __restrict__ em, float* __restrict__ gsc,
+                                                                      float* __restrict__ eprobe, int mixture, const hml_layout lay,
+                                                                      uint32_t* __restrict__ host_words, uint32_t spin_limit,
+                                                                      unsigned long long* __restrict__ dbg,
+                                                                      const hml_model* __restrict__ mdl_ro) {
+    constexpr uint32_t NT = HML_TABLE_THREADS;
+    constexpr int NW = HML_TABLE_THREADS / 64;
+    constexpr int PT = HML_TABLE_PER_THREAD;
+    const float thr = mdl_ro->thr;
+    const uint32_t n_rec = mdl_ro->table_n;
+    if (!(thr >= mdl_ro->table_floor) || n_rec < 2u) {
+        if (blockIdx.x == 0 && threadIdx.x == 0) {
+            mdl->B = 0u;
+            mdl->halted = 1u;
+            mdl->table_miss = 1u;
+            if (host_words) {
+                __hip_atomic_store(host_words + 3, 1u, __ATOMIC_RELAXED, __HIP_MEMORY_SCOPE_SYSTEM);
+                __hip_atomic_store(host_words + 2, 1u, __ATOMIC_RELAXED, __HIP_MEMORY_SCOPE_SYSTEM);
+            }
+        }
+        return;
+    }
+    if (dbg && threadIdx.x == 0) dbg[blockIdx.x * 4 + 0] = wall_clock64();
+    __shared__ uint32_t sel_pos[HML_TABLE_WG_RECORDS];
+    __shared__ float2 sel_ia[HML_TABLE_WG_RECORDS];
+    __shared__ uint32_t plane_count[PT][NW];
+    __shared__ unsigned long long red_sum[NW], red_near[NW];
+    __shared__ uint64_t sm_exp_tab[32];
+    if (threadIdx.x < 32u) sm_exp_tab[threadIdx.x] = HML_EXP2F_TAB[threadIdx.x];
+    constexpr bool LOOPED = K > 6;
+    __shared__ hml_emit_lds<LOOPED ? K : 1> sm_emit;
+    if (LOOPED) hml_emit_lds_fill<LOOPED ? K : 1>(sm_emit, mdl_ro, (int)threadIdx.x);
+
+    const int lane = threadIdx.x & 63, wave = threadIdx.x >> 6;
+    const uint32_t g = blockIdx.x;
+    const uint32_t gen = hml_fused_generation(mdl_ro);
+    const uint32_t cap = mdl_ro->cap;
+    const uint32_t first_rec = g * (uint32_t)HML_TABLE_WG_RECORDS;
+
+    hml_table_rec rec[PT];
+    bool sel[PT];
+    unsigned long long ball[PT];
+#pragma unroll
+    for (int j = 0; j < PT; ++j) {
+        const uint32_t idx = first_rec + (uint32_t)j * NT + threadIdx.x;
+        if (idx < n_rec) {
+            const hml_f4 v = __builtin_nontemporal_load(reinterpret_cast<const hml_f4*>(table) + idx);
+            rec[j].pos = __float_as_uint(v.x); rec[j].w = v.y; rec[j].ia = make_float2(v.z, v.w);
+        } else {
+            rec[j].pos = 0u; rec[j].w = 0.0f; rec[j].ia = make_float2(0.0f, 0.0f);
+        }
+    }
+#pragma unroll
+    for (int j = 0; j < PT; ++j) {
+        const uint32_t idx = first_rec + (uint32_t)j * NT + threadIdx.x;
+        sel[j] = hml_table_selected(rec[j], idx, n_rec, thr);
+        ball[j] = __ballot(sel[j]);
+        if (lane == 0) plane_count[j][wave] = (uint32_t)__popcll(ball[j]);
+    }
+    __syncthreads();
+    uint32_t wg_count = 0u, wg_last = 0u;
+    uint32_t my_rank[PT];
+#pragma unroll
+    for (int j = 0; j < PT; ++j) {
+#pragma unroll
+        for (int q = 0; q < NW; ++q) {
+            const uint32_t n = plane_count[j][q];
+            if (q == wave) my_rank[j] = wg_count + hml_mbcnt(ball[j]);
+            if (n) wg_last = first_rec + (uint32_t)j * NT + (uint32_t)q * 64u;
+            wg_count += n;
+        }
+    }
+    __shared__ uint32_t sm_last;
+#pragma unroll
+    for (int j = 0; j < PT; ++j)
+        if (ball[j] && wg_last == first_rec + (uint32_t)j * NT + (uint32_t)wave * 64u && lane == 0)
+            sm_last = wg_last + (63u - (uint32_t)__clzll((long long)ball[j]));
+#pragma unroll
+    for (int j = 0; j < PT; ++j)
+        if (sel[j]) { sel_pos[my_rank[j]] = rec[j].pos; sel_ia[my_rank[j]] = rec[j].ia; }
+    __syncthreads();
+    if (dbg && threadIdx.x == 0) dbg[blockIdx.x * 4 + 1] = wall_clock64();
+    if (threadIdx.x == 0)
+        __hip_atomic_store(&group_word[g], hml_table_word(gen, wg_count, wg_count ? sm_last : 0u), __ATOMIC_RELAXED, __HIP_MEMORY_SCOPE_AGENT);
+
+    unsigned long long acc = 0ull, near = 0ull;
+    for (uint32_t i = threadIdx.x; i < g; i += NT) {
+        unsigned long long d = spin_limit ? __hip_atomic_load(&group_word[i], __ATOMIC_RELAXED, __HIP_MEMORY_SCOPE_AGENT)
+                                          : hml_table_word(gen + 1u, 0u, 0u);
+        uint32_t tries = 0u;
+        while ((uint32_t)(d >> (HML_TABLE_CNT_BITS + HML_TABLE_IDX_BITS)) != gen) {
+            if (tries++ >= spin_limit) {
+                d = hml_table_wg_word(table, n_rec, thr, i, gen);
+                __hip_atomic_store(&group_word[i], d, __ATOMIC_RELAXED, __HIP_MEMORY_SCOPE_AGENT);
+                if (host_words) __hip_atomic_store(host_words + 1, 1u, __ATOMIC_RELAXED, __HIP_MEMORY_SCOPE_SYSTEM);
+                atomicAdd(&mdl->fused_fallbacks, 1ull);
+                break;
+            }
+            __builtin_amdgcn_s_sleep(1);
+            d = __hip_atomic_load(&group_word[i], __ATOMIC_RELAXED, __HIP_MEMORY_SCOPE_AGENT);
+        }
+        const uint32_t cnt = (uint32_t)(d >> HML_TABLE_IDX_BITS) & ((1u << HML_TABLE_CNT_BITS) - 1u);
+        acc += cnt;
+        if (cnt) near = (d & ((1ull << HML_TABLE_IDX_BITS) - 1ull)) + 1ull;
+    }
+#pragma unroll
+    for (int m = 1; m < 64; m <<= 1) {
+        acc += __shfl_xor(acc, m);
+        const unsigned long long o = __shfl_xor(near, m);
+        near = o > near ? o : near;
+    }
+    if (lane == 0) { red_sum[wave] = acc; red_near[wave] = near; }
+    __syncthreads();
+    unsigned long long sum_all = 0ull, nr = 0ull;
+#pragma unroll
+    for (int k = 0; k < NW; ++k) { sum_all += red_sum[k]; nr = red_near[k] > nr ? red_near[k] : nr; }
+    const uint32_t before_group = (uint32_t)sum_all;
+    uint32_t prev_pos = 0u;
+    float2 prev_ia = make_float2(0.0f, 0.0f);
+    if (threadIdx.x == 0 && wg_count && nr) {
+        const hml_table_rec r = table[(uint32_t)(nr - 1ull)];
+        prev_pos = r.pos; prev_ia = r.ia;
+    }
+    if (dbg && threadIdx.x == 0) dbg[blockIdx.x * 4 + 2] = wall_clock64();
+
+    hml_emit_params<LOOPED ? 1 : K> p;
+    if (!LOOPED) hml_emit_load<LOOPED ? 1 : K>(p, mdl_ro, mixture);
+    const bool self_trans = mdl_ro->self_trans != 0;
+    for (uint32_t k = threadIdx.x; k < wg_count; k += NT) {
+        const uint32_t b = before_group + k;
+        const uint32_t t = sel_pos[k];
+        if (b > cap) continue;
+        starts[b] = t;
+        if (t == 0u) continue;
+        const uint32_t pt = k ? sel_pos[k - 1u] : prev_pos;
+        const float2 pv = k ? sel_ia[k - 1u] : prev_ia;
+        float sx, sq;
+        hml_block_stats_ends(ia, pt, t, pv, sel_ia[k], sx, sq);
+        bstat[b - 1u] = make_float2(sx, sq);
+        const uint32_t n = t - pt;
+        if constexpr (LOOPED)
+            hml_emit_block_looped<K>(reinterpret_cast<const hml_emit_lds<K>&>(sm_emit), mdl, self_trans, b - 1u, sx, sq, (float)n, em, gsc, eprobe, mixture, lay, sm_exp_tab);
+        else
+            hml_emit_block<LOOPED ? 1 : K, true>(p, mdl, b - 1u, sx, sq, (float)n, em, gsc, eprobe, mixture, lay, sm_exp_tab);
+    }
+    if (dbg) { __syncthreads(); if (threadIdx.x == 0) dbg[blockIdx.x * 4 + 3] = wall_clock64(); }
+    if (g == gridDim.x - 1u && threadIdx.x == 0) {
+        const uint32_t Bn = before_group + wg_count - 1u;
+        if (Bn > cap) { hml_halt(mdl, Bn, host_words); return; }
+        mdl->B = Bn;
+        hml_warmup_for_many_blocks(mdl, Bn);
+        if (host_words) __hip_atomic_store(host_words, Bn, __ATOMIC_RELAXED, __HIP_MEMORY_SCOPE_SYSTEM);
+    }
+}
+
+#endif
diff --git a/hammlet_amd/csrc/hml_state.h b/hammlet_amd/csrc/hml_state.h
--- a/hammlet_amd/csrc/hml_state.h
+++ b/hammlet_amd/csrc/hml_state.h
@@ -99,6 +99,9 @@
     unsigned long long n_levels_recorded;
     unsigned long long n_breaks_recorded;
     unsigned long long n_bands_recorded;
+    float table_floor;
+    uint32_t table_n;
+    uint32_t table_miss;
 };
 
 #if defined(__HIPCC__)
diff --git a/hammlet_amd/csrc/hml_sweep.hip b/hammlet_amd/csrc/hml_sweep.hip
--- a/hammlet_amd/csrc/hml_sweep.hip
+++ b/hammlet_amd/csrc/hml_sweep.hip
@@ -37,7 +37,26 @@
             HIPCHK(hipStreamSynchronize(s));
         }
     }
+    if (c->hint_stale) hml_table_drop(c->tb);
     c->hint_stale = false;
+    if (hml_table_due(c->tb) && c->dynamic && c->D == 1 && c->use_keys && c->fused_blocks && !(c->h_B[1] && !c->fused_keep) && !shares_device(c) &&
+        !cap_limited(c) && !c->in_many && !c->use_graph) {
+        hipStreamCaptureStatus cap = hipStreamCaptureStatusNone;
+        if (hipStreamIsCapturing(s, &cap) == hipSuccess && cap == hipStreamCaptureStatusNone) {
+            if (c->table_slots == 0) {
+                int per_cu = 0, cus = 0;
+                if (hipOccupancyMaxActiveBlocksPerMultiprocessor(&per_cu, hml_k_blocks_table<KK>, HML_TABLE_THREADS, 0) != hipSuccess ||
+                    hipDeviceGetAttribute(&cus, hipDeviceAttributeMultiprocessorCount, c->device) != hipSuccess || per_cu <= 0 || cus <= 0) {
+                    (void)hipGetLastError();
+                    c->table_slots = -1;
+                } else {
+                    c->table_slots = per_cu * cus;
+                }
+            }
+            if (int r = table_build(c, c->table_slots)) return r;
+        }
+    }
+    c->tb.age++;
     refresh_hint(c);
     const bool dense_geo = c->B_hint >= c->dense_min_blocks;
     const bool trellis = dense_geo && !mix && c->D == 1 && c->tre_fused;
@@ -52,6 +71,12 @@
         if (c->D == 1 && c->use_keys && c->fused_blocks && !shares_device(c) &&
             !(!c->summary_always && c->B_hint && (uint64_t)c->B_hint * 24u > c->T) && fused_geometry<KK>(c, &n_sub, &n_wg)) {
             ProfScope ps(c, "blocks_compact", 1);
+            if (c->tb.valid && c->dynamic && !c->in_many) {
+                hipLaunchKernelGGL(HIP_KERNEL_NAME(hml_k_blocks_table<KK>), dim3(c->table_wg), dim3(HML_TABLE_THREADS), 0, s, (const hml_table_rec*)c->d_table,
+                                   c->d_ia, T, c->d_mdl, c->d_table_word, c->d_starts, c->d_bstat, c->d_em, gsc_plane, c->probes ? c->d_eprobe : nullptr,
+                                   mix ? 1 : 0, lay, c->d_hB, c->fused_spin_limit, c->table_wg <= 4096u ? c->d_dbg : nullptr, c->d_mdl);
+                c->tb.live = true;
+            } else
             hipLaunchKernelGGL(HIP_KERNEL_NAME(hml_k_blocks_fused<KK>), dim3(n_wg), dim3(HML_FUSED_WAVES * 64), 0, s, c->d_summary, c->d_w, c->d_ia,
                                T, c->d_mdl, c->key_base, c->d_group_word, c->d_stage, c->d_starts, c->d_bstat, c->d_em,
                                gsc_plane, c->probes ? c->d_eprobe : nullptr, mix ? 1 : 0, lay, c->d_hB, n_sub, c->fused_spin_limit, c->d_dbg, c->d_mdl);
diff --git a/hammlet_amd/csrc/hml_table_host.hpp b/hammlet_amd/csrc/hml_table_host.hpp
--- /dev/null
+++ b/hammlet_amd/csrc/hml_table_host.hpp
@@ -0,0 +1,49 @@
+#ifndef HML_TABLE_HOST_HPP
+#define HML_TABLE_HOST_HPP
+
+#include <algorithm>
+#include <cstdint>
+#include <vector>
+
+#define HML_TABLE_MAX_MISSES 3
+
+struct hml_table_book {
+    bool enable = true;
+    uint32_t after = 32;
+    float margin = 0.01f;
+    uint32_t max_shift = 6;
+    bool valid = false;
+    bool live = false;
+    bool off = false;
+    uint64_t age = 0;
+    uint64_t next = 32;
+    uint32_t chain_misses = 0;
+    uint64_t builds = 0, misses = 0;
+};
+
+inline void hml_table_drop(hml_table_book& b) { b.valid = false; b.age = 0; b.next = b.after; }
+inline bool hml_table_due(const hml_table_book& b) { return b.enable && !b.off && !b.valid && b.age >= b.next; }
+inline void hml_table_built(hml_table_book& b, bool usable) {
+    if (usable) { b.valid = true; ++b.builds; }
+    else b.next = b.age + std::max<uint64_t>(std::max<uint64_t>(b.age, b.after), 1);
+}
+inline void hml_table_missed(hml_table_book& b) {
+    ++b.misses;
+    b.valid = false;
+    b.next = b.age;
+    if (++b.chain_misses >= HML_TABLE_MAX_MISSES) b.off = true;
+}
+
+inline void hml_log_note(std::vector<uint8_t>& log, unsigned long long& log_base, unsigned long long& requested, bool may_have_halted,
+                         bool mixture, bool record) {
+    ++requested;
+    if (!may_have_halted) { log.clear(); log_base = requested - 1; }
+    log.push_back((uint8_t)((mixture ? 1 : 0) | (record ? 2 : 0)));
+}
+inline std::vector<uint8_t> hml_log_pending(const std::vector<uint8_t>& log, unsigned long long log_base, unsigned long long sweeps_done) {
+    const unsigned long long ran = sweeps_done >= log_base ? sweeps_done - log_base : 0;
+    if (ran >= log.size()) return {};
+    return std::vector<uint8_t>(log.begin() + (size_t)ran, log.end());
+}
+
+#endif
diff --git a/include/hml.h b/include/hml.h
--- a/include/hml.h
+++ b/include/hml.h
@@ -166,6 +166,8 @@
     uint64_t fused_fallbacks;
     uint64_t buffer_growths;
     uint64_t block_capacity;
+    uint64_t table_builds;
+    uint64_t table_misses;
 } hml_stats;
 int hml_get_stats(hml_ctx* ctx, hml_stats* out);
 
```

Result: slower. 2.928 billion block-updates/s (-5.4%).
